# DrorT/demucs

Measured on AMD Instinct MI355X. Metric: real-time factor (audio-sec/wall-sec) htdemucs 4-stem 44.1kHz stereo, 1/8 GPU, higher is better.
Workload: dtype f32

## Files before the change

### demucs_amd/_lib.py

```python
from __future__ import annotations

import ctypes as C
import os
import threading

_HERE = os.path.dirname(os.path.abspath(__file__))
LIB_PATH = os.environ.get("DEMUCS_AMD_LIB") or os.path.join(_HERE, "libdemucs_amd.so")

MI_OK = 0


class MiTensorDesc(C.Structure):
    _fields_ = [("name", C.c_char_p), ("data", C.c_void_p), ("numel", C.c_int64)]


class MiConfig(C.Structure):
    _fields_ = [("n_sources", C.c_int32), ("segment_length", C.c_int32), ("max_batch", C.c_int32),
                ("dtype", C.c_int32)]


class MiProfileRow(C.Structure):
    _fields_ = [("name", C.c_char * 48), ("launches", C.c_int64), ("ms", C.c_double), ("flops", C.c_double),
                ("bytes", C.c_double)]


class MiConvDesc(C.Structure):
    _fields_ = [
        ("wt", C.c_void_p), ("M", C.c_int32), ("Mpad", C.c_int32), ("K", C.c_int32), ("Kpad", C.c_int32),
        ("ktab", C.c_void_p),
        ("x", C.c_void_p), ("x_bstride", C.c_int64),
        ("B", C.c_int32), ("D1", C.c_int32), ("D2", C.c_int32), ("O1", C.c_int32), ("O2", C.c_int32),
        ("S1", C.c_int32), ("S2", C.c_int32),
        ("pro", C.c_int32), ("pro_stats", C.c_void_p), ("pro_w", C.c_void_p), ("pro_b", C.c_void_p),
        ("row_mode", C.c_int32),
        ("epi", C.c_int32), ("flags", C.c_int32),
        ("bias", C.c_void_p), ("scale", C.c_void_p), ("res", C.c_void_p), ("emb", C.c_void_p),
        ("y", C.c_void_p), ("y_bstride", C.c_int64), ("y_cstride", C.c_int64),
        ("stats", C.c_void_p), ("gn_stats", C.c_void_p), ("gn_w", C.c_void_p), ("gn_b", C.c_void_p),
        ("out_len", C.c_int32), ("tile_m", C.c_int32), ("plain", C.c_int32), ("half", C.c_int32),
        ("o2_valid", C.c_int32), ("ktab_len", C.c_int32), ("sink", C.c_void_p), ("wx", C.c_void_p), ("tr_stride", C.c_int32), ("tr_pad", C.c_int32), ("x_ld", C.c_int32), ("x_ld_pad", C.c_int32), ("wh", C.c_void_p),
        ("xh", C.c_void_p), ("xh_n", C.c_int64), ("yh", C.c_void_p), ("yh_n", C.c_int64),
        ("wtap", C.c_void_p), ("ntaps", C.c_int32), ("tap_k2", C.c_int32), ("tap_pad1", C.c_int32), ("tap_pad2", C.c_int32),
        ("tap_dil1", C.c_int32), ("tap_dil2", C.c_int32), ("yh_pq", C.c_int64),
        ("dma_rows", C.c_int32), ("dma_rows_pad", C.c_int32),
    ]


SIGNATURES = {
    "mi_model_create": (C.c_int, [C.POINTER(MiConfig), C.POINTER(MiTensorDesc), C.c_size_t, C.POINTER(C.c_void_p)]),
    "mi_model_destroy": (None, [C.c_void_p]),
    "mi_model_forward": (C.c_int, [C.c_void_p, C.c_void_p, C.c_void_p, C.c_int32, C.c_void_p]),
    "mi_model_forward_core": (C.c_int, [C.c_void_p, C.c_void_p, C.c_void_p, C.c_void_p, C.c_void_p, C.c_int32, C.c_void_p]),
    "mi_model_tap": (C.c_int, [C.c_void_p, C.c_char_p, C.c_void_p, C.c_int32, C.POINTER(C.c_int64), C.c_void_p]),
    "mi_hmodel_create": (C.c_int, [C.POINTER(MiConfig), C.POINTER(MiTensorDesc), C.c_size_t, C.POINTER(C.c_void_p)]),
    "mi_hmodel_destroy": (None, [C.c_void_p]),
    "mi_hmodel_forward": (C.c_int, [C.c_void_p, C.c_void_p, C.c_void_p, C.c_int32, C.c_int32, C.c_void_p]),
    "mi_hmodel_tap": (C.c_int, [C.c_void_p, C.c_char_p, C.c_void_p, C.c_int32, C.POINTER(C.c_int64), C.c_void_p]),
    "mi_hmodel_device_bytes": (C.c_int64, [C.c_void_p]),
    "mi_hmodel_status": (C.c_int, [C.c_void_p, C.c_void_p]),
    "mi_set_two_streams": (C.c_int, [C.c_int32]),
    "mi_set_split_bf16": (C.c_int, [C.c_int32]),
    "mi_set_istft_fused": (C.c_int, [C.c_int32]),
    "mi_set_transpose_tiles": (C.c_int, [C.c_int32]),
    "mi_profile_begin": (C.c_int, [C.c_void_p]),
    "mi_profile_end": (C.c_int, [C.c_void_p, C.POINTER(MiProfileRow), C.c_int32, C.POINTER(C.c_int32), C.c_void_p]),
    "mi_model_device_bytes": (C.c_int64, [C.c_void_p]),
    "mi_segments_gather": (C.c_int, [C.c_void_p, C.c_int64, C.c_int32, C.c_void_p, C.c_int32, C.c_int32, C.c_void_p,
                                     C.c_int64, C.c_void_p]),
    "mi_ola_accumulate": (C.c_int, [C.c_void_p, C.c_int64, C.c_int32, C.c_void_p, C.c_int32, C.c_int64, C.c_void_p, C.c_void_p,
                                    C.c_void_p, C.c_int32, C.c_int64, C.c_int64, C.c_void_p, C.c_int32, C.c_void_p]),
    "mi_ola_finish": (C.c_int, [C.c_void_p, C.c_int64, C.c_int32, C.c_int64, C.c_void_p, C.c_void_p, C.c_int32,
                                C.c_int32, C.c_void_p, C.c_void_p]),
    "mi_segments_gather_packed": (C.c_int, [C.c_void_p, C.c_int64, C.c_int32, C.c_void_p, C.c_int32, C.c_int32, C.c_void_p,
                                            C.c_int64, C.c_void_p]),
    "mi_ola_accumulate_packed": (C.c_int, [C.c_void_p, C.c_int64, C.c_int32, C.c_void_p, C.c_int32, C.c_int64, C.c_void_p, C.c_int32,
                                           C.c_void_p, C.c_int32, C.c_void_p, C.c_int64, C.c_void_p]),
    "mi_ola_finish_packed": (C.c_int, [C.c_void_p, C.c_int64, C.c_int32, C.c_void_p, C.c_int32, C.c_void_p, C.c_int32, C.c_void_p,
                                       C.c_int64, C.c_void_p]),
    "mi_stream_emit": (C.c_int, [C.c_void_p, C.c_int64, C.c_int32, C.c_int32, C.c_void_p, C.c_int32, C.c_void_p, C.c_int32,
                                 C.c_void_p, C.c_int64, C.c_void_p, C.c_int32, C.c_int32, C.c_int32, C.c_void_p, C.c_int64,
                                 C.c_void_p, C.c_int64, C.c_void_p]),
    "mi_streams_emit": (C.c_int, [C.c_void_p, C.c_int64, C.c_int32, C.c_int32, C.c_void_p, C.c_int32, C.c_int64, C.c_void_p,
                                  C.c_int32, C.c_void_p, C.c_int32, C.c_void_p, C.c_int64, C.c_void_p, C.c_int32, C.c_int32,
                                  C.c_int32, C.c_void_p, C.c_int32, C.c_void_p, C.c_int64, C.c_void_p]),
    "mi_streams_append": (C.c_int, [C.c_void_p, C.c_int64, C.c_int32, C.c_void_p, C.c_int32, C.c_int64, C.c_void_p, C.c_int32,
                                    C.c_void_p]),
    "mi_streams_convert_append": (C.c_int, [C.c_void_p, C.c_int64, C.c_int32, C.c_void_p, C.c_int32, C.c_int64, C.c_void_p, C.c_int64,
                                            C.c_void_p, C.c_int64, C.c_void_p, C.c_int32, C.c_int32, C.c_void_p]),
    "mi_pcm_planar": (C.c_int, [C.c_void_p, C.c_int32, C.c_int32, C.c_int64, C.c_int32, C.c_void_p, C.c_void_p, C.c_void_p]),
    "mi_streams_append_pcm": (C.c_int, [C.c_void_p, C.c_int64, C.c_int32, C.c_void_p, C.c_int32, C.c_int64, C.c_void_p, C.c_int32,
                                        C.c_void_p]),
    "mi_streams_convert_append_pcm": (C.c_int, [C.c_void_p, C.c_int64, C.c_int32, C.c_void_p, C.c_int32, C.c_int64, C.c_void_p,
                                                C.c_int64, C.c_void_p, C.c_int64, C.c_void_p, C.c_int32, C.c_int32, C.c_void_p]),
    "mi_streams_compact": (C.c_int, [C.c_void_p, C.c_int64, C.c_void_p, C.c_int64, C.c_void_p, C.c_int32, C.c_int64, C.c_void_p]),
    "mi_mono_stats_scratch_bytes": (C.c_int32, []),
    "mi_mono_stats": (C.c_int, [C.c_void_p, C.c_int32, C.c_int64, C.c_void_p, C.c_void_p, C.c_void_p]),
    "mi_mono_stats_state_bytes": (C.c_int32, []),
    "mi_mono_stats_update": (C.c_int, [C.c_void_p, C.c_int32, C.c_int32, C.c_int64, C.c_int32, C.c_int64, C.c_void_p, C.c_void_p]),
    "mi_mono_stats_finish": (C.c_int, [C.c_void_p, C.c_int64, C.c_void_p, C.c_void_p, C.c_void_p]),
    "mi_sdr_state_bytes": (C.c_int64, [C.c_int32]),
    "mi_sdr_scratch_bytes": (C.c_int64, [C.c_int32]),
    "mi_sdr_update": (C.c_int, [C.c_void_p, C.c_int32, C.c_int32, C.c_int64, C.c_void_p, C.c_int64, C.c_int32, C.c_int32, C.c_int64,
                                C.c_int64, C.c_void_p, C.c_void_p]),
    "mi_sdr_finish": (C.c_int, [C.c_void_p, C.c_int32, C.c_void_p, C.c_void_p, C.c_void_p]),
    "mi_sdr": (C.c_int, [C.c_void_p, C.c_void_p, C.c_int32, C.c_int32, C.c_int32, C.c_int64, C.c_void_p, C.c_void_p, C.c_void_p,
                         C.c_void_p]),
    "mi_track_affine": (C.c_int, [C.c_void_p, C.c_int64, C.c_void_p, C.c_int32, C.c_void_p]),
    "mi_prevent_clip": (C.c_int, [C.c_void_p, C.c_int64, C.c_int32, C.c_void_p, C.c_void_p, C.c_void_p]),
    "mi_two_stems": (C.c_int, [C.c_void_p, C.c_int32, C.c_int32, C.c_void_p, C.c_int32, C.c_int64, C.c_void_p, C.c_void_p]),
    "mi_deliver_peaks": (C.c_int, [C.c_void_p, C.c_int32, C.c_int64, C.c_int32, C.c_int32, C.c_void_p, C.c_int32, C.c_int64, C.c_void_p]),
    "mi_deliver_pcm": (C.c_int, [C.c_void_p, C.c_int32, C.c_int64, C.c_int32, C.c_int32, C.c_void_p, C.c_int32, C.c_void_p, C.c_int64,
                                 C.c_void_p]),
    "mi_deliver_resample_pcm": (C.c_int, [C.c_void_p, C.c_int32, C.c_int64, C.c_int32, C.c_int32, C.c_void_p, C.c_int64, C.c_void_p,
                                          C.c_int64, C.c_int32, C.c_void_p, C.c_int64, C.c_void_p]),
    "mi_stft_cac": (C.c_int, [C.c_void_p, C.c_int32, C.c_int32, C.c_void_p, C.c_void_p]),
    "mi_istft_cac": (C.c_int, [C.c_void_p, C.c_int32, C.c_int32, C.c_int32, C.c_void_p, C.c_void_p]),
    "mi_stft_norm": (C.c_int, [C.c_void_p, C.c_int32, C.c_int32, C.c_void_p, C.c_int32, C.c_void_p, C.c_void_p, C.c_void_p]),
    "mi_istft_full": (C.c_int, [C.c_void_p, C.c_int32, C.c_int32, C.c_int32, C.c_int32, C.c_void_p, C.c_void_p, C.c_int32, C.c_void_p,
                                C.c_void_p, C.c_void_p]),
    "mi_item_norm": (C.c_int, [C.c_void_p, C.c_int32, C.c_int64, C.c_void_p, C.c_void_p, C.c_void_p, C.c_void_p]),
    "mi_item_denorm": (C.c_int, [C.c_void_p, C.c_int32, C.c_int64, C.c_void_p, C.c_void_p, C.c_void_p]),
    "mi_conv_forward": (C.c_int, [C.POINTER(MiConvDesc), C.c_void_p]),
    "mi_resample_frac": (C.c_int, [C.c_void_p, C.c_int32, C.c_int64, C.c_void_p, C.c_int32, C.c_int32, C.c_int32, C.c_void_p, C.c_int64,
                                   C.c_void_p]),
    "mi_conv_pack_split": (C.c_int, [C.c_void_p, C.c_int32, C.c_int32, C.c_int32, C.c_void_p, C.c_void_p]),
    "mi_conv_pack_half": (C.c_int, [C.c_void_p, C.c_int32, C.c_int32, C.c_int32, C.c_void_p, C.c_void_p]),
    "mi_f32_to_image": (C.c_int, [C.c_void_p, C.c_int32, C.c_int32, C.c_int64, C.c_int32, C.c_void_p, C.c_void_p]),
    "mi_conv_pack_tap": (C.c_int, [C.c_void_p, C.c_int32, C.c_int32, C.c_int32, C.c_int32, C.c_void_p, C.c_void_p]),
    "mi_attention": (C.c_int, [C.c_void_p, C.c_void_p, C.c_void_p, C.c_void_p, C.c_int32, C.c_int32, C.c_int32,
                               C.c_int32, C.c_int64, C.c_int64, C.c_int64, C.c_int32, C.c_void_p]),
    "mi_attention_split": (C.c_int, [C.c_void_p, C.c_void_p, C.c_void_p, C.c_void_p, C.c_int32, C.c_int32, C.c_int32,
                                     C.c_int32, C.c_int64, C.c_int64, C.c_int64, C.c_void_p]),
    "mi_attention_heads": (C.c_int, [C.c_void_p, C.c_void_p, C.c_void_p, C.c_void_p, C.c_int32, C.c_int32, C.c_int32, C.c_int32,
                                     C.c_int32, C.c_int32, C.c_int32, C.c_void_p]),
    "mi_attention_heads_image": (C.c_int, [C.c_void_p, C.c_void_p, C.c_void_p, C.c_void_p, C.c_int64, C.c_int32, C.c_int32, C.c_int32,
                                           C.c_int32, C.c_int32, C.c_int32, C.c_int32, C.c_void_p]),
    "mi_attention_image": (C.c_int, [C.c_void_p, C.c_void_p, C.c_void_p, C.c_void_p, C.c_int64, C.c_int32, C.c_int32, C.c_int32,
                                     C.c_int32, C.c_int64, C.c_int64, C.c_int32, C.c_void_p]),
    "mi_lstm_seq": (C.c_int, [C.c_void_p, C.c_void_p, C.c_int32, C.c_int32, C.c_int32, C.c_void_p, C.c_int32, C.c_void_p]),
    "mi_gn_gelu": (C.c_int, [C.c_void_p, C.c_int32, C.c_int32, C.c_int32, C.c_int32, C.c_int32, C.c_int32, C.c_void_p, C.c_void_p,
                             C.c_void_p, C.c_void_p]),
    "mi_gram_order": (C.c_int32, [C.c_int32]),
    "mi_gn_gelu_gram": (C.c_int, [C.c_void_p, C.c_int32, C.c_int32, C.c_int32, C.c_int32, C.c_int32, C.c_int32, C.c_int32, C.c_void_p,
                                  C.c_void_p, C.c_void_p, C.c_void_p, C.c_int32, C.c_void_p]),
    "mi_dconv_gn_gelu_gram": (C.c_int, [C.c_void_p, C.c_int32, C.c_int32, C.c_int32, C.c_int32, C.c_int32, C.c_int32, C.c_int32,
                                        C.c_void_p, C.c_void_p, C.c_void_p, C.c_void_p, C.c_int32, C.c_void_p]),
    "mi_gram_finalize": (C.c_int, [C.c_void_p, C.c_int32, C.c_int32, C.c_int32, C.c_void_p, C.c_void_p, C.c_double, C.c_double,
                                   C.c_double, C.c_double, C.c_float, C.c_void_p, C.c_void_p]),
    "mi_layernorm_cf": (C.c_int, [C.c_void_p, C.c_int32, C.c_int32, C.c_int32, C.c_void_p, C.c_void_p, C.c_void_p,
                                  C.c_void_p, C.c_void_p]),
    "mi_token_norm": (C.c_int, [C.c_int32, C.c_void_p, C.c_int32, C.c_int32, C.c_int32, C.c_void_p, C.c_void_p, C.c_void_p, C.c_void_p,
                                C.c_void_p, C.c_void_p, C.c_void_p, C.c_int64, C.c_int32, C.c_void_p]),
    "mi_local_attn": (C.c_int, [C.c_void_p, C.c_int32, C.c_int32, C.c_int32, C.c_int32, C.c_void_p, C.c_int32, C.c_void_p]),
    "mi_group_norm_apply": (C.c_int, [C.c_void_p, C.c_int32, C.c_int32, C.c_int32, C.c_int32, C.c_int32, C.c_int32, C.c_void_p,
                                      C.c_void_p, C.c_int32, C.c_int32, C.c_void_p, C.c_void_p, C.c_int32, C.c_void_p, C.c_int32,
                                      C.c_int32, C.c_int32, C.c_int32, C.c_void_p, C.c_void_p, C.c_void_p]),
    "mi_blstm_unfold": (C.c_int, [C.c_void_p, C.c_int32, C.c_int32, C.c_int32, C.c_int32, C.c_int32, C.c_int32, C.c_void_p, C.c_void_p]),
    "mi_blstm_restitch": (C.c_int, [C.c_void_p, C.c_int32, C.c_int32, C.c_int32, C.c_int32, C.c_int32, C.c_int32, C.c_void_p,
                                    C.c_void_p, C.c_void_p]),
    "mi_row_affine_pitch": (C.c_int, [C.c_void_p, C.c_int32, C.c_int32, C.c_int32, C.c_int32, C.c_void_p, C.c_void_p, C.c_void_p]),
    "mi_dconv_row": (C.c_int, [C.c_void_p, C.c_void_p, C.c_int32, C.c_int32, C.c_int32, C.c_int32, C.c_void_p, C.c_int32, C.c_void_p]),
    "mi_dconv_time_layer": (C.c_int, [C.c_void_p, C.c_void_p, C.c_int32, C.c_int32, C.c_int32, C.c_int32, C.c_int32, C.c_void_p,
                                      C.c_void_p, C.c_void_p, C.c_void_p, C.c_void_p, C.c_void_p]),
    "mi_debug_set_post_launch_hook": (None, [C.c_void_p]),
    "mi_debug_last_conv_route": (C.c_int, []),
    "mi_debug_last_conv_tile": (C.c_int, []),
    "mi_debug_conv_route": (C.c_int, [C.POINTER(MiConvDesc), C.POINTER(C.c_int)]),
    "mi_debug_switches": (C.c_int, [C.c_char_p, C.c_int32]),
    "mi_last_error": (C.c_char_p, []),
    "mi_version": (C.c_char_p, []),
}

_lib = None
_lock = threading.Lock()


class EngineError(RuntimeError):
    """A libdemucs_amd call returned a non-zero status (the reference convention for this path
    is "exceptions propagate", demucs/apply.py:289-293)."""


def load() -> C.CDLL:
    global _lib
    with _lock:
        if _lib is None:
            if not os.path.exists(LIB_PATH):
                raise EngineError(
                    f"{LIB_PATH} not found: build it with `python -c 'import __graft_entry__ as g; g.build()'` "
                    "(hipcc --offload-arch=gfx950).  demucs_amd has no CPU / eager fallback.")
            lib = C.CDLL(LIB_PATH)
            for name, (res, args) in SIGNATURES.items():
                fn = getattr(lib, name)
                fn.restype = res
                fn.argtypes = args
            _lib = lib
    return _lib


def check(status: int, what: str) -> None:
    if status != MI_OK:
        msg = load().mi_last_error().decode(errors="replace")
        raise EngineError(f"{what} failed ({status}): {msg}")


def current_stream_ptr() -> int:
    import torch
    return torch.cuda.current_stream().cuda_stream
```

### demucs_amd/csrc/api.hip

```cpp
#include <new>

#include "hmodel.h"
#include "model.h"

namespace mi {

post_launch_hook_t g_post_launch_hook = nullptr;
int g_last_conv_route = -1;
int g_last_conv_tile = -1;

char *last_error_buf() {
    static thread_local char buf[1024] = "";
    return buf;
}

int set_error(int code, const char *fmt, ...) {
    va_list ap;
    va_start(ap, fmt);
    vsnprintf(last_error_buf(), 1024, fmt, ap);
    va_end(ap);
    return code;
}

struct Tables {
    FftTables t{};
    bool ready = false;
};
static int get_tables(FftTables *out) {
    static Tables tb;
    if (!tb.ready) {
        const FftHostTables h = fft_host_tables();
        float *dw, *de; float2 *dt;
        MI_HIP(hipMalloc((void **)&dw, 4096 * 4)); MI_HIP(hipMalloc((void **)&dt, h.twiddle.size() * 8)); MI_HIP(hipMalloc((void **)&de, 1024 * 4));
        MI_HIP(hipMemcpy(dw, h.window.data(), 4096 * 4, hipMemcpyHostToDevice));
        MI_HIP(hipMemcpy(dt, h.twiddle.data(), h.twiddle.size() * 8, hipMemcpyHostToDevice));
        MI_HIP(hipMemcpy(de, h.envelope.data(), 1024 * 4, hipMemcpyHostToDevice));
        tb.t = FftTables{dw, dt, de};
        tb.ready = true;
    }
    *out = tb.t;
    return MI_OK;
}

static size_t dconv_layer_floats(int C) { const size_t h = C / 8; return h * C * 3 + 3 * h + 2 * C * h + 6 * (size_t)C + C; }
struct DConvTestLayer {
    std::vector<void *> bufs;
    DConvTimeLayer l{};
    ~DConvTestLayer() { for (void *p : bufs) (void)hipFree(p); }
    template <typename T> int up(const T *h, size_t n, const T **out) {
        void *p = nullptr;
        MI_HIP(hipMalloc(&p, n * sizeof(T)));
        bufs.push_back(p);
        MI_HIP(hipMemcpy(p, h, n * sizeof(T), hipMemcpyHostToDevice));
        *out = (const T *)p;
        return MI_OK;
    }
    int init(int C, const float *w) {
        const int h = C / 8;
        const float *w0 = w, *b0 = w0 + (size_t)h * C * 3, *g1w = b0 + h, *g1b = g1w + h, *w3 = g1b + h, *b3 = w3 + (size_t)2 * C * h,
                    *g2w = b3 + 2 * C, *g2b = g2w + 2 * C, *ls = g2b + 2 * C;
        const DConvHostPack p = dconv_pack_host(C, h, w0, b0, g1w, g1b, w3, b3);
        MI_TRY(up(p.w0.data(), p.w0.size(), &l.w.w0)); MI_TRY(up(p.b0.data(), p.b0.size(), &l.w.b0));
        MI_TRY(up(p.g1w.data(), p.g1w.size(), &l.w.g1w)); MI_TRY(up(p.g1b.data(), p.g1b.size(), &l.w.g1b));
        MI_TRY(up(p.w3.data(), p.w3.size(), &l.w.w3));
        MI_TRY(up(b3, (size_t)2 * C, &l.w.b3)); MI_TRY(up(g2w, (size_t)2 * C, &l.w.g2w)); MI_TRY(up(g2b, (size_t)2 * C, &l.w.g2b));
        MI_TRY(up(ls, (size_t)C, &l.w.ls));
        MI_TRY(up(p.gram_a.data(), p.gram_a.size(), &l.gram_a)); MI_TRY(up(p.gram_v.data(), p.gram_v.size(), &l.gram_v));
        MI_TRY(up(p.gram_c.data(), p.gram_c.size(), &l.gram_c)); MI_TRY(up(p.gram_e1.data(), p.gram_e1.size(), &l.gram_e1));
        MI_TRY(up(p.gram_e2.data(), p.gram_e2.size(), &l.gram_e2));
        l.sum_b3 = p.sum_b3; l.sum_b3sq = p.sum_b3sq;
        return MI_OK;
    }
};

struct TestScratch {
    std::vector<void *> bufs;
    ~TestScratch() { for (void *p : bufs) (void)hipFree(p); }
    template <typename T> int get(size_t n, T **out) {
        void *p = nullptr;
        MI_HIP(hipMalloc(&p, std::max<size_t>(n, 1) * sizeof(T)));
        bufs.push_back(p);
        *out = (T *)p;
        return MI_OK;
    }
};
static int finish_entry(int r, hipStream_t st, const char *who) {
    const hipError_t e = hipStreamSynchronize(st);
    if (e != hipSuccess && r == MI_OK) r = set_error(MI_EHIP, "%s: hipStreamSynchronize: %s", who, hipGetErrorString(e));
    return r;
}

static int stft_entry(const char *who, const float *mix_dev, int B, int L, float *x_dev, int x_pitch, float *norm_dev, float *denorm_dev,
                      hipStream_t st) {
    FftTables tb;
    MI_TRY(get_tables(&tb));
    const int T = (L + 1023) / 1024;
    TestScratch ws;
    float *zt = nullptr; double *stats = nullptr;
    MI_TRY(ws.get((size_t)B * T * 4 * 2048, &zt));
    MI_TRY(ws.get((size_t)2 * kStatSlots * B, &stats));
    MI_HIP(hipMemsetAsync(stats, 0, sizeof(double) * 2 * kStatSlots * B, st));
    int r = launch_stft_frames(mix_dev, B, L, tb, zt, stats, st);
    if (r == MI_OK && norm_dev) r = launch_finalize_stats(stats, B, 4.0 * 2048 * T, 1e-5f, 1, (float2 *)norm_dev, (float2 *)denorm_dev, st);
    if (r == MI_OK) r = launch_cac_transpose(zt, B, T, (const float2 *)norm_dev, x_dev, st, x_pitch);
    return finish_entry(r, st, who);
}

static const char *const kKindNames[2] = {"htdemucs", "hdemucs"};
template <typename Engine>
static Engine *engine_of(void *handle, EngineKind want, const char *entry) {
    EngineCore *core = static_cast<EngineCore *>(handle);
    if (core->kind != want) {
        set_error(MI_EINVAL, "%s: the handle belongs to the %s engine, this entry takes one of the %s engine", entry, kKindNames[core->kind], kKindNames[want]);
        return nullptr;
    }
    return static_cast<Engine *>(core);
}
static Model *as_model(void *handle, const char *entry) { return engine_of<Model>(handle, ENGINE_HTDEMUCS, entry); }
static HModel *as_hmodel(void *handle, const char *entry) { return engine_of<HModel>(handle, ENGINE_HDEMUCS, entry); }

}

using namespace mi;

extern "C" {

const char *mi_last_error(void) { return last_error_buf(); }
void mi_debug_set_post_launch_hook(void (*hook)(void *stream)) { g_post_launch_hook = hook; }
int mi_debug_last_conv_route(void) { return g_last_conv_route; }
int mi_debug_last_conv_tile(void) { return g_last_conv_tile; }
int mi_debug_conv_route(const struct mi_conv_desc *desc, int *tile) {
    if (!desc) return -1;
    if (conv_check_tile_m(*desc) != MI_OK) return -1;
    const ConvRoute r = conv_route(*desc);
    if (tile) *tile = r.tile;
    return r.route;
}
const char *mi_version(void) { return "demucs_amd 0.1 gfx950"; }

int mi_model_create(const mi_config *cfg, const mi_tensor_desc *weights, size_t n_weights, void **handle) {
    if (!cfg || !weights || !handle) return set_error(MI_EINVAL, "mi_model_create: null argument");
    *handle = nullptr;
    Model *m = new (std::nothrow) Model();
    if (!m) return set_error(MI_ENOMEM, "mi_model_create: host allocation failed");
    const int r = m->init(*cfg, weights, n_weights);
    if (r != MI_OK) { delete m; return r; }
    *handle = static_cast<EngineCore *>(m);
    return MI_OK;
}

void mi_model_destroy(void *handle) {
    if (!handle) return;
    Model *m = as_model(handle, "mi_model_destroy");
    if (!m) return;
    (void)hipDeviceSynchronize();
    delete m;
}

int mi_model_forward(void *handle, const float *mix_dev, float *out_dev, int32_t B, void *stream) {
    if (!handle) return set_error(MI_EINVAL, "mi_model_forward: null handle");
    Model *m = as_model(handle, "mi_model_forward");
    return m ? m->forward(mix_dev, out_dev, B, (hipStream_t)stream) : MI_EINVAL;
}

int mi_model_tap(void *handle, const char *name, float *dst_dev, int32_t B, int64_t *numel_per_item, void *stream) {
    if (!handle || !name || !numel_per_item) return set_error(MI_EINVAL, "mi_model_tap: null argument");
    Model *m = as_model(handle, "mi_model_tap");
    if (!m) return MI_EINVAL;
    const float *src = nullptr;
    const float **ptr_dev = &src;
    const std::string n(name);
    const int64_t T = m->T, Tf = 8 * T, Tt = m->Lt[4];
    static const int ch[4] = {48, 96, 192, 384}, fr[4] = {512, 128, 32, 8};
    *ptr_dev = nullptr;
    if (n == "x0") { *ptr_dev = m->w_x0; *numel_per_item = 4 * 2048 * T; }
    else if (n == "xt0") { *ptr_dev = m->w_xt0; *numel_per_item = 2 * (int64_t)m->SL; }
    else if (n == "yspec") { *ptr_dev = m->w_yspec; *numel_per_item = 4 * (int64_t)m->S * 2048 * T; }
    else if (n == "ytime") { *ptr_dev = m->w_ytime; *numel_per_item = 2 * (int64_t)m->S * m->SL; }
    else if (n == "tr_f") { *ptr_dev = m->w_tr_x[0][1]; *numel_per_item = 512 * Tf; }
    else if (n == "tr_t") { *ptr_dev = m->w_tr_x[1][1]; *numel_per_item = 512 * Tt; }
    else if (n.size() == 4 && n.compare(0, 3, "enc") == 0 && n[3] >= '0' && n[3] <= '3') {
        const int i = n[3] - '0'; *ptr_dev = m->w_skip[i]; *numel_per_item = (int64_t)ch[i] * fr[i] * T;
    } else if (n.size() == 5 && n.compare(0, 4, "tenc") == 0 && n[4] >= '0' && n[4] <= '3') {
        const int i = n[4] - '0'; *ptr_dev = m->w_skip_t[i]; *numel_per_item = (int64_t)ch[i] * m->Lp[i + 1];
    }
    if (!*ptr_dev) return set_error(MI_EINVAL, "mi_model_tap: unknown tap '%s'", name);
    if (dst_dev) {
        MI_REQUIRE(B >= 1 && B <= m->cfg.max_batch, "mi_model_tap: batch %d out of range", B);
        MI_HIP(hipMemcpyAsync(dst_dev, src, sizeof(float) * (size_t)B * *numel_per_item, hipMemcpyDeviceToDevice, (hipStream_t)stream));
    }
    return MI_OK;
}

int mi_model_forward_core(void *handle, const float *mix_dev, const float *mag_dev, float *spec_out_dev, float *time_out_dev,
                          int32_t B, void *stream) {
    if (!handle) return set_error(MI_EINVAL, "mi_model_forward_core: null handle");
    Model *m = as_model(handle, "mi_model_forward_core");
    return m ? m->forward_core(mix_dev, mag_dev, spec_out_dev, time_out_dev, B, (hipStream_t)stream) : MI_EINVAL;
}

int mi_hmodel_create(const mi_config *cfg, const mi_tensor_desc *weights, size_t n_weights, void **handle) {
    if (!cfg || !weights || !handle) return set_error(MI_EINVAL, "mi_hmodel_create: null argument");
    *handle = nullptr;
    HModel *m = new (std::nothrow) HModel();
    if (!m) return set_error(MI_ENOMEM, "mi_hmodel_create: host allocation failed");
    const int r = m->hinit(*cfg, weights, n_weights);
    if (r != MI_OK) { delete m; return r; }
    *handle = static_cast<EngineCore *>(m);
    return MI_OK;
}

void mi_hmodel_destroy(void *handle) {
    if (!handle) return;
    HModel *m = as_hmodel(handle, "mi_hmodel_destroy");
    if (!m) return;
    (void)hipDeviceSynchronize();
    delete m;
}

int mi_hmodel_forward(void *handle, const float *mix_dev, float *out_dev, int32_t B, int32_t length, void *stream) {
    if (!handle) return set_error(MI_EINVAL, "mi_hmodel_forward: null handle");
    HModel *m = as_hmodel(handle, "mi_hmodel_forward");
    return m ? m->hforward(mix_dev, out_dev, B, length, (hipStream_t)stream) : MI_EINVAL;
}

int mi_hmodel_tap(void *handle, const char *name, float *dst_dev, int32_t B, int64_t *numel_per_item, void *stream) {
    if (!handle || !name || !numel_per_item) return set_error(MI_EINVAL, "mi_hmodel_tap: null argument");
    HModel *m = as_hmodel(handle, "mi_hmodel_tap");
    if (!m) return MI_EINVAL;
    auto it = m->taps.find(name);
    if (it == m->taps.end()) return set_error(MI_EINVAL, "mi_hmodel_tap: unknown tap '%s'", name);
    *numel_per_item = it->second.second;
    if (dst_dev) {
        MI_REQUIRE(B >= 1 && B <= m->cfg.max_batch, "mi_hmodel_tap: batch %d out of range", B);
        MI_HIP(hipMemcpyAsync(dst_dev, it->second.first, sizeof(float) * (size_t)B * it->second.second, hipMemcpyDeviceToDevice, (hipStream_t)stream));
    }
    return MI_OK;
}

int mi_hmodel_status(void *handle, void *stream) {
    if (!handle) return set_error(MI_EINVAL, "mi_hmodel_status: null handle");
    HModel *m = as_hmodel(handle, "mi_hmodel_status");
    if (!m) return MI_EINVAL;
    MI_HIP(hipStreamSynchronize((hipStream_t)stream));
    MI_REQUIRE(!m->lstm_timeout || *(volatile unsigned *)m->lstm_timeout == 0,
               "a forward's persistent LSTM kernel timed out waiting for its hidden-state exchange (GPU shared with another process's "
               "persistent kernels?): its output and every later one are invalid; MI_LSTM_STEPS=1 selects the one-launch-per-step recurrence");
    return MI_OK;
}

int64_t mi_hmodel_device_bytes(void *handle) {
    HModel *m = handle ? as_hmodel(handle, "mi_hmodel_device_bytes") : nullptr;
    return m ? m->weights.bytes + m->work.bytes : 0;
}

int mi_set_two_streams(int32_t enabled) {
    const int old = g_two_streams;
    g_two_streams = enabled ? 1 : 0;
    return old;
}

int mi_set_istft_fused(int32_t enabled) {
    const int old = g_istft_fused;
    g_istft_fused = enabled ? 1 : 0;
    return old;
}

int mi_set_split_bf16(int32_t enabled) {
    const int old = g_split_bf16;
    g_split_bf16 = enabled ? 1 : 0;
    return old;
}

int mi_set_transpose_tiles(int32_t enabled) {
    const int old = g_transpose_tiles == 7 ? 1 : g_transpose_tiles;
    g_transpose_tiles = enabled == 1 ? 7 : (enabled & 7);
    return old;
}

int mi_profile_begin(void *handle) {
    if (!handle) return set_error(MI_EINVAL, "mi_profile_begin: null handle");
    static_cast<EngineCore *>(handle)->prof.begin();
    return MI_OK;
// ... 626 lines not shown
```

### demucs_amd/csrc/common.h

```cpp
#pragma once
#include <hip/hip_runtime.h>
#include <cstdarg>
#include <cstdint>
#include <cstdio>
#include <cstring>
#include <string>

#include "../../include/demucs_amd.h"

namespace mi {

char *last_error_buf();
int set_error(int code, const char *fmt, ...);

#define MI_HIP(expr)                                                                              \
    do {                                                                                          \
        hipError_t _e = (expr);                                                                   \
        if (_e != hipSuccess)                                                                     \
            return mi::set_error(MI_EHIP, "%s failed: %s (%s:%d)", #expr, hipGetErrorString(_e), \
                                 __FILE__, __LINE__);                                             \
    } while (0)

typedef void (*post_launch_hook_t)(void *stream);
extern post_launch_hook_t g_post_launch_hook;
extern int g_last_conv_route;
extern int g_last_conv_tile;

#define MI_CHECK_LAUNCH()                                                   \
    do {                                                                    \
        MI_HIP(hipGetLastError());                                          \
        if (mi::g_post_launch_hook) mi::g_post_launch_hook((void *)st);     \
    } while (0)

#define MI_REQUIRE(cond, ...)                                  \
    do {                                                       \
        if (!(cond)) return mi::set_error(MI_EINVAL, __VA_ARGS__); \
    } while (0)

#define MI_TRY(expr)              \
    do {                          \
        int _r = (expr);          \
        if (_r != MI_OK) return _r; \
    } while (0)

static inline int ceil_div(int64_t a, int64_t b) { return (int)((a + b - 1) / b); }

__device__ __forceinline__ float gelu_exact(float x) {
    const float t = fminf(fabsf(x), 5.586143494f);
    float q = 5.128879366e-07f;
    q = fmaf(q, t, -9.561274965e-06f);
    q = fmaf(q, t, 7.498410559e-05f);
    q = fmaf(q, t, -2.843918046e-04f);
    q = fmaf(q, t, 1.508691730e-05f);
    q = fmaf(q, t, 6.931011099e-03f);
    q = fmaf(q, t, -5.243470520e-02f);
    q = fmaf(q, t, -4.592214525e-01f);
    q = fmaf(q, t, -1.151104212e+00f);
    const float e = __builtin_amdgcn_exp2f(q * t);
    return 0.5f * x * (1.0f + copysignf(1.0f - e, x));
}
__device__ __forceinline__ float sigmoid_f(float x) {
    return __builtin_amdgcn_rcpf(1.0f + __builtin_amdgcn_exp2f(-1.44269504088896341f * x));
}

__device__ __forceinline__ float tanh_f(float x) {
    const float e = __builtin_amdgcn_exp2f(-2.88539008177792681f * fabsf(x));
    return copysignf((1.0f - e) * __builtin_amdgcn_rcpf(1.0f + e), x);
}
__device__ __forceinline__ unsigned lstm_tag(int step) { return (((unsigned)step >> 1) & 1u) ^ 1u; }
__device__ __forceinline__ float lstm_cell(float ai, float af, float ag, float ao, float &c, unsigned tag) {
    c = sigmoid_f(af) * c + sigmoid_f(ai) * tanh_f(ag);
    const float h = sigmoid_f(ao) * tanh_f(c);
    return __uint_as_float((__float_as_uint(h) & ~1u) | tag);
}

__device__ __forceinline__ unsigned pack_half2(int dtype, float a, float b) {
    typedef __bf16 pk_bf16x2 __attribute__((ext_vector_type(2)));
    typedef _Float16 pk_f16x2 __attribute__((ext_vector_type(2)));
    if (dtype == 1 ) {
        const pk_bf16x2 h = {(__bf16)a, (__bf16)b};
        return __builtin_bit_cast(unsigned, h);
    }
    const pk_f16x2 h = {(_Float16)a, (_Float16)b};
    return __builtin_bit_cast(unsigned, h);
}

#pragma clang diagnostic push
#pragma clang diagnostic ignored "-Winline-asm"
__device__ __forceinline__ void lds_dma16(const void *g, void *lds_wave_base) {
    const unsigned l = (unsigned)(uintptr_t)(__attribute__((address_space(3))) void *)lds_wave_base;
    asm volatile("s_mov_b32 m0, %1\n\ts_nop 0\n\tglobal_load_lds_dwordx4 %0, off" ::"v"(g), "s"(l) : "memory", "m0");
}
__device__ __forceinline__ void lds_dma16_s(const void *sbase, unsigned voff, void *lds_wave_base) {
    const unsigned l = (unsigned)(uintptr_t)(__attribute__((address_space(3))) void *)lds_wave_base;
    asm volatile("s_mov_b32 m0, %2\n\ts_nop 0\n\tglobal_load_lds_dwordx4 %0, %1" ::"v"(voff), "s"(sbase), "s"(l) : "memory", "m0");
}
#pragma clang diagnostic pop
__device__ __forceinline__ void lds_dma16_tracked(const void *g, void *lds_wave_base) {
    __builtin_amdgcn_global_load_lds((__attribute__((address_space(1))) const void *)g, (__attribute__((address_space(3))) void *)lds_wave_base,
                                     16, 0, 0);
}

typedef float v2f __attribute__((ext_vector_type(2)));
__device__ __forceinline__ v2f fma2(v2f a, v2f b, v2f c) { return __builtin_elementwise_fma(a, b, c); }
__device__ __forceinline__ v2f splat2(float x) { return (v2f){x, x}; }

constexpr int kStatSlots = 32;

}
```

### demucs_amd/csrc/conv_route.hip

```cpp
#include "common.h"
#include "kernels.h"

namespace mi {

int g_split_bf16 = 1;

int conv_pick_tile(int M) {
    if (M <= 32) return 32;
    if (M <= 64) return 64;
    if (M % 128 == 0) return 128;
    if (M % 96 == 0) return 96;
    if (M <= 96) return 96;
    return 128;
}

static bool under_filled(const mi_conv_desc &d, int tile = 128) {
    return (int64_t)(d.Mpad / tile) * ceil_div((int64_t)d.B * d.O1 * d.O2, BN) < 200;
}

static bool dmatap_eligible(const mi_conv_desc &d, int tile, bool has_image, bool split = false) {
    const bool off = switches().no_dma_tap;
    const int ld = d.x_ld ? d.x_ld : d.D2;
    if (switches().no_dma_dconv && d.epi == MI_EPI_BIAS_STATS) return false;
    const int dil = d.tap_dil2 ? d.tap_dil2 : 1;
    const bool kind = (d.epi == MI_EPI_GLU && (tile == 96 || tile == 128) && (d.ntaps == 9 || d.ntaps == 3) && dil == 1) ||
                      (d.epi == MI_EPI_BIAS_STATS && (tile == 32 || tile == 64) && d.ntaps == 3 && (dil == 1 || dil == 2) && d.flags == 0);
    return !off && !d.half && (split ? has_image && d.epi == MI_EPI_GLU : !has_image) && kind && d.tap_k2 == 3 && d.Mpad % tile == 0 &&
           d.K % d.ntaps == 0 && d.S1 == 1 && d.S2 == 1 && d.O1 == d.D1 && d.O2 == ld && ld % 4 == 0 && d.tap_pad2 == dil &&
           d.tap_pad1 == (d.ntaps / 3 - 1) / 2 && !(d.flags & (MI_FLAG_IMG | MI_FLAG_IMG4)) && d.x_bstride == (int64_t)(d.K / d.ntaps) * d.D1 * ld;
}
static bool dmarow_eligible(const mi_conv_desc &d, int tile, bool plain, bool has_image, bool split = false) {
    const bool off = switches().no_dma_rows;
    const int ld = d.x_ld ? d.x_ld : d.D2;
    const int lf = d.flags & (MI_FLAG_GELU | MI_FLAG_SCALE | MI_FLAG_RES | MI_FLAG_LN | MI_FLAG_STATS | MI_FLAG_IMG | MI_FLAG_IMG4 | MI_FLAG_HEADS);
    const bool epi_ok = (d.epi == MI_EPI_LINEAR && lf == MI_FLAG_GELU && !plain) || d.epi == MI_EPI_CONVTR ||
                        ((d.epi == MI_EPI_GLU || d.epi == MI_EPI_GN_GLU) && plain && tile == 128 && !(d.flags & (MI_FLAG_IMG | MI_FLAG_IMG4)));
    if (split && (d.epi == MI_EPI_GN_GLU || tile == 64)) return false;
    return !off && !d.half && (split ? has_image : !has_image) && d.ktab && epi_ok && (plain || d.dma_rows) && (tile == 64 || tile == 96 || tile == 128) &&
           d.Mpad % tile == 0 && d.S2 == 1 && d.O2 == ld && ld % 4 == 0 && ((uintptr_t)d.x & 3) == 0 && ((uintptr_t)d.ktab & 63) == 0 &&
           (d.epi == MI_EPI_CONVTR || tile != 64 || d.epi == MI_EPI_LINEAR);
}

int conv_check_tile_m(const mi_conv_desc &d) {
    MI_REQUIRE(d.tile_m != 192 || (d.M > 0 && d.M % 192 == 0 && d.Mpad == d.M), "conv: tile_m 192 needs M %% 192 == 0 and no M padding (M %d, Mpad %d)", d.M, d.Mpad);
    return MI_OK;
}

static bool conv_plain(const mi_conv_desc &d) {
    const int64_t P = (int64_t)d.O1 * d.O2;
    return d.plain && (d.xh || (d.K == d.Kpad && P % 4 == 0 && d.x_bstride % 4 == 0 && ((uintptr_t)d.x & 15) == 0)) &&
           d.S1 == 1 && d.S2 == 1 && d.D1 == d.O1 && (d.x_ld ? d.x_ld : d.D2) == d.O2;
}

static bool half_img256_only(int f) { return f == (MI_FLAG_LN | MI_FLAG_HEADS) || f == (MI_FLAG_LN | MI_FLAG_GELU | MI_FLAG_IMG); }
static int half_linear_flags(const mi_conv_desc &d) {
    return d.flags & (MI_FLAG_GELU | MI_FLAG_SCALE | MI_FLAG_RES | MI_FLAG_LN | MI_FLAG_IMG | MI_FLAG_HEADS | MI_FLAG_STATS);
}

int conv_validate(const mi_conv_desc &d) {
    MI_TRY(conv_check_tile_m(d));
    MI_REQUIRE((int64_t)d.Mpad * d.y_cstride < (1ll << 31), "conv: output channel stride too large for 32-bit row offsets");
    MI_REQUIRE(d.Kpad % BK == 0 && d.Kpad >= BK, "conv: Kpad %d must be a positive multiple of %d", d.Kpad, BK);
    MI_REQUIRE(d.Mpad % 4 == 0, "conv: Mpad %d must be a multiple of 4", d.Mpad);
    MI_REQUIRE(d.O2 >= 32 || d.row_mode == 0 || (d.epi != MI_EPI_BIAS_STATS && d.epi != MI_EPI_STATS_ONLY),
               "conv: statistics epilogue needs O2 >= 32");
    MI_REQUIRE(d.pro == 0, "conv: the fused GroupNorm+GELU prologue was replaced by launch_gn_gelu");
    MI_REQUIRE(!(d.flags & MI_FLAG_IMG4) || (d.epi == MI_EPI_GLU && d.half && d.yh && d.yh_pq > 0 && d.yh_n >= (int64_t)d.B * d.yh_pq && d.M % 32 == 0 &&
                                             ((uintptr_t)d.yh & 15) == 0),
               "conv: MI_FLAG_IMG4 needs a half-mode GLU layer with M %% 32 == 0 and an aligned phase image of >= B * yh_pq positions per plane");
    MI_REQUIRE(!(d.flags & MI_FLAG_STATS) || (d.epi == MI_EPI_LINEAR && d.stats && d.O2 >= 32 && d.row_mode == 0),
               "conv: MI_FLAG_STATS needs a LINEAR layer, a statistics buffer and O2 >= 32");
    MI_REQUIRE(!(d.flags & MI_FLAG_LN) || (d.pro_stats && d.scale && d.epi == MI_EPI_LINEAR), "conv: MI_FLAG_LN needs pro_stats and scale");
    const int64_t P = (int64_t)d.O1 * d.O2;
    MI_REQUIRE(!(d.flags & MI_FLAG_IMG) || d.epi == MI_EPI_CONVTR ||
               (d.half && d.yh && d.epi == MI_EPI_LINEAR && d.M % 8 == 0 && d.yh_n >= (int64_t)d.B * P && ((uintptr_t)d.yh & 15) == 0) ||
               (d.half && d.yh && d.epi == MI_EPI_GLU && d.M % 32 == 0 && !(d.flags & (MI_FLAG_IMG4 | MI_FLAG_EMB)) && d.yh_n >= (int64_t)d.B * P &&
                ((uintptr_t)d.yh & 15) == 0),
               "conv: MI_FLAG_IMG needs a half-precision LINEAR layer with M %% 8 == 0 (or GLU layer with M %% 32 == 0) and an aligned "
               "output image of >= B * P columns");
    MI_REQUIRE(d.epi != MI_EPI_CONVTR || ((int64_t)d.Mpad * d.y_cstride < (1ll << 30) && (d.tr_stride == 0 || d.tr_stride == 2 || d.tr_stride == 4) &&
                                          d.M % (d.tr_stride == 2 ? 2 : 4) == 0),
               "conv: transposed conv needs stride 2 or 4, M a multiple of it and 30-bit output offsets per item");
    {
        const int f = d.flags & (MI_FLAG_GELU | MI_FLAG_RES | MI_FLAG_IMG);
        MI_REQUIRE(d.epi != MI_EPI_CONVTR || f == 0 || (d.tr_stride != 2 && (f == (MI_FLAG_GELU | MI_FLAG_RES) || f == (MI_FLAG_GELU | MI_FLAG_RES | MI_FLAG_IMG))),
                   "conv: transposed conv epilogue supports no flags, GELU|RES or GELU|RES|IMG (stride 2: no flags), got %d", d.flags);
    }
    MI_REQUIRE(!(d.flags & MI_FLAG_IMG) || d.epi != MI_EPI_CONVTR ||
               (d.half && d.yh && d.yh_n >= (int64_t)d.B * d.y_cstride && ((uintptr_t)d.yh & 15) == 0),
               "conv: MI_FLAG_IMG on a transposed conv needs a half mode and an output image of >= B * y_cstride positions");
    MI_REQUIRE(!d.wtap || (d.half && d.xh), "conv: tap-ordered weights need a half mode and an operand-image input");
    MI_REQUIRE(d.wtap || !(d.flags & MI_FLAG_HEADS) || (d.half && d.yh && d.epi == MI_EPI_LINEAR && d.M % 512 == 0 && d.O1 == 1 && d.yh_n >= d.O2 &&
                                                        ((uintptr_t)d.yh & 15) == 0 && !(d.flags & MI_FLAG_IMG)),
               "conv: MI_FLAG_HEADS needs a half-precision LINEAR layer on tokens (O1 = 1) with M %% 512 == 0 and an aligned output");
    MI_REQUIRE(!d.xh || d.half, "conv: an operand-image input needs a half-precision layer");
    if (d.xh && !d.wtap) {
        const int f = half_linear_flags(d);
        MI_REQUIRE(d.epi == MI_EPI_LINEAR && conv_plain(d), "conv: an operand-image input needs a plain LINEAR layer");
        MI_REQUIRE(f == (MI_FLAG_SCALE | MI_FLAG_RES) || f == (MI_FLAG_SCALE | MI_FLAG_RES | MI_FLAG_STATS) || half_img256_only(f),
                   "conv: an operand-image input is not instantiated for LINEAR flags %d", d.flags);
    }
    return MI_OK;
}

ConvRoute conv_route(const mi_conv_desc &d) {
    const bool image = d.wx && g_split_bf16;
    const Switches &sw = switches();
    const int tile = d.tile_m && d.tile_m != 192 ? d.tile_m : conv_pick_tile(d.M);
    const bool plain = conv_plain(d);
    if (d.wtap) return {MI_ROUTE_TAP_HALF, tile, plain};
    if (d.half && d.xh) {
        const int f = half_linear_flags(d);
        const bool wide = d.Mpad % 256 == 0;
        if (half_img256_only(f) || (f == (MI_FLAG_SCALE | MI_FLAG_RES) && sw.img256 && wide)) return {MI_ROUTE_HALF_IMG256, 256, plain};
        return {MI_ROUTE_HALF_IMG, wide ? 256 : 128, plain};
    }
    if (d.half) return {MI_ROUTE_HALF, sw.half_tile256 && plain && tile == 128 && d.epi == MI_EPI_LINEAR && d.Mpad % 256 == 0 ? 256 : tile, plain};
    const bool t192 = d.tile_m == 192 && image;
    const bool small = sw.small_tile && tile == 128 && !t192 && under_filled(d), small_linear = small && plain && d.epi == MI_EPI_LINEAR;
    const int lf = d.flags & (MI_FLAG_GELU | MI_FLAG_SCALE | MI_FLAG_RES | MI_FLAG_LN | MI_FLAG_STATS);
    auto split_tile = [&](int ntaps) {
        if (!t192) return small ? 64 : tile;
        const bool filled = !(sw.small_tile && under_filled(d, 192));
        return filled && conv_x6_tile192(d.epi, d.epi == MI_EPI_LINEAR ? lf : 0, plain, ntaps) ? 192 : 96;
    };
    if (!plain && !sw.x6_plain_only && dmatap_eligible(d, tile, image, true)) return {MI_ROUTE_TAP_X6, split_tile(d.ntaps), plain};
    if (!sw.x6_plain_only && dmarow_eligible(d, tile, plain, image, true)) return {MI_ROUTE_ROWS_X6, split_tile(kRowTaps), plain};
    const int ktile = small && !plain && d.epi == MI_EPI_GLU && d.Mpad % 96 == 0 ? 96 : tile;
    if (!plain && dmatap_eligible(d, ktile, image)) return {MI_ROUTE_DMATAP, ktile, plain};
    if (dmarow_eligible(d, tile, plain, image)) return {MI_ROUTE_DMAROW, tile, plain};
    if (image && conv_x6_supported(tile) && (!sw.x6_plain_only || plain)) return {MI_ROUTE_X6, t192 ? split_tile(0) : small_linear ? 64 : tile, plain};
    const int ntile = small_linear && d.Mpad % 64 == 0 ? 64 : tile;
    const bool dma = plain && ntile == 128 && d.epi == MI_EPI_LINEAR && !sw.no_dma;
    return {dma ? MI_ROUTE_DMA : MI_ROUTE_TABLE, ntile, plain, sw.mgroups};
}

}
```

### demucs_amd/csrc/engine_core.h

```cpp
#pragma once
#include <algorithm>
#include <cstring>
#include <map>
#include <string>
#include <vector>

#include "common.h"
#include "gemm_conv.h"
#include "kernels.h"

namespace mi {

extern int g_two_streams;

struct DeviceArena {
    int64_t bytes = 0;
    DeviceArena() = default;
    DeviceArena(const DeviceArena &) = delete;
    DeviceArena &operator=(const DeviceArena &) = delete;
    int alloc(void **p, size_t n);
    void release(void *p);
    ~DeviceArena();

   private:
    std::map<void *, size_t> sizes;
};

struct PackedConv {
    float *wt = nullptr, *bias = nullptr;
    void *wx = nullptr;
    void *wh = nullptr;
    void *wtap = nullptr;
    int ntaps = 0;
    int M = 0, Mpad = 0, K = 0, Kpad = 0, tile = 0, half = 0;
};

struct DConvLayerW {
    PackedConv conv3, conv1;
    mi_ktab_entry *ktab3 = nullptr, *ktab1 = nullptr;
    float *gn1_w = nullptr, *gn1_b = nullptr, *gn2_w = nullptr, *gn2_b = nullptr, *ls = nullptr;
    double *gram_wt = nullptr, *gram_ct = nullptr, sum_b = 0.0, sum_bsq = 0.0;
};
struct DConvW {
    DConvLayerW l[2];
    int h = 0;
    bool has_row = false;
    DConvRowLayer row[2];
    bool has_time = false;
    DConvTimeLayer tl[2];
};

struct ProfRow {
    int cls = 0;
    char name[48] = "";
    long long launches = 0;
    double ms = 0.0, flops = 0.0, bytes = 0.0;
};
struct Profiler {
    bool on = false;
    struct Pending { int cls; hipEvent_t a, b; double flops, bytes; long long launches = 1; };
    std::vector<Pending> pending;
    std::vector<hipEvent_t> pool;
    ProfRow rows[128];
    hipEvent_t get();
    template <typename Fn>
    int timed(int cls, const char *name, double flops, double bytes, hipStream_t st, Fn &&fn, long long launches = 1) {
        if (!on) return fn();
        Pending p{cls, get(), get(), flops, bytes, launches};
        MI_HIP(hipEventRecord(p.a, st));
        const int r = fn();
        MI_HIP(hipEventRecord(p.b, st));
        pending.push_back(p);
        if (name) snprintf(rows[cls].name, sizeof(rows[cls].name), "%s", name);
        return r;
    }
    void begin();
    int end(hipStream_t st);
    ~Profiler();
};

enum SplitScope {
    SPLIT_OPT_IN,
    SPLIT_DEFAULT,
    SPLIT_ROWS,
};

struct WeightTable {
    std::map<std::string, std::pair<const float *, int64_t>> t;
    int get(const std::string &name, int64_t numel, const float **out) const {
        auto it = t.find(name);
        if (it == t.end()) return set_error(MI_EWEIGHT, "missing tensor '%s'", name.c_str());
        if (it->second.second != numel)
            return set_error(MI_EWEIGHT, "tensor '%s' has %lld elements, expected %lld", name.c_str(),
                             (long long)it->second.second, (long long)numel);
        *out = it->second.first;
        return MI_OK;
    }
};

static inline int round_up(int v, int m) { return (v + m - 1) / m * m; }

struct Gather {
    int Cin, K1, K2, dil1, dil2, pad1, pad2;
    int64_t chan_stride;
    int D2;
};

static inline std::vector<mi_ktab_entry> build_ktab(const Gather &g, int Kpad) {
    std::vector<mi_ktab_entry> tab(Kpad);
    const int K = g.Cin * g.K1 * g.K2;
    for (int k = 0; k < Kpad; ++k) {
        mi_ktab_entry e;
        if (k < K) {
            const int ci = k / (g.K1 * g.K2), r = k % (g.K1 * g.K2), k1 = r / g.K2, k2 = r % g.K2;
            e.d1 = k1 * g.dil1 - g.pad1;
            e.d2 = k2 * g.dil2 - g.pad2;
            e.off = (int32_t)(ci * g.chan_stride + (int64_t)e.d1 * g.D2 + e.d2);
            e.ci = ci;
        } else {
            e.d1 = -(1 << 29); e.d2 = -(1 << 29); e.off = 0; e.ci = 0;
        }
        tab[k] = e;
    }
    return tab;
}

struct Geo {
    int B, D1, D2;
    int row_mode;
    int ld;
    int pitch() const { return ld ? ld : D2; }
};

static inline mi_conv_desc base_desc(const PackedConv &pc, const mi_ktab_entry *ktab, const float *x, int64_t x_bs, const Geo &g) {
    mi_conv_desc d;
    memset(&d, 0, sizeof(d));
    d.wt = pc.wt; d.M = pc.M; d.Mpad = pc.Mpad; d.K = pc.K; d.Kpad = pc.Kpad; d.ktab = ktab; d.bias = pc.bias; d.tile_m = pc.tile; d.wx = pc.wx;
    d.wh = pc.wh; d.half = pc.wh ? pc.half : 0; d.ktab_len = round_up(pc.Kpad, 32);
    d.x = x; d.x_bstride = x_bs; d.B = g.B; d.D1 = g.D1; d.D2 = g.D2; d.O1 = g.D1; d.O2 = g.pitch(); d.S1 = 1; d.S2 = 1;
    d.o2_valid = g.pitch() != g.D2 ? g.D2 : 0;
    d.x_ld = g.pitch() != g.D2 ? g.pitch() : 0;
    d.row_mode = g.row_mode;
    return d;
}

enum EngineKind { ENGINE_HTDEMUCS, ENGINE_HDEMUCS };

struct EngineCore {
    const EngineKind kind;
    mi_config cfg{};
    Profiler prof;
    int conv(const mi_conv_desc &d, hipStream_t st);
    DeviceArena weights;
    FftTables fft{};

    hipStream_t side_st = nullptr;
    hipEvent_t ev_main = nullptr, ev_side = nullptr;
    int side_streams();

   protected:
    explicit EngineCore(EngineKind k) : kind(k) {}
    ~EngineCore();
    template <typename T> int upload(const std::vector<T> &h, T **dptr) {
        void *p = nullptr;
        MI_TRY(weights.alloc(&p, std::max<size_t>(h.size(), 1) * sizeof(T)));
        MI_HIP(hipMemcpy(p, h.data(), h.size() * sizeof(T), hipMemcpyHostToDevice));
        *dptr = (T *)p;
        return MI_OK;
    }
    int upload_fft_tables();
    int pack_split(PackedConv *pc, SplitScope scope);
    int pack_half(PackedConv *pc);
    int pack_conv(const float *W, const float *bias, int M, int K, bool glu, PackedConv *pc, int ntaps = 0, SplitScope scope = SPLIT_OPT_IN);
    int pack_tap(PackedConv *pc, int ntaps);
    int pack_enc_tap(const float *W, int Cin, PackedConv *pc);
    int pack_convtr(const float *W, const float *bias, int Cin, int Cout, PackedConv *pc, int stride = 4, SplitScope scope = SPLIT_OPT_IN);
    int pack_vec(const float *v, int n, int npad, bool glu, float **out);
    int pack_linear_ln(const float *W, const float *bias, const float *ln_w, const float *ln_b, int M, int K, PackedConv *pc,
                       float **c1, SplitScope scope);
    int make_ktab(const Gather &g, int Kpad, mi_ktab_entry **out);
    int load_dconv(const WeightTable &wt, const std::string &prefix, int C, int64_t chan_stride, int D2, bool freq, DConvW *dw, int comp = 8);
    double *dconv_gram = nullptr;
    double *dconv_gram2 = nullptr;
    size_t dconv_gram2_bytes = 0;
    bool dconv_tap_dma = false;
    int run_dconv(const DConvW &w, int C, const Geo &g, float *x, float *tmp, float *hidden, double *stats, float2 *st1, float2 *st2,
                  hipStream_t st, double *gram2 = nullptr, size_t gram2_cap = 0);
};

}
```

### demucs_amd/csrc/engine_core.hip

```cpp
#include <cmath>
#include <string>
#include <vector>

#include "engine_core.h"

namespace mi {

int DeviceArena::alloc(void **p, size_t n) {
    n = (n + 255) & ~(size_t)255;
    hipError_t e = hipMalloc(p, n);
    if (e != hipSuccess) return set_error(MI_ENOMEM, "hipMalloc(%zu) failed: %s", n, hipGetErrorString(e));
    sizes[*p] = n;
    bytes += (int64_t)n;
    return MI_OK;
}
void DeviceArena::release(void *p) {
    auto it = sizes.find(p);
    if (it == sizes.end()) return;
    (void)hipFree(p);
    bytes -= (int64_t)it->second;
    sizes.erase(it);
}
DeviceArena::~DeviceArena() {
    for (auto &a : sizes) (void)hipFree(a.first);
}

int EngineCore::upload_fft_tables() {
    const FftHostTables h = fft_host_tables();
    float *dw, *de; float2 *dt;
    MI_TRY(upload(h.window, &dw)); MI_TRY(upload(h.twiddle, &dt)); MI_TRY(upload(h.envelope, &de));
    fft = FftTables{dw, dt, de};
    return MI_OK;
}

EngineCore::~EngineCore() {
    if (side_st) (void)hipStreamDestroy(side_st);
    if (ev_main) (void)hipEventDestroy(ev_main);
    if (ev_side) (void)hipEventDestroy(ev_side);
}

int g_two_streams = 1;

int EngineCore::side_streams() {
    if (side_st) return MI_OK;
    const int prio = switches().side_prio;
    if (prio) {
        int least = 0, greatest = 0;
        MI_HIP(hipDeviceGetStreamPriorityRange(&least, &greatest));
        MI_HIP(hipStreamCreateWithPriority(&side_st, hipStreamNonBlocking, prio < 0 ? least : greatest));
    } else
        MI_HIP(hipStreamCreateWithFlags(&side_st, hipStreamNonBlocking));
    MI_HIP(hipEventCreateWithFlags(&ev_main, hipEventDisableTiming));
    MI_HIP(hipEventCreateWithFlags(&ev_side, hipEventDisableTiming));
    return MI_OK;
}

hipEvent_t Profiler::get() {
    if (!pool.empty()) { hipEvent_t e = pool.back(); pool.pop_back(); return e; }
    hipEvent_t e;
    (void)hipEventCreate(&e);
    return e;
}
void Profiler::begin() {
    for (auto &r : rows) r = ProfRow();
    on = true;
}
int Profiler::end(hipStream_t st) {
    on = false;
    MI_HIP(hipStreamSynchronize(st));
    for (auto &p : pending) {
        float ms = 0.f;
        MI_HIP(hipEventElapsedTime(&ms, p.a, p.b));
        ProfRow &r = rows[p.cls];
        r.cls = p.cls; r.launches += p.launches; r.ms += ms; r.flops += p.flops; r.bytes += p.bytes;
        pool.push_back(p.a); pool.push_back(p.b);
    }
    pending.clear();
    return MI_OK;
}
Profiler::~Profiler() {
    for (auto &p : pending) { (void)hipEventDestroy(p.a); (void)hipEventDestroy(p.b); }
    for (auto e : pool) (void)hipEventDestroy(e);
}

static const char *kEpiNames[6] = {"linear", "glu", "bias_stats", "stats_only", "gn_glu", "convtr"};

int EngineCore::conv(const mi_conv_desc &d, hipStream_t st) {
    if (!prof.on) return launch_conv(d, st);
    const int route = conv_route(d).route;
    const int tile = d.tile_m && d.tile_m != 192 ? d.tile_m : conv_pick_tile(d.M), ti = tile == 32 ? 0 : tile == 64 ? 1 : tile == 96 ? 2 : 3;
    const bool tap_x6 = route == MI_ROUTE_TAP_X6, rows_x6 = route == MI_ROUTE_ROWS_X6;
    const int cls = tap_x6    ? 105 + (d.ntaps == 9 ? 2 : 0) + (tile == 128 ? 1 : 0)
                    : rows_x6 ? 109 + (d.epi == MI_EPI_CONVTR ? 4 : d.epi == MI_EPI_GLU ? 2 : 0) + (tile == 128 ? 1 : 0)
                              : (route >= MI_ROUTE_X6 ? 48 : 0) + d.epi * 8 + ti * 2 + (d.plain ? 1 : 0);
    const double N = (double)d.B * d.O1 * d.O2;
    const double in_bytes = 4.0 * (double)d.B * (double)d.x_bstride;
    double out_rows = d.M;
    if (d.epi == MI_EPI_GLU || d.epi == MI_EPI_GN_GLU) out_rows = d.M / 2;
    if (d.epi == MI_EPI_CONVTR) out_rows = d.M;
    if (d.epi == MI_EPI_STATS_ONLY) out_rows = 0;
    double bytes = in_bytes + 4.0 * out_rows * N + 4.0 * (double)d.M * d.K;
    if (d.flags & MI_FLAG_RES || d.epi == MI_EPI_GN_GLU) bytes += 4.0 * out_rows * N;
    char name[sizeof(ProfRow::name)];
    const bool unnamed = !prof.rows[cls].name[0];
    if (unnamed && tap_x6)
        snprintf(name, sizeof(name), "conv_tap_x6<%s,tile%d,taps%d>", kEpiNames[d.epi], tile, d.ntaps);
    else if (unnamed && rows_x6)
        snprintf(name, sizeof(name), "conv_rows_x6<%s,tile%d>", kEpiNames[d.epi], tile);
    else if (unnamed)
        snprintf(name, sizeof(name), "conv_gemm%s<%s,tile%d%s>", d.half == MI_DTYPE_BF16 ? "_bf16" : d.half == MI_DTYPE_F16 ? "_f16" : cls >= 48 ? "_x6" : "",
                 kEpiNames[d.epi], tile, d.plain ? ",1x1" : "");
    return prof.timed(cls, unnamed ? name : nullptr, 2.0 * d.M * (double)d.K * N, bytes, st, [&] { return launch_conv(d, st); });
}

int EngineCore::pack_split(PackedConv *pc, SplitScope scope) {
    const Switches &sw = switches();
    const bool in_default = scope == SPLIT_DEFAULT || (scope == SPLIT_ROWS && !sw.no_dma_rows);
    const bool want = sw.x6_scope == 2 || (sw.x6_scope == 1 && in_default && cfg.dtype == MI_DTYPE_F32);
    if (!want || !conv_x6_supported(pc->tile)) return MI_OK;
    const bool t192 = pc->M % 192 == 0 && pc->Mpad == pc->M;
    MI_TRY(weights.alloc(&pc->wx, (size_t)6 * pc->Kpad * pc->Mpad));
    MI_TRY(launch_pack_split(pc->wt, pc->Kpad, pc->Mpad, t192 ? 96 : pc->tile, pc->wx, nullptr));
    MI_HIP(hipStreamSynchronize(nullptr));
    if (t192) pc->tile = 192;
    return MI_OK;
}

int EngineCore::pack_half(PackedConv *pc) {
    if (cfg.dtype == MI_DTYPE_F32) return MI_OK;
    const int Kh = round_up(pc->Kpad, 32);
    MI_TRY(weights.alloc(&pc->wh, (size_t)2 * Kh * pc->Mpad));
    pc->half = cfg.dtype;
    MI_TRY(launch_pack_half(pc->wt, pc->Kpad, pc->Mpad, cfg.dtype, pc->wh, nullptr));
    MI_HIP(hipStreamSynchronize(nullptr));
    return MI_OK;
}

int EngineCore::pack_tap(PackedConv *pc, int ntaps) {
    if (cfg.dtype == MI_DTYPE_F32 || switches().no_tap_image || ntaps < 2 || pc->K % ntaps || (pc->K / ntaps) % 8) return MI_OK;
    const int Cin = pc->K / ntaps;
    MI_TRY(weights.alloc(&pc->wtap, (size_t)16 * conv_tap_pairs_pad(Cin, ntaps) * pc->Mpad));
    pc->ntaps = ntaps;
    MI_TRY(launch_pack_tap(pc->wt, pc->Mpad, Cin, ntaps, cfg.dtype, pc->wtap, nullptr));
    MI_HIP(hipStreamSynchronize(nullptr));
    return MI_OK;
}

int EngineCore::pack_enc_tap(const float *W , int Cin, PackedConv *pc) {
    if (cfg.dtype == MI_DTYPE_F32 || switches().no_enc_image || switches().no_tap_image || Cin % 8) return MI_OK;
    const int M = pc->M, K = 8 * Cin;
    std::vector<float> wt((size_t)K * pc->Mpad, 0.f);
    for (int m = 0; m < M; ++m)
        for (int ci = 0; ci < Cin; ++ci)
            for (int rho = 0; rho < 4; ++rho)
                for (int j = 0; j < 2; ++j) {
                    const int tau = 4 * (j - (rho >= 2)) + rho + 2, ce = ((ci >> 3) * 4 + rho) * 8 + (ci & 7);
                    wt[(size_t)(ce * 2 + j) * pc->Mpad + m] = W[((size_t)m * Cin + ci) * 8 + tau];
                }
    float *tmp = nullptr;
    MI_HIP(hipMalloc((void **)&tmp, wt.size() * sizeof(float)));
    MI_HIP(hipMemcpy(tmp, wt.data(), wt.size() * sizeof(float), hipMemcpyHostToDevice));
    int r = weights.alloc(&pc->wtap, (size_t)16 * conv_tap_pairs_pad(4 * Cin, 2) * pc->Mpad);
    if (r == MI_OK) r = launch_pack_tap(tmp, pc->Mpad, 4 * Cin, 2, cfg.dtype, pc->wtap, nullptr);
    (void)hipStreamSynchronize(nullptr);
    (void)hipFree(tmp);
    if (r == MI_OK) pc->ntaps = 2;
    return r;
}

int EngineCore::pack_conv(const float *W, const float *bias, int M, int K, bool glu, PackedConv *pc, int ntaps, SplitScope scope) {
    const int tile = conv_pick_tile(M);
    pc->M = M; pc->K = K; pc->Mpad = round_up(M, tile); pc->Kpad = round_up(K, 16); pc->tile = tile;
    std::vector<float> wt((size_t)pc->Kpad * pc->Mpad, 0.f), b(pc->Mpad, 0.f);
    for (int m = 0; m < M; ++m) {
        const int src = glu ? ((m & 1) ? (m >> 1) + M / 2 : (m >> 1)) : m;
        for (int k = 0; k < K; ++k) wt[(size_t)k * pc->Mpad + m] = W[(size_t)src * K + k];
        b[m] = bias ? bias[src] : 0.f;
    }
    MI_TRY(upload(wt, &pc->wt));
    MI_TRY(upload(b, &pc->bias));
    MI_TRY(pack_half(pc));
    MI_TRY(pack_tap(pc, ntaps));
    return pack_split(pc, scope);
}

int EngineCore::pack_convtr(const float *W, const float *bias, int Cin, int Cout, PackedConv *pc, int stride, SplitScope scope) {
    const int M = stride * Cout, K = 2 * Cin, ks = 2 * stride;
    const int tile = conv_pick_tile(M);
    pc->M = M; pc->K = K; pc->Mpad = round_up(M, tile); pc->Kpad = round_up(K, 16); pc->tile = tile;
    std::vector<float> wt((size_t)pc->Kpad * pc->Mpad, 0.f), b(pc->Mpad, 0.f);
    for (int ci = 0; ci < Cin; ++ci)
        for (int co = 0; co < Cout; ++co)
            for (int r = 0; r < stride; ++r)
                for (int j = 0; j < 2; ++j)
                    wt[(size_t)(2 * ci + j) * pc->Mpad + stride * co + r] = W[((size_t)ci * Cout + co) * ks + r + stride * j];
    for (int co = 0; co < Cout; ++co)
        for (int r = 0; r < stride; ++r) b[stride * co + r] = bias[co];
    MI_TRY(upload(wt, &pc->wt));
    MI_TRY(upload(b, &pc->bias));
    MI_TRY(pack_half(pc));
    MI_TRY(pack_tap(pc, 2));
    return pack_split(pc, scope);
}

int EngineCore::pack_linear_ln(const float *W, const float *bias, const float *ln_w, const float *ln_b, int M, int K, PackedConv *pc,
                               float **c1, SplitScope scope) {
    std::vector<float> wf((size_t)M * K), c2(M), c1h(M);
    for (int m = 0; m < M; ++m) {
        double s1 = 0.0, s2 = bias ? (double)bias[m] : 0.0;
        for (int k = 0; k < K; ++k) {
            const float wp = W[(size_t)m * K + k] * ln_w[k];
            wf[(size_t)m * K + k] = wp;
            s1 += (double)wp;
            s2 += (double)W[(size_t)m * K + k] * (double)ln_b[k];
        }
        c1h[m] = (float)s1; c2[m] = (float)s2;
    }
    MI_TRY(pack_conv(wf.data(), c2.data(), M, K, false, pc, 0, scope));
    return pack_vec(c1h.data(), M, pc->Mpad, false, c1);
}

int EngineCore::pack_vec(const float *v, int n, int npad, bool glu, float **out) {
    std::vector<float> h(npad, 0.f);
    for (int m = 0; m < n; ++m) h[m] = v[glu ? ((m & 1) ? (m >> 1) + n / 2 : (m >> 1)) : m];
    return upload(h, out);
}

int EngineCore::make_ktab(const Gather &g, int Kpad, mi_ktab_entry **out) {
    return upload(build_ktab(g, round_up(Kpad, 32)), out);
}

int EngineCore::load_dconv(const WeightTable &wt, const std::string &prefix, int C, int64_t chan_stride, int D2, bool freq, DConvW *dw, int comp) {
    const int h = C / comp;
    dw->h = h;
    dw->has_row = comp == 8 && freq && dconv_row_supported(C, D2);
    dw->has_time = comp == 8 && !freq && !switches().no_dconv_time && dconv_time_supported(C, D2);
    for (int d = 0; d < 2; ++d) {
        DConvLayerW &l = dw->l[d];
        const std::string p = prefix + ".dconv.layers." + std::to_string(d);
        const float *w0, *b0, *g1w, *g1b, *w3, *b3, *g2w, *g2b, *ls;
        MI_TRY(wt.get(p + ".0.weight", (int64_t)h * C * 3, &w0));
        MI_TRY(wt.get(p + ".0.bias", h, &b0));
        MI_TRY(wt.get(p + ".1.weight", h, &g1w));
        MI_TRY(wt.get(p + ".1.bias", h, &g1b));
        MI_TRY(wt.get(p + ".3.weight", (int64_t)2 * C * h, &w3));
        MI_TRY(wt.get(p + ".3.bias", 2 * C, &b3));
        MI_TRY(wt.get(p + ".4.weight", 2 * C, &g2w));
        MI_TRY(wt.get(p + ".4.bias", 2 * C, &g2b));
        MI_TRY(wt.get(p + ".6.scale", C, &ls));
        MI_TRY(pack_conv(w0, b0, h, 3 * C, false, &l.conv3));
        const int dil = 1 << d;
        MI_TRY(make_ktab(Gather{C, 1, 3, 1, dil, 0, dil, chan_stride, D2}, l.conv3.Kpad, &l.ktab3));
        const int hp = round_up(h, 16);
        std::vector<float> w3p((size_t)2 * C * hp, 0.f);
        for (int m = 0; m < 2 * C; ++m)
            for (int k = 0; k < h; ++k) w3p[(size_t)m * hp + k] = w3[(size_t)m * h + k];
        MI_TRY(pack_conv(w3p.data(), b3, 2 * C, hp, true, &l.conv1));
        MI_TRY(make_ktab(Gather{hp, 1, 1, 1, 1, 0, 0, chan_stride, D2}, l.conv1.Kpad, &l.ktab1));
        MI_TRY(pack_vec(g1w, h, h, false, &l.gn1_w));
        MI_TRY(pack_vec(g1b, h, h, false, &l.gn1_b));
        MI_TRY(pack_vec(g2w, 2 * C, l.conv1.Mpad, true, &l.gn2_w));
        MI_TRY(pack_vec(g2b, 2 * C, l.conv1.Mpad, true, &l.gn2_b));
        MI_TRY(pack_vec(ls, C, C, false, &l.ls));
        {
            const int HP = gram_hp(h);
            std::vector<double> gw((size_t)HP * HP, 0.0), gc(HP, 0.0);
            double sb = 0.0, sbq = 0.0;
            for (int m = 0; m < 2 * C; ++m) { sb += (double)b3[m]; sbq += (double)b3[m] * (double)b3[m]; }
            for (int i = 0; i < h; ++i) {
                for (int k = 0; k < h; ++k) {
// ... 80 lines not shown
```

### demucs_amd/csrc/gemm_conv.h

```cpp
#pragma once
#include <stdint.h>

#ifdef __cplusplus
extern "C" {
#endif

enum mi_epilogue {
    MI_EPI_LINEAR = 0,
    MI_EPI_GLU = 1,
    MI_EPI_BIAS_STATS = 2,
    MI_EPI_STATS_ONLY = 3,
    MI_EPI_GN_GLU = 4,
    MI_EPI_CONVTR = 5
};

#define MI_FLAG_GELU 1
#define MI_FLAG_SCALE 2
#define MI_FLAG_RES 4
#define MI_FLAG_EMB 8
#define MI_FLAG_TR_FREQ 16
#define MI_FLAG_LN 32
#define MI_FLAG_IMG 64
#define MI_FLAG_HEADS 128
#define MI_FLAG_STATS 256
#define MI_FLAG_IMG4 512

#define MI_SINK_FLOATS 256
#define MI_ZERO_PAGE_FLOATS 64

typedef struct mi_ktab_entry {
    int32_t off;
    int32_t d1;
    int32_t d2;
    int32_t ci;
} mi_ktab_entry;

typedef struct mi_conv_desc {
    const float *wt;
    int32_t M, Mpad, K, Kpad;
    const mi_ktab_entry *ktab;
    const float *x;
    int64_t x_bstride;
    int32_t B, D1, D2, O1, O2, S1, S2;
    int32_t pro;
    const float *pro_stats;
    const float *pro_w, *pro_b;
    int32_t row_mode;
    int32_t epi, flags;
    const float *bias;
    const float *scale;
    const float *res;
    const float *emb;
    float *y;
    int64_t y_bstride, y_cstride;
    double *stats;
    const float *gn_stats;
    const float *gn_w, *gn_b;
    int32_t out_len;
    int32_t tile_m;
    int32_t plain;
    int32_t half;
    int32_t o2_valid;
    int32_t ktab_len;
    float *sink;
    const void *wx;
    int32_t tr_stride;
    int32_t tr_pad;
    int32_t x_ld;
    int32_t x_ld_pad;
    const void *wh;
    const void *xh;
    int64_t xh_n;
    void *yh;
    int64_t yh_n;
    const void *wtap;
    int32_t ntaps, tap_k2, tap_pad1, tap_pad2;
    int32_t tap_dil1, tap_dil2;
    int64_t yh_pq;
    int32_t dma_rows;
    int32_t dma_rows_pad;
} mi_conv_desc;

#ifdef __cplusplus
}
#endif
```

### demucs_amd/csrc/gemm_conv.hip

```cpp
#include "gemm_loop.h"

namespace mi {

template <int WM, int WN, int TM, int TN, int EPI, int LFLAGS, bool PLAIN>
__global__ __launch_bounds__(256, (TM * TN == 4 ? 3 : 4)) void conv_gemm_kernel(const mi_conv_desc d, const int N, const int MT, const int Gm) {
    constexpr int BM = WM * TM * 32;
    static_assert(WN * TN * 32 == BN, "block N tile is 128");
    static_assert(WM * WN == 4, "4 waves");
    __shared__ float As[2][BK][BM];
    __shared__ float Bs[2][BK][BN];
    Wg w;
    if (!wg_tile<WN, BM>(d, MT, Gm, N, w)) return;
    const int tid = w.tid;

    constexpr int A_F4 = BK * BM / 4, A_FULL = A_F4 / 256, A_REM = A_F4 % 256;
    constexpr int A_SLOTS = A_FULL + (A_REM ? 1 : 0);
    static_assert(A_SLOTS <= 2, "A tile fits two float4 per thread");
    const int aidx0 = tid < A_F4 ? tid : 0, aidx1 = (tid + 256 < A_F4) ? tid + 256 : 0;
    const int ar0 = aidx0 / (BM / 4), ac0 = (aidx0 % (BM / 4)) * 4;
    const int ar1 = aidx1 / (BM / 4), ac1 = (aidx1 % (BM / 4)) * 4;
    const bool a_on0 = tid < A_F4, a_on1 = tid + 256 < A_F4;
    const float *ap0 = d.wt + (size_t)ar0 * d.Mpad + w.m0 + ac0;
    const float *ap1 = d.wt + (size_t)ar1 * d.Mpad + w.m0 + ac1;
    const size_t a_step = (size_t)BK * d.Mpad;
// ... 35 lines not shown
        } else {                                                                                      \
            _Pragma("unroll") for (int j = 0; j < 8; ++j)                                              \
                Bs[buf][khalf + 2 * j][tid & 127] = bok[j] ? breg[j] : 0.f;                            \
        }                                                                                             \
        if (A_SLOTS >= 1 && a_on0) *reinterpret_cast<float4 *>(&As[buf][ar0][ac0]) = areg0;           \
        if (A_SLOTS >= 2 && a_on1) *reinterpret_cast<float4 *>(&As[buf][ar1][ac1]) = areg1;           \
    } while (0)

    f32x16 acc[TM][TN];
    zero_acc(acc);

    const int nk = d.Kpad / BK;
    MI_LOAD_TILE(0);
    MI_STORE_TILE(0);
    __syncthreads();
    int cur = 0;
    for (int kt = 0; kt < nk; ++kt) {
        if (kt + 1 < nk) MI_LOAD_TILE(kt + 1);
        fp32_kstep<TM, TN, BM>(&As[cur][0][0], &Bs[cur][0][0], w, acc);
        if (kt + 1 < nk) MI_STORE_TILE(cur ^ 1);
        __syncthreads();
        cur ^= 1;
    }
#undef MI_LOAD_TILE
#undef MI_STORE_TILE

    conv_epilogue<TM, TN, EPI, LFLAGS>(d, acc, w.m0, w.n0, w.wm, w.wn, N, w.P, w.o2v);
}

template <int BM, int EPI, int LFLAGS, int NT, int DIL, bool ROWPAIRS>
__device__ __forceinline__ void conv_dma_body(const mi_conv_desc &d, const int N, const int MT, const int Gm) {
    constexpr int WM = BM == 128 ? 2 : 1, WN = 4 / WM, TM = BM / (32 * WM), TN = BN / (32 * WN);
    constexpr int SS = BK * (BM + BN);
    __shared__ __attribute__((aligned(16))) float smem[3 * SS];
    Wg w;
    if (!wg_tile<WN, BM>(d, MT, Gm, N, w)) return;
    const AImagePlan<BM, ROWPAIRS> A(d, w);
    BLoader<NT, DIL> B(d, w, N, (int64_t)d.D1 * (d.x_ld ? d.x_ld : d.D2));
    const auto brows = [&](int stage) { return smem + stage * SS + BK * BM + (4 * w.wave) * BN; };
    f32x16 acc[TM][TN];
    zero_acc(acc);
    dma_ring3(
        d.Kpad / BK, kBInFlight + A.in_flight(), [&](int kt) { B.prefetch(kt); },
        [&](int kt, int stage) {
            A.issue(kt, smem + stage * SS);
            B.issue(d, kt, brows(stage));
        },
        [&](int kt, int stage) {
            if constexpr (NT > 0) {
                B.fix(d, kt, brows(stage));
                asm volatile("s_waitcnt lgkmcnt(0)" ::: "memory");
            }
        },
        [&](int stage) { fp32_kstep<TM, TN, BM>(smem + stage * SS, smem + stage * SS + BK * BM, w, acc); });
    conv_epilogue<TM, TN, EPI, LFLAGS>(d, acc, w.m0, w.n0, w.wm, w.wn, N, w.P, w.o2v);
}

template <int EPI, int LFLAGS>
__global__ __launch_bounds__(256, 3) void conv_gemm_dma_kernel(const mi_conv_desc d, const int N, const int MT, const int Gm) {
    conv_dma_body<128, EPI, LFLAGS, 0, 1, true>(d, N, MT, Gm);
}

template <int BMT, int EPI, int NT, int DIL = 1>
__global__ __launch_bounds__(256, 3) void conv_gemm_dmatap_kernel(const mi_conv_desc d, const int N, const int MT, const int Gm) {
    conv_dma_body<BMT, EPI, 0, NT, DIL, true>(d, N, MT, Gm);
}

template <int EPI>
static int launch_dmatap(const mi_conv_desc &d, int tile, hipStream_t st) {
    ConvGeom g;
    MI_TRY(conv_geom(d, "conv: DMA tap route", tile, tile, g));
    if constexpr (EPI == MI_EPI_BIAS_STATS) {
        const bool d2 = d.tap_dil2 == 2;
        if (tile == 64 && d2) MI_LAUNCH_TILES((conv_gemm_dmatap_kernel<64, EPI, 3, 2>), d, g, 1, st);
        else if (tile == 64) MI_LAUNCH_TILES((conv_gemm_dmatap_kernel<64, EPI, 3, 1>), d, g, 1, st);
        else if (d2) MI_LAUNCH_TILES((conv_gemm_dmatap_kernel<32, EPI, 3, 2>), d, g, 1, st);
        else MI_LAUNCH_TILES((conv_gemm_dmatap_kernel<32, EPI, 3, 1>), d, g, 1, st);
    } else if (tile == 128 && d.ntaps == 9) MI_LAUNCH_TILES((conv_gemm_dmatap_kernel<128, EPI, 9>), d, g, 1, st);
    else if (tile == 128) MI_LAUNCH_TILES((conv_gemm_dmatap_kernel<128, EPI, 3>), d, g, 1, st);
    else if (d.ntaps == 9) MI_LAUNCH_TILES((conv_gemm_dmatap_kernel<96, EPI, 9>), d, g, 1, st);
    else MI_LAUNCH_TILES((conv_gemm_dmatap_kernel<96, EPI, 3>), d, g, 1, st);
    return MI_OK;
}

template <int BMT, int EPI, int LFLAGS>
__global__ __launch_bounds__(256, 3) void conv_gemm_dmarow_kernel(const mi_conv_desc d, const int N, const int MT, const int Gm) {
    conv_dma_body<BMT, EPI, LFLAGS, kRowTaps, 1, false>(d, N, MT, Gm);
}

template <int EPI, int LFLAGS>
static int launch_dmarow(const mi_conv_desc &d, int tile, hipStream_t st) {
    ConvGeom g;
    MI_TRY(conv_geom(d, "conv: DMA row route", tile, tile, g));
    if (tile == 128) MI_LAUNCH_TILES((conv_gemm_dmarow_kernel<128, EPI, LFLAGS>), d, g, 1, st);
    else if constexpr (EPI == MI_EPI_LINEAR || EPI == MI_EPI_CONVTR) {
        if (tile == 96) MI_LAUNCH_TILES((conv_gemm_dmarow_kernel<96, EPI, LFLAGS>), d, g, 1, st);
        else MI_LAUNCH_TILES((conv_gemm_dmarow_kernel<64, EPI, LFLAGS>), d, g, 1, st);
    } else return set_error(MI_EINVAL, "conv: DMA row route has no %d-row tile for epilogue %d", tile, EPI);
    return MI_OK;
}

template <int WM, int WN, int TM, int TN, int EPI, int LFLAGS, bool PLAIN>
static int launch_cfg(const mi_conv_desc &d, const ConvRoute &r, hipStream_t st) {
    constexpr int BM = WM * TM * 32;
    const bool dma = r.route == MI_ROUTE_DMA;
    ConvGeom g;
    MI_TRY(conv_geom(d, "conv", BM, BM, g));
    const int Gm = r.mgroups ? pick_m_groups(g.MT, (size_t)d.Kpad * d.Mpad * 4) : 1;
    if constexpr (PLAIN && BM == 128 && EPI == MI_EPI_LINEAR) {
        if (dma) {
            MI_LAUNCH_TILES((conv_gemm_dma_kernel<EPI, LFLAGS>), d, g, Gm, st);
            return MI_OK;
        }
    }
    MI_REQUIRE(!dma, "conv: the LDS-DMA linear tile takes a plain LINEAR layer on the 128-row tile");
    MI_LAUNCH_TILES((conv_gemm_kernel<WM, WN, TM, TN, EPI, LFLAGS, PLAIN>), d, g, Gm, st);
    return MI_OK;
}

template <int EPI, int LFLAGS, bool PLAIN>
static int launch_tile(const mi_conv_desc &d, const ConvRoute &r, hipStream_t st) {
    switch (r.tile) {
        case 128: return launch_cfg<2, 2, 2, 2, EPI, LFLAGS, PLAIN>(d, r, st);
        case 96: return launch_cfg<1, 4, 3, 1, EPI, LFLAGS, PLAIN>(d, r, st);
        case 64: return launch_cfg<1, 4, 2, 1, EPI, LFLAGS, PLAIN>(d, r, st);
        case 32: return launch_cfg<1, 4, 1, 1, EPI, LFLAGS, PLAIN>(d, r, st);
    }
    return set_error(MI_EINVAL, "conv: unsupported tile_m %d", r.tile);
}

static float *conv_sink() {
    static float *p = nullptr;
    if (!p) {
        if (hipMalloc((void **)&p, (MI_SINK_FLOATS + MI_ZERO_PAGE_FLOATS) * sizeof(float)) != hipSuccess) { p = nullptr; return nullptr; }
        (void)hipMemset(p, 0, (MI_SINK_FLOATS + MI_ZERO_PAGE_FLOATS) * sizeof(float));
    }
    return p;
}

const void *conv_zero_page() {
    float *p = conv_sink();
    return p ? p + MI_SINK_FLOATS : nullptr;
}

int launch_conv(const mi_conv_desc &din, hipStream_t st) {
    mi_conv_desc d = din;
    if (!d.sink) d.sink = conv_sink();
    MI_REQUIRE(d.sink && ((uintptr_t)d.sink & 15) == 0, "conv: the store sink could not be allocated or is not 16-byte aligned");
    MI_TRY(conv_validate(d));
    const ConvRoute r = conv_route(d);
    const int image_tile = d.tile_m == 192 ? 96 : d.tile_m ? d.tile_m : conv_pick_tile(d.M);
    g_last_conv_route = r.route;
    g_last_conv_tile = r.tile;
    switch (r.route) {
        case MI_ROUTE_TAP_HALF: return launch_conv_tap(d, r.tile, st);
        case MI_ROUTE_HALF:
        case MI_ROUTE_HALF_IMG:
        case MI_ROUTE_HALF_IMG256: return launch_conv_half(d, r, st);
        case MI_ROUTE_TAP_X6: return launch_conv_tap_x6(d, r.tile, image_tile, st);
        case MI_ROUTE_ROWS_X6: return launch_conv_rows_x6(d, r.tile, image_tile, st);
        case MI_ROUTE_X6: return launch_conv_x6(d, r.tile, image_tile, r.plain, st);
        case MI_ROUTE_DMATAP:
            return d.epi == MI_EPI_GLU ? launch_dmatap<MI_EPI_GLU>(d, r.tile, st) : launch_dmatap<MI_EPI_BIAS_STATS>(d, r.tile, st);
        case MI_ROUTE_DMAROW:
            switch (d.epi) {
                case MI_EPI_LINEAR: return launch_dmarow<MI_EPI_LINEAR, MI_FLAG_GELU>(d, r.tile, st);
                case MI_EPI_CONVTR: return launch_dmarow<MI_EPI_CONVTR, 0>(d, r.tile, st);
                case MI_EPI_GLU: return launch_dmarow<MI_EPI_GLU, 0>(d, r.tile, st);
                case MI_EPI_GN_GLU: return launch_dmarow<MI_EPI_GN_GLU, 0>(d, r.tile, st);
            }
            return set_error(MI_EINVAL, "conv: DMA row route has no epilogue %d", d.epi);
    }
    return dispatch_epilogue(d, [&](auto epi, auto lflags) {
        constexpr int E = decltype(epi)::value, F = decltype(lflags)::value;
        return r.plain ? launch_tile<E, F, true>(d, r, st) : launch_tile<E, F, false>(d, r, st);
    });
}

}
```

### demucs_amd/csrc/gemm_loop.h

```cpp
#pragma once
#include "gemm_tile.h"

namespace mi {

struct Wg {
    int tid, lane, li, lh;
    int wave, wm, wn;
    int mt, nt, m0, n0;
    int P, o2v;
};
template <int WN>
__device__ __forceinline__ Wg wg_lanes(const mi_conv_desc &d) {
    Wg w;
    w.tid = threadIdx.x; w.lane = w.tid & 63; w.li = w.lane & 31; w.lh = w.lane >> 5;
    w.wave = __builtin_amdgcn_readfirstlane(w.tid >> 6);
    w.wm = w.wave / WN; w.wn = w.wave % WN;
    w.mt = w.nt = w.m0 = w.n0 = 0;
    w.P = d.O1 * d.O2;
    w.o2v = d.o2_valid ? d.o2_valid : d.O2;
    return w;
}
template <int WN, int BM>
__device__ __forceinline__ bool wg_tile(const mi_conv_desc &d, int MT, int Gm, int N, Wg &w) {
    w = wg_lanes<WN>(d);
// ... 94 lines not shown
    issue(0, 0);
    if (nk > 1) { prefetch(1); issue(1, 1); }
    int stage = 0;
    for (int kt = 0; kt < nk; ++kt) {
        if (kt + 2 < nk) prefetch(kt + 2);
        if (kt + 1 < nk) wait_vmcnt(in_flight);
        else wait_vmcnt(0);
        landed(kt, stage);
        __builtin_amdgcn_s_barrier();
        if (kt + 2 < nk) issue(kt + 2, stage == 0 ? 2 : stage - 1);
        step(stage);
        stage = stage == 2 ? 0 : stage + 1;
    }
}

template <int BM, bool ROWPAIRS>
struct AImagePlan {
    static constexpr int NA = BM >= 96 ? 2 : 1;
    const float *src[NA];
    size_t step;
    int lds[NA];
    bool a1, a2;
    __device__ __forceinline__ AImagePlan(const mi_conv_desc &d, const Wg &w) {
        a1 = BM != 32 || w.wave < 2; a2 = BM == 128 || (BM == 96 && w.wave < 2);
        step = (size_t)BK * d.Mpad;
#pragma unroll
        for (int j = 0; j < NA; ++j) {
            int row, col;
            if (ROWPAIRS && BM == 128) { row = 4 * w.wave + 2 * j + w.lh; col = w.li * 4; lds[j] = (4 * w.wave + 2 * j) * BM; }
            else { const int q = j ? 4 + w.wave : w.wave, f = 256 * q + 4 * w.lane; row = f / BM; col = f % BM; lds[j] = 256 * q; }
            src[j] = d.wt + (size_t)row * d.Mpad + w.m0 + col;
        }
    }
    __device__ __forceinline__ int in_flight() const { return a2 ? 2 : a1 ? 1 : 0; }
    __device__ __forceinline__ void issue(int kt, float *sa) const {
#pragma unroll
        for (int j = 0; j < NA; ++j)
            if (j == 0 ? a1 : a2) lds_dma16_tracked(src[j] + (size_t)kt * step, sa + lds[j]);
    }
};

constexpr int kBInFlight = 2;

struct PlainRows {
    const float *src;
    size_t row2, step;
    __device__ __forceinline__ PlainRows(const mi_conv_desc &d, const Wg &w, int N, int64_t) {
        const ColInfo lc = decompose(w.n0 + w.li * 4, N, w.P, d.O2, d.O2);
        src = lc.valid ? d.x + (size_t)lc.b * d.x_bstride + lc.p + (size_t)(4 * w.wave + w.lh) * w.P : d.sink + MI_SINK_FLOATS;
        row2 = lc.valid ? (size_t)2 * w.P : 0; step = lc.valid ? (size_t)BK * w.P : 0;
    }
    __device__ __forceinline__ void prefetch(int) {}
    __device__ __forceinline__ void issue(const mi_conv_desc &, int kt, float *brows) const {
        const float *g = src + (size_t)kt * step;
        lds_dma16_tracked(g, brows);
        lds_dma16_tracked(g + row2, brows + 2 * BN);
    }
    __device__ __forceinline__ void fix(const mi_conv_desc &, int, float *) const {}
};

template <int NT, int DIL>
struct TapRows {
    static constexpr int K2 = 3;
    ColInfo lc;
    const float *xcol;
    int64_t chan;
    int x_ld, rb0, lofs, fix_l, fix_r;
    bool edge;
    __device__ __forceinline__ TapRows(const mi_conv_desc &d, const Wg &w, int N, int64_t chan_stride) {
        lc = decompose(w.n0 + w.li * 4, N, w.P, d.O2, w.o2v);
        x_ld = d.x_ld ? d.x_ld : d.D2;
        chan = chan_stride;
        rb0 = 4 * w.wave + w.lh; lofs = w.lh * BN + w.li * 4;
        xcol = d.x + (size_t)lc.b * d.x_bstride + (size_t)lc.o1 * x_ld + lc.o2;
        fix_l = (lc.valid && lc.o2 == 0) ? 0 : -1;
        const int fr = d.D2 - 1 - lc.o2;
        fix_r = (lc.valid && fr >= 0 && fr < 4) ? fr : -1;
        edge = lc.valid && (lc.o2 < 4 || lc.o2 + 8 > d.D2);
    }
    __device__ __forceinline__ void prefetch(int) {}
    __device__ __forceinline__ int row_k(int kt, int j) const {
        const int k = kt * BK + rb0 + 2 * j;
        __builtin_assume(k >= 0);
        return k;
    }
    __device__ __forceinline__ void issue(const mi_conv_desc &d, int kt, float *brows) const {
        const float *const zero = d.sink + MI_SINK_FLOATS;
#pragma unroll
        for (int j = 0; j < 2; ++j) {
            const int k = row_k(kt, j), ci = k / NT, tap = k - ci * NT, t1 = tap / K2, t2 = tap - t1 * K2;
            const int i1 = lc.o1 + t1 - d.tap_pad1;
            const bool ok = lc.valid && k < d.K && (unsigned)i1 < (unsigned)d.D1;
            const float *g = xcol + (int64_t)ci * chan + (int64_t)(t1 - d.tap_pad1) * x_ld + (t2 * DIL - d.tap_pad2);
            lds_dma16_tracked(ok ? g : zero, brows + 2 * j * BN);
        }
    }
    __device__ __forceinline__ void fix(const mi_conv_desc &d, int kt, float *brows) const {
        float *sb = brows + lofs;
        if constexpr (DIL == 1) {
#pragma unroll
            for (int j = 0; j < 2; ++j) {
                const int k = row_k(kt, j), tap = k % NT, dd2 = tap % K2 - d.tap_pad2;
                if (dd2 < 0 && fix_l >= 0) sb[2 * j * BN + fix_l] = 0.f;
                if (dd2 > 0 && fix_r >= 0) sb[2 * j * BN + fix_r] = 0.f;
            }
        } else if (edge) {
#pragma unroll
            for (int j = 0; j < 2; ++j) {
                const int k = row_k(kt, j), tap = k % NT, dd2 = (tap % K2) * DIL - d.tap_pad2;
#pragma unroll
                for (int e = 0; e < 4; ++e)
                    if ((unsigned)(lc.o2 + e + dd2) >= (unsigned)d.D2) sb[2 * j * BN + e] = 0.f;
            }
        }
    }
};

#define MI_ROW_LOADS "s_load_dwordx2 %0, %4, 0x0\n\ts_load_dwordx2 %1, %4, 0x10\n\ts_load_dwordx2 %2, %4, 0x20\n\t" \
                     "s_load_dwordx2 %3, %4, 0x30\n\t"
struct RowTaps {
    typedef int v2i __attribute__((ext_vector_type(2)));
    const float *xcol;
    const int4 *ktab4;
    int i1b, lh;
    bool valid;
    v2i e0, e1, e2, e3;
    __device__ __forceinline__ RowTaps(const mi_conv_desc &d, const Wg &w, int N, int64_t) {
        const ColInfo lc = decompose(w.n0 + w.li * 4, N, w.P, d.O2, w.o2v);
        valid = lc.valid; lh = w.lh;
        i1b = lc.o1 * d.S1;
        xcol = d.x + (size_t)lc.b * d.x_bstride + (size_t)i1b * (d.x_ld ? d.x_ld : d.D2) + lc.o2;
        ktab4 = reinterpret_cast<const int4 *>(d.ktab) + 4 * w.wave;
    }
    template <bool DRAIN = false>
    __device__ __forceinline__ void prefetch(int kt) {
        if constexpr (DRAIN)
            asm volatile(MI_ROW_LOADS "s_waitcnt vmcnt(0) lgkmcnt(0)" : "=&s"(e0), "=&s"(e1), "=&s"(e2), "=&s"(e3) : "s"(ktab4 + kt * BK) : "memory");
        else
            asm volatile(MI_ROW_LOADS "s_waitcnt lgkmcnt(0)" : "=&s"(e0), "=&s"(e1), "=&s"(e2), "=&s"(e3) : "s"(ktab4 + kt * BK) : "memory");
    }
    __device__ __forceinline__ void issue(const mi_conv_desc &d, int, float *brows) const {
        const float *const zero = d.sink + MI_SINK_FLOATS;
#pragma unroll
        for (int j = 0; j < 2; ++j) {
            const int off = j ? (lh ? e3.x : e2.x) : (lh ? e1.x : e0.x), dd1 = j ? (lh ? e3.y : e2.y) : (lh ? e1.y : e0.y);
            const bool ok = valid && (unsigned)(i1b + dd1) < (unsigned)d.D1;
            lds_dma16_tracked(ok ? xcol + off : zero, brows + 2 * j * BN);
        }
    }
    __device__ __forceinline__ void fix(const mi_conv_desc &, int, float *) const {}
};
#undef MI_ROW_LOADS

template <int NT, int DIL = 1>
using BLoader = std::conditional_t<NT == 0, PlainRows, std::conditional_t<NT == kRowTaps, RowTaps, TapRows<(NT > 0 ? NT : 3), DIL>>>;

struct ConvGeom { int N, MT, NT; };
static inline int conv_geom(const mi_conv_desc &d, const char *what, int tile, int image_rows, ConvGeom &g, int bn = BN) {
    const int64_t N64 = (int64_t)d.B * d.O1 * d.O2;
    MI_REQUIRE(N64 < (1ll << 31) - 256, "%s: too many output positions (%lld)", what, (long long)N64);
    MI_REQUIRE(d.Mpad % image_rows == 0, "%s: Mpad %d not a multiple of the %d-row tile", what, d.Mpad, tile);
    g.N = (int)N64; g.MT = d.Mpad / tile; g.NT = ceil_div(g.N, bn);
    return MI_OK;
}
#define MI_LAUNCH_TILES(kernel, d, g, Gm, st)                                                                          \
    do {                                                                                                          \
        hipLaunchKernelGGL(kernel, dim3(grouped_grid((g).MT, (g).NT, (Gm))), dim3(256), 0, (st), (d), (g).N, (g).MT, (Gm)); \
        MI_CHECK_LAUNCH();                                                                                        \
    } while (0)

}
```

### demucs_amd/csrc/gemm_x6.hip

```cpp
#include "gemm_loop.h"
#include "split_bf16.h"

namespace mi {

__global__ void pack_split_kernel(const float *__restrict__ wt, int Kpad, int Mpad, int BM, __bf16 *__restrict__ wx) {
    const size_t idx = blockIdx.x * (size_t)blockDim.x + threadIdx.x;
    if (idx >= (size_t)Kpad * Mpad) return;
    const int k = (int)(idx / Mpad), m = (int)(idx % Mpad);
    const int mt = m / BM, mi = m % BM, kt = k / BK, h = (k % BK) / 8, j = k % 8, nk = Kpad / BK;
    const float x = wt[idx];
    const __bf16 a = (__bf16)x;
    const float r = x - (float)a;
    const __bf16 b = (__bf16)r;
    const __bf16 c = (__bf16)(r - (float)b);
    __bf16 *img = wx + ((size_t)mt * nk + kt) * ((size_t)BM * 48);
    img[((0 * 2 + h) * BM + mi) * 8 + j] = a;
    img[((1 * 2 + h) * BM + mi) * 8 + j] = b;
    img[((2 * 2 + h) * BM + mi) * 8 + j] = c;
}

int launch_pack_split(const float *wt, int Kpad, int Mpad, int tile_m, void *wx, hipStream_t st) {
    MI_REQUIRE(Kpad % BK == 0 && Mpad % tile_m == 0, "pack_split: Kpad %d / Mpad %d do not fit tile %d", Kpad, Mpad, tile_m);
    const size_t n = (size_t)Kpad * Mpad;
    hipLaunchKernelGGL(pack_split_kernel, dim3((unsigned)((n + 255) / 256)), dim3(256), 0, st, wt, Kpad, Mpad, tile_m, (__bf16 *)wx);
    MI_CHECK_LAUNCH();
    return MI_OK;
}

template <int WM, int WN, int TM, int TN, int EPI, int LFLAGS, bool PLAIN, bool HALF_IMG, int NT>
__device__ __forceinline__ void conv_x6_body(const mi_conv_desc &d, const int N, const int MT, const int Gm) {
    constexpr int BM = WM * TM * 32;
    constexpr bool RAW = PLAIN || NT != 0;
    constexpr bool ROWS = NT == kRowTaps;
    static_assert(NT <= 0 || (!PLAIN && EPI == MI_EPI_GLU), "tap loader: GLU rewrite convs");
    static_assert(!ROWS || (!PLAIN && (EPI == MI_EPI_LINEAR || EPI == MI_EPI_CONVTR || EPI == MI_EPI_GLU)),
                  "row-tap loader: encoder / transposed convs, 1 x 1 + GLU rewrites");
    static_assert(NT >= kRowTaps, "NT: taps, 0 or kRowTaps");
    static_assert(WN * TN * 32 == BN, "block N tile is 128");
    static_assert(WM * WN == 4, "4 waves");
    constexpr int A_BYTES = BM * 96, B_BYTES = BN * 96, STAGE = A_BYTES + B_BYTES;
    constexpr int A_CHUNKS = A_BYTES / 1024;
    static_assert(!HALF_IMG || BM == 64, "HALF_IMG: 64-row tile of a 128-row image");
    constexpr bool PAIR = BM == 192;
    static_assert(!PAIR || (WM == 2 && TM == 3), "192-row tile: two wave rows of 96 rows");
    constexpr int IMG_ROWS = PAIR ? 96 : BM, IMG_BYTES = IMG_ROWS * 96, IMG_CHUNKS = IMG_BYTES / 1024;
    constexpr int A_KSTEP = HALF_IMG ? 2 * A_BYTES : IMG_BYTES, A_CHUNK_STRIDE = HALF_IMG ? 2048 : 1024;
    __shared__ __attribute__((aligned(16))) unsigned char smem[2 * STAGE];
    __shared__ __attribute__((aligned(16))) float braw[RAW ? 2 * BK * BN : 4];

    agpr_anchor();
    Wg w;
    if (!wg_tile<WN, BM>(d, MT, Gm, N, w)) return;
    const int nk = d.Kpad / BK;

    const unsigned char *aimg = reinterpret_cast<const unsigned char *>(d.wx) + (size_t)(HALF_IMG ? w.mt >> 1 : PAIR ? 2 * w.mt : w.mt) * nk * A_KSTEP +
                                (HALF_IMG ? (w.mt & 1) * 1024 : 0) + w.lane * 16;
#define MI_A_DMA(kt, stage)                                                                                         \
    do {                                                                                                            \
        _Pragma("unroll") for (int c = 0; c < (A_CHUNKS + 3) / 4; ++c) {                                             \
            const int chunk = c * 4 + w.wave, img = PAIR ? chunk / IMG_CHUNKS : 0, ic = chunk - img * IMG_CHUNKS;      \
            if (chunk < A_CHUNKS)                                                                                   \
                lds_dma16_tracked(aimg + ((size_t)img * nk + (kt)) * A_KSTEP + ic * A_CHUNK_STRIDE,                    \
                                  smem + (stage) * STAGE + chunk * 1024);                                          \
        }                                                                                                           \
    } while (0)

    const int bn = w.tid & 127;
    const int bh = __builtin_amdgcn_readfirstlane(w.tid >> 7);
    const ColInfo lc = decompose(w.n0 + bn, N, w.P, d.O2, PLAIN ? d.O2 : w.o2v);
    const int i1b = lc.o1 * d.S1, i2b = lc.o2 * d.S2;
    const float *xcol = d.x + (size_t)lc.b * d.x_bstride + (PLAIN ? (size_t)lc.p : (size_t)i1b * (d.x_ld ? d.x_ld : d.D2) + i2b);
    const float *bp = lc.valid ? xcol + (size_t)(8 * bh) * w.P : d.sink + MI_SINK_FLOATS;
    const size_t b_row = lc.valid ? (size_t)w.P : 0, b_step = lc.valid ? (size_t)BK * w.P : 0;
    float breg[8];
    BLoader<NT> L(d, w, N, w.P);
#define MI_BRAW_DMA(kt, rs) L.issue(d, (kt), braw + (rs) * (BK * BN) + (4 * w.wave) * BN)
#define MI_BRAW_FIX(kt, rs) L.fix(d, (kt), braw + (rs) * (BK * BN) + (4 * w.wave) * BN)
#define MI_BRAW_READ(rs)                                                                                            \
    do {                                                                                                            \
        _Pragma("unroll") for (int j = 0; j < 8; ++j) breg[j] = braw[(rs) * (BK * BN) + (8 * bh + j) * BN + bn];     \
    } while (0)

#define MI_B_LOAD(kt)                                                                                               \
    do {                                                                                                            \
        if (PLAIN) {                                                                                                \
            _Pragma("unroll") for (int j = 0; j < 8; ++j) breg[j] = bp[(size_t)(kt) * b_step + j * b_row];           \
        } else {                                                                                                    \
            mi_ktab_entry ke[8];                                                                                    \
            _Pragma("unroll") for (int j = 0; j < 8; ++j) ke[j] = d.ktab[(kt) * BK + 8 * bh + j];                    \
            _Pragma("unroll") for (int j = 0; j < 8; ++j) {                                                          \
                bool ok;                                                                                            \
                const float v = gather_b(d, ke[j], xcol, i1b, i2b, lc.valid, ok);                                   \
                breg[j] = ok ? v : 0.f;                                                                             \
            }                                                                                                       \
        }                                                                                                           \
    } while (0)

#define MI_B_STORE(stage)                                                                                           \
    do {                                                                                                            \
        unsigned ph[4], pm[4], pl[4];                                                                               \
        _Pragma("unroll") for (int j = 0; j < 4; ++j) split3(breg[2 * j], breg[2 * j + 1], ph[j], pm[j], pl[j]);    \
        unsigned char *bs = smem + (stage) * STAGE + A_BYTES + (bh * BN + bn) * 16;                                 \
        *reinterpret_cast<uint4 *>(bs) = make_uint4(ph[0], ph[1], ph[2], ph[3]);                                    \
        *reinterpret_cast<uint4 *>(bs + 2 * BN * 16) = make_uint4(pm[0], pm[1], pm[2], pm[3]);                      \
        *reinterpret_cast<uint4 *>(bs + 4 * BN * 16) = make_uint4(pl[0], pl[1], pl[2], pl[3]);                      \
    } while (0)

    f32x16 acc[TM][TN];
    zero_acc(acc);

    constexpr int PA[6] = {2, 0, 1, 1, 0, 0}, PB[6] = {0, 2, 1, 0, 1, 0};
    MI_A_DMA(0, 0);
    if constexpr (RAW) {
        L.prefetch(0);
        MI_BRAW_DMA(0, 0);
        if (nk > 1) {
            L.prefetch(1);
            MI_BRAW_DMA(1, 1);
        }
        if (nk > 2) L.prefetch(2);
        asm volatile("s_waitcnt vmcnt(0)" ::: "memory");
        MI_BRAW_FIX(0, 0);
        if (nk > 1) MI_BRAW_FIX(1, 1);
        __syncthreads();
        MI_BRAW_READ(0);
    } else {
        MI_B_LOAD(0);
    }
    MI_B_STORE(0);
    asm volatile("s_waitcnt vmcnt(0)" ::: "memory");
    __syncthreads();
    int cur = 0;
    for (int kt = 0; kt < nk; ++kt) {
        const unsigned char *As = smem + cur * STAGE, *Bs = As + A_BYTES;
        bf16x8 af[TM][3], bf[TN][3];
#pragma unroll
        for (int p = 0; p < 3; ++p) {
#pragma unroll
            for (int a = 0; a < TM; ++a)
                af[a][p] = *reinterpret_cast<const bf16x8 *>(As + (PAIR ? w.wm * IMG_BYTES : 0) +
                                                             (((p * 2 + w.lh) * IMG_ROWS) + ((PAIR ? 0 : w.wm * TM) + a) * 32 + w.li) * 16);
#pragma unroll
            for (int b = 0; b < TN; ++b)
                bf[b][p] = *reinterpret_cast<const bf16x8 *>(Bs + (((p * 2 + w.lh) * BN) + (w.wn * TN + b) * 32 + w.li) * 16);
        }
        __builtin_amdgcn_sched_barrier(0);
        if (kt + 1 < nk) {
            MI_A_DMA(kt + 1, cur ^ 1);
            if constexpr (RAW) {
                if (kt + 2 < nk) MI_BRAW_DMA(kt + 2, kt & 1);
            } else {
                MI_B_LOAD(kt + 1);
            }
        }
        if constexpr (RAW) {
            MI_BRAW_READ((kt + 1) & 1);
        }
        __builtin_amdgcn_sched_barrier(0);
#pragma unroll
        for (int q = 0; q < 6; ++q)
#pragma unroll
            for (int a = 0; a < TM; ++a)
#pragma unroll
                for (int b = 0; b < TN; ++b)
                    acc[a][b] = __builtin_amdgcn_mfma_f32_32x32x16_bf16(af[a][PA[q]], bf[b][PB[q]], acc[a][b], 0, 0, 0);
        if (RAW || kt + 1 < nk) MI_B_STORE(cur ^ 1);
        if constexpr (RAW) {
#pragma unroll
            for (int i = 0; i < 6 * TM * TN; ++i) {
                __builtin_amdgcn_sched_group_barrier(0x008, 1, 0);
                __builtin_amdgcn_sched_group_barrier(0x002, (72 + 6 * TM * TN - 1) / (6 * TM * TN), 0);
            }
        }
        if constexpr (ROWS) {
            if (kt + 3 < nk) L.template prefetch<true>(kt + 3);
            else asm volatile("s_waitcnt vmcnt(0)" ::: "memory");
        } else {
            asm volatile("s_waitcnt vmcnt(0)" ::: "memory");
        }
        if (kt + 2 < nk) MI_BRAW_FIX(kt + 2, kt & 1);
        __syncthreads();
        cur ^= 1;
    }
#undef MI_A_DMA
#undef MI_B_LOAD
#undef MI_BRAW_DMA
#undef MI_BRAW_FIX
#undef MI_BRAW_READ
#undef MI_B_STORE

    conv_epilogue<TM, TN, EPI, LFLAGS>(d, acc, w.m0, w.n0, w.wm, w.wn, N, w.P, w.o2v);
}

template <int WM, int WN, int TM, int TN, int EPI, int LFLAGS, bool PLAIN, bool HALF_IMG = false>
__global__ __launch_bounds__(256, 2) void conv_gemm_x6_kernel(const mi_conv_desc d, const int N, const int MT, const int Gm) {
    conv_x6_body<WM, WN, TM, TN, EPI, LFLAGS, PLAIN, HALF_IMG, 0>(d, N, MT, Gm);
}

template <int WM, int WN, int TM, int TN, bool HALF_IMG, int NT>
__global__ __launch_bounds__(256, 2) void conv_tap_x6_kernel(const mi_conv_desc d, const int N, const int MT, const int Gm) {
    conv_x6_body<WM, WN, TM, TN, MI_EPI_GLU, 0, false, HALF_IMG, NT>(d, N, MT, Gm);
}

template <int WM, int WN, int TM, int TN, int EPI, int LFLAGS, bool HALF_IMG>
__global__ __launch_bounds__(256, 2) void conv_rows_x6_kernel(const mi_conv_desc d, const int N, const int MT, const int Gm) {
    conv_x6_body<WM, WN, TM, TN, EPI, LFLAGS, false, HALF_IMG, kRowTaps>(d, N, MT, Gm);
}

template <int WM, int WN, int TM, int TN, int EPI, int LFLAGS, bool PLAIN, bool HALF_IMG = false, int NTAPS = 0>
static int launch_cfg_x6(const mi_conv_desc &d, hipStream_t st) {
    constexpr int BM = WM * TM * 32;
    ConvGeom g;
    MI_TRY(conv_geom(d, "conv", BM, HALF_IMG ? 2 * BM : BM, g));
    const int Gm = pick_m_groups(g.MT, (size_t)d.Kpad * d.Mpad * 6);
    if constexpr (NTAPS > 0) MI_LAUNCH_TILES((conv_tap_x6_kernel<WM, WN, TM, TN, HALF_IMG, NTAPS>), d, g, Gm, st);
    else if constexpr (NTAPS == kRowTaps) MI_LAUNCH_TILES((conv_rows_x6_kernel<WM, WN, TM, TN, EPI, LFLAGS, HALF_IMG>), d, g, Gm, st);
    else MI_LAUNCH_TILES((conv_gemm_x6_kernel<WM, WN, TM, TN, EPI, LFLAGS, PLAIN, HALF_IMG>), d, g, Gm, st);
    return MI_OK;
}

template <int EPI, int LFLAGS, bool PLAIN, int NTAPS>
static int launch_tile_x6(const mi_conv_desc &d, int tile, int image_tile, hipStream_t st) {
    if (tile != image_tile) {
        if constexpr (NTAPS != 0 || (PLAIN && EPI == MI_EPI_LINEAR)) {
            if (tile == 64 && image_tile == 128) return launch_cfg_x6<1, 4, 2, 1, EPI, LFLAGS, PLAIN, true, NTAPS>(d, st);
        }
        if constexpr (conv_x6_tile192(EPI, LFLAGS, PLAIN, NTAPS)) {
            if (tile == 192 && image_tile == 96) return launch_cfg_x6<2, 2, 3, 2, EPI, LFLAGS, PLAIN, false, NTAPS>(d, st);
        }
        return set_error(MI_EINVAL, "conv x6: no %d-row tile on a %d-row image for epilogue %d", tile, image_tile, EPI);
    }
    switch (tile) {
        case 128: return launch_cfg_x6<2, 2, 2, 2, EPI, LFLAGS, PLAIN, false, NTAPS>(d, st);
        case 96: return launch_cfg_x6<1, 4, 3, 1, EPI, LFLAGS, PLAIN, false, NTAPS>(d, st);
        case 64:
            if constexpr (NTAPS == 0) return launch_cfg_x6<1, 4, 2, 1, EPI, LFLAGS, PLAIN>(d, st);
    }
    return set_error(MI_EINVAL, "conv x6: unsupported tile_m %d", tile);
}

int launch_conv_tap_x6(const mi_conv_desc &d, int tile, int image_tile, hipStream_t st) {
    MI_REQUIRE(d.wx && ((uintptr_t)d.wx & 15) == 0, "conv tap x6: split weight image missing or misaligned");
    MI_REQUIRE(d.epi == MI_EPI_GLU && (image_tile == 96 || image_tile == 128) && (d.ntaps == 9 || d.ntaps == 3),
               "conv tap x6: GLU layer with 9 or 3 taps on a 96- or 128-row tile (epi %d, tile %d, ntaps %d)", d.epi, image_tile, d.ntaps);
    return d.ntaps == 9 ? launch_tile_x6<MI_EPI_GLU, 0, false, 9>(d, tile, image_tile, st) : launch_tile_x6<MI_EPI_GLU, 0, false, 3>(d, tile, image_tile, st);
}

int launch_conv_rows_x6(const mi_conv_desc &d, int tile, int image_tile, hipStream_t st) {
    MI_REQUIRE(d.wx && ((uintptr_t)d.wx & 15) == 0, "conv rows x6: split weight image missing or misaligned");
    MI_REQUIRE(d.ktab && ((uintptr_t)d.ktab & 63) == 0, "conv rows x6: gather table missing or misaligned");
    MI_REQUIRE(image_tile == 96 || image_tile == 128, "conv rows x6: 96- or 128-row tile (tile %d)", image_tile);
    if (d.epi == MI_EPI_CONVTR) return launch_tile_x6<MI_EPI_CONVTR, 0, false, kRowTaps>(d, tile, image_tile, st);
    if (d.epi == MI_EPI_GLU) {
        MI_REQUIRE(image_tile == 128 || d.tile_m == 192, "conv rows x6: GLU on a 128-row tile or a 192-row layer (tile %d)", image_tile);
        return launch_tile_x6<MI_EPI_GLU, 0, false, kRowTaps>(d, tile, image_tile, st);
    }
    MI_REQUIRE(d.epi == MI_EPI_LINEAR && (d.flags & (MI_FLAG_GELU | MI_FLAG_SCALE | MI_FLAG_RES | MI_FLAG_LN | MI_FLAG_STATS)) == MI_FLAG_GELU,
               "conv rows x6: LINEAR + GELU, CONVTR or GLU (epi %d, flags %d)", d.epi, d.flags);
    return launch_tile_x6<MI_EPI_LINEAR, MI_FLAG_GELU, false, kRowTaps>(d, tile, image_tile, st);
}

int launch_conv_x6(const mi_conv_desc &d, int tile, int image_tile, bool plain, hipStream_t st) {
    MI_REQUIRE(d.wx && ((uintptr_t)d.wx & 15) == 0, "conv x6: split weight image missing or misaligned");
    return dispatch_epilogue(d, [&](auto epi, auto lflags) {
        constexpr int E = decltype(epi)::value, F = decltype(lflags)::value;
        return plain ? launch_tile_x6<E, F, true, 0>(d, tile, image_tile, st) : launch_tile_x6<E, F, false, 0>(d, tile, image_tile, st);
    });
}

}
```

### demucs_amd/csrc/kernels.h

```cpp
#pragma once
#include <cmath>
#include <vector>
#include <hip/hip_runtime.h>
#include <stdint.h>

#include "gemm_conv.h"

namespace mi {

struct FftTables {
    const float *window;
    const float2 *twiddle;
    const float *envelope;
};
struct FftHostTables {
    std::vector<float> window, envelope;
    std::vector<float2> twiddle;
};
static inline FftHostTables fft_host_tables() {
    FftHostTables t{std::vector<float>(4096), std::vector<float>(1024), std::vector<float2>(2048)};
    for (int i = 0; i < 4096; ++i) t.window[i] = 0.5f - 0.5f * cosf((float)i * (float)(2.0 * M_PI / 4096.0));
    for (int r = 0; r < 1024; ++r) {
        float e = 0.f;
        for (int j = 3; j >= 0; --j) e += t.window[r + 1024 * j] * t.window[r + 1024 * j];
        t.envelope[r] = e;
    }
    for (int i = 0; i < 2048; ++i) { const double a = -2.0 * M_PI * i / 4096.0; t.twiddle[i] = make_float2((float)cos(a), (float)sin(a)); }
    return t;
}

int launch_stft_frames(const float *mix, int B, int L, const FftTables &tb, float *zt, double *stats, hipStream_t st);
int launch_cac_transpose(const float *zt, int B, int T, const float2 *norm, float *x, hipStream_t st, int x_pitch = 0 );
int launch_istft(const float *y, int B, int S, int L, const float2 *denorm, const float *xt, const float2 *denorm_t,
                 const FftTables &tb, float *yt, float *fr, float *out, hipStream_t st, int xt_pitch = 0 ,
                 int y_pitch = 0 );

extern int g_transpose_tiles;
extern int g_istft_fused;

int launch_row_stats(const float *x, int rows, int64_t count, int64_t row_stride, double *stats, hipStream_t st);
int launch_finalize_stats(double *stats, int rows, double count, float eps, int mode, float2 *out_a, float2 *out_b,
                          hipStream_t st);
int launch_row_affine(const float *x, int rows, int64_t count, const float2 *norm, float *y, hipStream_t st);
int launch_row_denorm(const float *x, int rows, int64_t count, const float2 *denorm, float *y, hipStream_t st);
int launch_layernorm_cf(const float *x, int B, int C, int T, const float *w, const float *b, const float *pe, float *y,
                        float2 *ostat, hipStream_t st, void *img = nullptr, int64_t img_n = 0, int img_dtype = 0);
int launch_token_stats(const float *x, int B, int C, int T, float2 *ostat, hipStream_t st, void *img = nullptr, int64_t img_n = 0,
                       int img_dtype = 0);
int launch_gn_apply_tokstats(const float *x, int B, int C, int T, const float2 *gstat, const float *w, const float *b, float *y,
                             float2 *ostat, hipStream_t st, void *img = nullptr, int64_t img_n = 0, int img_dtype = 0);

int gram_hp(int h);
int launch_gn_gelu_gram(float *x, int B, int h, int Cs, int D1, int D2 , int pitch, int row_mode, const float2 *stats, const float *w,
                        const float *b, double *gram , int slots, bool zero_pad, hipStream_t st);
int launch_gram_finalize(double *gram, int rows, int h, int slots, const double *wt , const double *ct , double sum_b,
                         double sum_bsq, double cols, double count, float eps, float2 *out, hipStream_t st);
int launch_gn_gelu(float *x, int B, int C, int Cs, int D1, int D2, int row_mode, const float2 *stats, const float *w, const float *b,
                   hipStream_t st);

struct DConvRowLayer {
    const float *w0;
    const float *b0;
    const float *g1w, *g1b;
    const float *w3;
    const float *b3, *g2w, *g2b;
    const float *ls;
};
struct DConvTimeLayer {
    DConvRowLayer w;
    const double *gram_a;
    const double *gram_v;
    const double *gram_c;
    const double *gram_e1, *gram_e2;
    double sum_b3, sum_b3sq;
};
struct DConvRowArgs {
    DConvTimeLayer l[2];
    const float *x;
    float *y;
    int Fr, T;
};
struct DConvHostPack {
    std::vector<float> w0, b0, g1w, g1b, w3;
    std::vector<double> gram_a, gram_v, gram_c, gram_e1, gram_e2;
    double sum_b3, sum_b3sq;
};
DConvHostPack dconv_pack_host(int C, int h, const float *w0, const float *b0, const float *g1w, const float *g1b, const float *w3,
                              const float *b3);
bool dconv_row_supported(int C, int T);
bool dconv_row_lds_supported(int C, int T);
int launch_dconv_row(const DConvRowArgs &a, int C, int rows, bool lds_row, hipStream_t st);

bool dconv_time_supported(int C, int Lp);
int launch_dconv_time_layer(const DConvTimeLayer &l, int C, int dil, int B, int Lv, int Lp, const float *x, float *y, float *hbuf,
                            double *stats, double *gram, float2 *st1, float2 *st2, hipStream_t st);

int launch_conv(const mi_conv_desc &d, hipStream_t st);

constexpr int BK = 16;
constexpr int BN = 128;
int conv_pick_tile(int M);
int conv_check_tile_m(const mi_conv_desc &d);
int conv_validate(const mi_conv_desc &d);
extern int g_split_bf16;
struct ConvRoute { int route; int tile; bool plain; bool mgroups; };
ConvRoute conv_route(const mi_conv_desc &d);
struct Switches {
    bool no_dma;
    bool no_dma_tap;
    bool no_dma_rows;
    bool no_dma_dconv;
    bool small_tile;
    bool mgroups;
    bool x6_plain_only;
    bool img256;
    bool half_tile256;
    int x6_scope;
    bool no_tap_image;
    bool no_enc_image;
    bool no_dconv_time;
    bool no_lin2_stats;
    bool no_ffn_image;
    bool no_qkv_heads;
    bool no_input_image;
    bool one_stream;
    bool debug_sync;
    int side_prio;
    bool h_no_deep_tap;
    bool h_no_last_tap;
    bool h_one_stream;
    bool lstm_steps;
    bool lstm_write_through;
    bool lstm_debug;
    int transpose_tiles;
    bool istft_split;
    bool dconv_row_lds;
};
const Switches &switches();
constexpr bool conv_x6_supported(int tile) { return tile == 128 || tile == 96 || tile == 64; }
constexpr int kRowTaps = -1;
constexpr bool conv_x6_tile192(int epi, int lflags, bool plain, int ntaps) {
    if (ntaps > 0) return epi == MI_EPI_GLU;
    if (ntaps == kRowTaps) return (epi == MI_EPI_LINEAR && lflags == MI_FLAG_GELU) || epi == MI_EPI_CONVTR || epi == MI_EPI_GLU;
    return plain && epi == MI_EPI_LINEAR && lflags == MI_FLAG_LN;
}
int launch_conv_x6(const mi_conv_desc &d, int tile, int image_tile, bool plain, hipStream_t st);
int launch_conv_tap_x6(const mi_conv_desc &d, int tile, int image_tile, hipStream_t st);
int launch_conv_rows_x6(const mi_conv_desc &d, int tile, int image_tile, hipStream_t st);
int launch_pack_split(const float *wt, int Kpad, int Mpad, int tile_m, void *wx, hipStream_t st);

int launch_conv_half(const mi_conv_desc &d, const ConvRoute &r, hipStream_t st);
int launch_pack_half(const float *wt, int Kpad, int Mpad, int dtype, void *wh, hipStream_t st);
int conv_tap_pairs_pad(int Cin, int ntaps);
int launch_pack_tap(const float *wt, int Mpad, int Cin, int ntaps, int dtype, void *out, hipStream_t st);
int launch_conv_tap(const mi_conv_desc &d, int tile, hipStream_t st);
int launch_f32_to_image(const float *x, int B, int C, int64_t P, int dtype, void *img, hipStream_t st);

int launch_row_affine_pitch(const float *x, int B, int C, int L, int out_pitch, const float2 *norm, float *y, hipStream_t st);
int launch_gn_apply(const float *x, int B, int Cin, int G, int in_pitch, int off, const float2 *stats, const float *w, const float *bias,
                    int glu, int gelu, const float *scale, const float *res, int res_pitch, float *y, int Cout, int out_len,
                    int out_pitch, hipStream_t st, int chan_div = 1);
int launch_unfold_frames(const float *x, int B, int C, int T, int F, int W, int S, float *fr, hipStream_t st);
int launch_restitch_frames(const float *fr, int B, int C, int T, int F, int W, int S, const float *skip, float *y, hipStream_t st);
void pack_lstm_whh(const float *whh , int H, float *packed);
int launch_lstm_seq(const float *gx, const float *whh , int N, int H, int W, float *out, float *state , hipStream_t st);
size_t lstm_persist_scratch_bytes();
size_t lstm_persist_ctl_offset();
int launch_lstm_persist(const float *gx, const float *whh , int N, int H, int W, float *out, void *scratch, unsigned *ctl_host,
                        hipStream_t st);
int launch_lstm_small(const float *gx, const float *whh_natural , int N, int H, int W, float *out, hipStream_t st);
int launch_local_attn(const float *qkc, int B, int C, int T, int ld , float *out, int ld_o, hipStream_t st);

int launch_attention(const float *q, const float *k, const float *v, float *o, int B, int heads, int Tq, int Tk, int64_t q_bs,
                     int64_t kv_bs, int64_t o_bs, int dtype, hipStream_t st, void *oh = nullptr, int64_t oh_n = 0);
int launch_attention_x6(const float *q, const float *k, const float *v, float *o, int B, int heads, int Tq, int Tk, int64_t q_bs,
                        int64_t kv_bs, int64_t o_bs, hipStream_t st);

int launch_segments_gather(const float *track, int64_t track_len, int channels, const int64_t *starts_dev, int B, int valid,
                           float *seg, hipStream_t st);
int launch_ola_accumulate(float *acc, int64_t acc_len, int rows, const float *model_out, int valid, const int64_t *offs_dev,
                          const int32_t *lens_dev, const int32_t *trim_dev, int B, int64_t span_lo, int64_t span_hi,
                          const float *weight, int weight_len, hipStream_t st);
int launch_ola_finish(float *acc, int64_t acc_len, int rows, int64_t acc_off0, const int64_t *offs_dev, const int32_t *lens_dev,
                      int n_segments, int max_len, const float *weight, hipStream_t st);

int launch_segments_gather_packed(const float *tracks, int64_t tracks_cap, int channels, const int64_t *items_dev, int B, int valid,
                                  float *seg, hipStream_t st);
int launch_ola_accumulate_packed(float *acc, int64_t acc_cap, int rows, const float *model_out, int valid, const int64_t *items_dev,
                                 int B, const int64_t *tiles_dev, int n_tiles, const float *weights, int64_t weights_cap,
                                 hipStream_t st);
int launch_ola_finish_packed(float *acc, int64_t acc_cap, int rows, const int64_t *tiles_dev, int n_tiles, const int64_t *segs_dev,
                             int n_segs, const float *weights, int64_t weights_cap, hipStream_t st);

int launch_resample_frac(const float *x, int rows, int64_t L, const float *table, int old_sr, int new_sr, int width, float *y,
                         int64_t Lout, hipStream_t st);

int launch_streams_convert_append(float *win, int64_t win_cap, int channels, const int64_t *table, int n_streams, int64_t max_groups,
                                  const float *bank, int64_t bank_cap, float *hist, int64_t hist_cap, const float *stats, int n_stats,
                                  int lds_floats, hipStream_t st);
int launch_streams_convert_append_pcm(float *win, int64_t win_cap, int channels, const int64_t *table, int n_streams,
                                      int64_t max_groups, const float *bank, int64_t bank_cap, float *hist, int64_t hist_cap,
                                      const float *stats, int n_stats, int lds_floats, hipStream_t st);

int launch_pcm_planar(const unsigned char *src, int fmt, int src_ch, int64_t n, int channels, const float *stats, float *dst,
                      hipStream_t st);
int launch_streams_append_pcm(float *win, int64_t win_cap, int channels, const int64_t *table, int n_streams, int64_t max_bytes,
                              const float *stats, int n_stats, hipStream_t st);

int mono_stats_state_bytes();
int launch_mono_stats_update(const unsigned char *src, int fmt, int src_ch, int64_t n, int channels, int64_t before, double *state,
                             hipStream_t st);
int launch_mono_stats_finish(const double *state, int64_t length, double *scratch, float *stats, hipStream_t st);

int64_t sdr_state_bytes(int n_sources);
int64_t sdr_scratch_bytes(int n_sources);
int launch_sdr_update(const void *const *refs, int fmt, int src_ch, int64_t ref_stride, const float *est, int64_t est_stride, int n_sources,
                      int channels, int64_t n, int64_t before, double *state, hipStream_t st);
int launch_sdr_finish(const double *state, int n_sources, double *scratch, double *sums, hipStream_t st);
int launch_sdr(const float *ref, const float *est, int B, int n_sources, int channels, int64_t length, double *state, double *scratch,
               double *sums, hipStream_t st);

const void *conv_zero_page();
int launch_attention_heads(const void *q, const void *k, const void *v, const void *zero_page, int B, int heads, int Tq, int Tk, int Tq_pitch,
                           int Tk_pitch, int dtype, void *oh, int64_t oh_n, float *o, int64_t o_bs, hipStream_t st);

int post_stats_scratch_bytes();
int launch_mono_stats(const float *wav, int channels, int64_t length, double *scratch, float *stats, hipStream_t st);
int launch_mono_stats_final(const double *scratch, int64_t length, float *stats, hipStream_t st);
int launch_stream_emit(const float *acc, int64_t acc_cap, int n_sources, int channels, const int64_t *passes, int n_passes,
                       const int64_t *segs, int n_segs, const float *weights, int64_t weights_cap, const float *scales, int n_members,
                       int shifts, int bag, const float *stats, int64_t n, float *out, hipStream_t st);
int launch_streams_emit(const float *acc, int64_t acc_cap, int n_sources, int channels, const int64_t *streams, int n_streams, int64_t max_n,
                        const int64_t *passes, int n_passes, const int64_t *segs, int n_segs, const float *weights, int64_t weights_cap,
                        const float *scales, int n_members, int shifts, int bag, const float *stats, int n_stats, float *out,
                        int64_t out_cap, hipStream_t st);
int launch_streams_append(float *win, int64_t win_cap, int channels, const int64_t *table, int n_streams, int64_t max_n,
                          const float *stats, int n_stats, hipStream_t st);
int launch_streams_compact(float *dst, int64_t dst_cap, const float *src, int64_t src_cap, const int64_t *table, int n_rows, int64_t max_len,
                           hipStream_t st);
int launch_track_affine(float *x, int64_t n, const float *stats, int mode, hipStream_t st);
int launch_prevent_clip(const float *x, int64_t n, int mode, unsigned *peak, float *y, hipStream_t st);
int launch_two_stems(const float *const *stems, int S, int sel, const float *origin, int mode, int64_t n, float *y, hipStream_t st);

int launch_deliver_peaks(const int64_t *table, int n_rows, int64_t max_n, int n_sources, int channels, unsigned *peaks, int n_peaks,
                         int64_t dst_cap, hipStream_t st);
int launch_deliver_pcm(const int64_t *table, int n_rows, int64_t max_n, int n_sources, int channels, const unsigned *peaks, int n_peaks,
                       unsigned char *dst, int64_t dst_cap, hipStream_t st);

int launch_deliver_resample_pcm(const int64_t *table, int n_rows, int64_t max_groups, int n_sources, int channels, const float *bank,
                                int64_t bank_cap, float *hist, int64_t hist_cap, int lds_floats, unsigned char *dst, int64_t dst_cap,
                                hipStream_t st);

}
```

### demucs_amd/csrc/model.hip

```cpp
#include <cmath>
#include <map>
#include <memory>
#include <mutex>
#include <string>
#include <vector>

#include "model.h"

namespace mi {

int Model::attn(const float *q, const float *k, const float *v, float *o, int B, int Tq, int Tk, int64_t q_bs, int64_t kv_bs,
                int64_t o_bs, hipStream_t st, bool image) {
    void *oh = image ? (void *)o : nullptr;
    const int64_t oh_n = (int64_t)B * Tq;
    const bool x6 = cfg.dtype == MI_DTYPE_F32 && !image && g_split_bf16 && switches().x6_scope != 0;
    auto launch = [&]() {
        return x6 ? launch_attention_x6(q, k, v, o, B, 8, Tq, Tk, q_bs, kv_bs, o_bs, st)
                  : launch_attention(q, k, v, o, B, 8, Tq, Tk, q_bs, kv_bs, o_bs, cfg.dtype, st, oh, oh_n);
    };
    const int cls = x6 ? 104 : 100;
    const char *name = x6 ? "attention_x6_kernel" : cfg.dtype == MI_DTYPE_BF16 ? "attention_bf16_kernel" : cfg.dtype == MI_DTYPE_F16 ? "attention_f16_kernel" : "attention_kernel";
    return prof.timed(cls, name, 4.0 * B * 8 * (double)Tq * Tk * 64.0, 4.0 * B * 512.0 * (2.0 * Tq + 2.0 * Tk), st, launch);
}

int Model::attn_heads(const void *q, const void *k, const void *v, float *o, int B, int Tq, int Tk, hipStream_t st) {
    const int64_t oh_n = (int64_t)B * Tq;
    const void *zero = conv_zero_page();
    MI_REQUIRE(zero, "attention: could not allocate the zero page");
    return prof.timed(100, cfg.dtype == MI_DTYPE_BF16 ? "attention_heads_bf16_kernel" : "attention_heads_f16_kernel",
                      4.0 * B * 8 * (double)Tq * Tk * 64.0, 2.0 * B * 512.0 * (2.0 * Tq + 2.0 * Tk), st,
                      [&] { return launch_attention_heads(q, k, v, zero, B, 8, Tq, Tk, Tq, Tk, cfg.dtype, o, oh_n, nullptr, 0, st); });
}

static const int kFr[5] = {2048, 512, 128, 32, 8};
static const int kCh[4] = {48, 96, 192, 384};

int Model::init(const mi_config &c, const mi_tensor_desc *weights, size_t n) {
    cfg = c;
    MI_REQUIRE(c.n_sources >= 1 && c.n_sources <= 8, "n_sources %d unsupported", c.n_sources);
    MI_REQUIRE(c.max_batch >= 1 && c.max_batch <= 64, "max_batch %d out of range [1, 64]", c.max_batch);
    MI_REQUIRE(c.dtype == MI_DTYPE_F32 || c.dtype == MI_DTYPE_BF16 || c.dtype == MI_DTYPE_F16, "unknown compute dtype %d", c.dtype);
    MI_REQUIRE(c.segment_length > 4096 && c.segment_length % 4 == 0, "segment_length %d unsupported", c.segment_length);
    S = c.n_sources; SL = c.segment_length; T = (SL + 1023) / 1024;
    MI_REQUIRE(T % 4 == 0, "segment_length %d gives %d STFT frames; the engine needs a multiple of 4", SL, T);
    Lt[0] = SL;
    for (int i = 0; i < 4; ++i) Lt[i + 1] = (Lt[i] + 3) / 4;
    for (int i = 0; i < 5; ++i) Lp[i] = round_up(Lt[i], 4);
    MI_REQUIRE(Lt[4] % 4 == 0, "time branch bottleneck length %d must be a multiple of 4", Lt[4]);
    WeightTable wt;
    for (size_t i = 0; i < n; ++i) wt.t[weights[i].name] = {weights[i].data, weights[i].numel};

    MI_TRY(upload_fft_tables());

    for (int i = 0; i < 4; ++i) {
        const int Cin = i ? kCh[i - 1] : 4, C = kCh[i];
        const std::string p = "encoder." + std::to_string(i);
        const float *w, *b, *rw, *rb;
        MI_TRY(wt.get(p + ".conv.weight", (int64_t)C * Cin * 8, &w));
        MI_TRY(wt.get(p + ".conv.bias", C, &b));
        MI_TRY(wt.get(p + ".rewrite.weight", (int64_t)2 * C * C, &rw));
        MI_TRY(wt.get(p + ".rewrite.bias", 2 * C, &rb));
        EncW &e = enc[i];
        MI_TRY(pack_conv(w, b, C, Cin * 8, false, &e.conv, 0, i > 0 ? SPLIT_ROWS : SPLIT_OPT_IN));
        if (i) MI_TRY(pack_enc_tap(w, Cin, &e.conv));
        MI_TRY(make_ktab(Gather{Cin, 8, 1, 1, 1, 2, 0, (int64_t)kFr[i] * T, T}, e.conv.Kpad, &e.ktab_conv));
        MI_TRY(pack_conv(rw, rb, 2 * C, C, true, &e.rewrite, 0, i >= 2 ? SPLIT_ROWS : SPLIT_OPT_IN));
        MI_TRY(make_ktab(Gather{C, 1, 1, 1, 1, 0, 0, (int64_t)kFr[i + 1] * T, T}, e.rewrite.Kpad, &e.ktab_rw));
        MI_TRY(load_dconv(wt, p, C, (int64_t)kFr[i + 1] * T, T, true, &e.dconv));

        const int Cint = i ? kCh[i - 1] : 2;
        const std::string pt = "tencoder." + std::to_string(i);
        MI_TRY(wt.get(pt + ".conv.weight", (int64_t)C * Cint * 8, &w));
        MI_TRY(wt.get(pt + ".conv.bias", C, &b));
        MI_TRY(wt.get(pt + ".rewrite.weight", (int64_t)2 * C * C, &rw));
        MI_TRY(wt.get(pt + ".rewrite.bias", 2 * C, &rb));
        EncW &te = tenc[i];
        MI_TRY(pack_conv(w, b, C, Cint * 8, false, &te.conv));
        if (i) MI_TRY(pack_enc_tap(w, Cint, &te.conv));
        MI_TRY(make_ktab(Gather{Cint, 1, 8, 1, 1, 0, 2, (int64_t)Lp[i], Lp[i]}, te.conv.Kpad, &te.ktab_conv));
        MI_TRY(pack_conv(rw, rb, 2 * C, C, true, &te.rewrite, 0, i >= 2 ? SPLIT_ROWS : SPLIT_OPT_IN));
        MI_TRY(make_ktab(Gather{C, 1, 1, 1, 1, 0, 0, (int64_t)Lp[i + 1], Lp[i + 1]}, te.rewrite.Kpad, &te.ktab_rw));
        MI_TRY(load_dconv(wt, pt, C, (int64_t)Lp[i + 1], Lp[i + 1], false, &te.dconv));
    }
    {
        const float *ew;
        MI_TRY(wt.get("freq_emb.embedding.weight", 512 * 48, &ew));
        std::vector<float> emb(48 * 512);
        for (int f = 0; f < 512; ++f)
            for (int ch = 0; ch < 48; ++ch) emb[ch * 512 + f] = 0.2f * (ew[f * 48 + ch] * 10.0f);
        MI_TRY(upload(emb, &freq_emb));
    }
    for (int j = 0; j < 4; ++j) {
        const int C = kCh[3 - j], Fr = kFr[4 - j];
        const int Cout = j < 3 ? kCh[2 - j] : 4 * S, Coutt = j < 3 ? kCh[2 - j] : 2 * S;
        const std::string p = "decoder." + std::to_string(j);
        const float *w, *b, *rw, *rb;
        MI_TRY(wt.get(p + ".conv_tr.weight", (int64_t)C * Cout * 8, &w));
        MI_TRY(wt.get(p + ".conv_tr.bias", Cout, &b));
        MI_TRY(wt.get(p + ".rewrite.weight", (int64_t)2 * C * C * 9, &rw));
        MI_TRY(wt.get(p + ".rewrite.bias", 2 * C, &rb));
        DecW &dd = dec[j];
        MI_TRY(pack_conv(rw, rb, 2 * C, C * 9, true, &dd.rewrite, 9, SPLIT_DEFAULT));
        MI_TRY(make_ktab(Gather{C, 3, 3, 1, 1, 1, 1, (int64_t)Fr * T, T}, dd.rewrite.Kpad, &dd.ktab_rw));
        MI_TRY(load_dconv(wt, p, C, (int64_t)Fr * T, T, true, &dd.dconv));
        MI_TRY(pack_convtr(w, b, C, Cout, &dd.convtr, 4, j < 3 ? SPLIT_ROWS : SPLIT_OPT_IN));
        MI_TRY(make_ktab(Gather{C, 2, 1, -1, 1, 0, 0, (int64_t)Fr * T, T}, dd.convtr.Kpad, &dd.ktab_tr));

        const int L = Lp[4 - j];
        const std::string pt = "tdecoder." + std::to_string(j);
        MI_TRY(wt.get(pt + ".conv_tr.weight", (int64_t)C * Coutt * 8, &w));
        MI_TRY(wt.get(pt + ".conv_tr.bias", Coutt, &b));
        MI_TRY(wt.get(pt + ".rewrite.weight", (int64_t)2 * C * C * 3, &rw));
        MI_TRY(wt.get(pt + ".rewrite.bias", 2 * C, &rb));
        DecW &td = tdec[j];
        MI_TRY(pack_conv(rw, rb, 2 * C, C * 3, true, &td.rewrite, 3, SPLIT_DEFAULT));
        MI_TRY(make_ktab(Gather{C, 1, 3, 1, 1, 0, 1, (int64_t)L, L}, td.rewrite.Kpad, &td.ktab_rw));
        MI_TRY(load_dconv(wt, pt, C, (int64_t)L, L, false, &td.dconv));
        MI_TRY(pack_convtr(w, b, C, Coutt, &td.convtr));
        MI_TRY(make_ktab(Gather{C, 1, 2, 1, -1, 0, 0, (int64_t)L, L}, td.convtr.Kpad, &td.ktab_tr));
    }
    const int Tf = 8 * T, Tt = Lt[4];
    {
        const char *names[4] = {"channel_upsampler", "channel_upsampler_t", "channel_downsampler", "channel_downsampler_t"};
        for (int i = 0; i < 4; ++i) {
            const int M = i < 2 ? 512 : 384, K = i < 2 ? 384 : 512, P = (i & 1) ? Tt : Tf;
            const float *w, *b;
            MI_TRY(wt.get(std::string(names[i]) + ".weight", (int64_t)M * K, &w));
            MI_TRY(wt.get(std::string(names[i]) + ".bias", M, &b));
            MI_TRY(pack_conv(w, b, M, K, false, &chan[i]));
            MI_TRY(make_ktab(Gather{K, 1, 1, 1, 1, 0, 0, (int64_t)P, P}, chan[i].Kpad, &chan_ktab[i]));
        }
        for (int br = 0; br < 2; ++br) {
            const int P = br ? Tt : Tf;
            MI_TRY(make_ktab(Gather{512, 1, 1, 1, 1, 0, 0, (int64_t)P, P}, 512, &tr_ktab512[br]));
            MI_TRY(make_ktab(Gather{2048, 1, 1, 1, 1, 0, 0, (int64_t)P, P}, 2048, &tr_ktab2048[br]));
        }
    }
    for (int br = 0; br < 2; ++br) {
        const std::string ni = br ? "crosstransformer.norm_in_t" : "crosstransformer.norm_in";
        const float *w, *b;
        MI_TRY(wt.get(ni + ".weight", 512, &w)); MI_TRY(wt.get(ni + ".bias", 512, &b));
        MI_TRY(pack_vec(w, 512, 512, false, &norm_in_w[br])); MI_TRY(pack_vec(b, 512, 512, false, &norm_in_b[br]));
        for (int k = 0; k < 5; ++k) {
            const std::string p = std::string("crosstransformer.") + (br ? "layers_t." : "layers.") + std::to_string(k);
            const bool cross = k & 1;
            const std::string at = p + (cross ? ".cross_attn" : ".self_attn");
            TrLayerW &l = tr[br][k];
            const float *ipw, *ipb, *ow, *ob, *w1, *b1, *w2, *b2;
            MI_TRY(wt.get(at + ".in_proj_weight", 1536 * 512, &ipw));
            MI_TRY(wt.get(at + ".in_proj_bias", 1536, &ipb));
            MI_TRY(wt.get(at + ".out_proj.weight", 512 * 512, &ow));
            MI_TRY(wt.get(at + ".out_proj.bias", 512, &ob));
            MI_TRY(wt.get(p + ".linear1.weight", 2048 * 512, &w1)); MI_TRY(wt.get(p + ".linear1.bias", 2048, &b1));
            MI_TRY(wt.get(p + ".linear2.weight", 512 * 2048, &w2)); MI_TRY(wt.get(p + ".linear2.bias", 512, &b2));
            const float *nw[4] = {}, *nb[4] = {};
            const char *nn[4] = {".norm1", ".norm2", ".norm3", ".norm_out"};
            for (int q = 0; q < 4; ++q) {
                if (q == 2 && !cross) continue;
                MI_TRY(wt.get(p + nn[q] + ".weight", 512, &nw[q])); MI_TRY(wt.get(p + nn[q] + ".bias", 512, &nb[q]));
            }
            MI_TRY(pack_vec(nw[3], 512, 512, false, &l.norm_w[3])); MI_TRY(pack_vec(nb[3], 512, 512, false, &l.norm_b[3]));
            if (cross) {
                MI_TRY(pack_linear_ln(ipw, ipb, nw[0], nb[0], 512, 512, &l.q_proj, &l.q_c1, SPLIT_DEFAULT));
                MI_TRY(pack_linear_ln(ipw + 512 * 512, ipb + 512, nw[1], nb[1], 1024, 512, &l.kv_proj, &l.kv_c1, SPLIT_DEFAULT));
                MI_TRY(pack_linear_ln(w1, b1, nw[2], nb[2], 2048, 512, &l.lin1, &l.lin1_c1, SPLIT_DEFAULT));
            } else {
                MI_TRY(pack_linear_ln(ipw, ipb, nw[0], nb[0], 1536, 512, &l.qkv_proj, &l.qkv_c1, SPLIT_DEFAULT));
                MI_TRY(pack_linear_ln(w1, b1, nw[1], nb[1], 2048, 512, &l.lin1, &l.lin1_c1, SPLIT_DEFAULT));
            }
            MI_TRY(pack_conv(ow, ob, 512, 512, false, &l.out_proj, 0, SPLIT_DEFAULT));
            MI_TRY(pack_conv(w2, b2, 512, 2048, false, &l.lin2, 0, SPLIT_DEFAULT));
            MI_TRY(wt.get(p + ".gamma_1.scale", 512, &w)); MI_TRY(pack_vec(w, 512, 512, false, &l.gamma1));
            MI_TRY(wt.get(p + ".gamma_2.scale", 512, &w)); MI_TRY(pack_vec(w, 512, 512, false, &l.gamma2));
        }
    }
    {
        std::vector<float> pe2((size_t)512 * Tf), pe1((size_t)512 * Tt);
        for (int i = 0; i < 128; ++i) {
            const float div = expf((float)(2 * i) * (float)(-(log(10000.0) / 256.0)));
            for (int fr = 0; fr < 8; ++fr)
                for (int t1 = 0; t1 < T; ++t1) {
                    const size_t tok = (size_t)fr * T + t1;
                    pe2[(size_t)(2 * i) * Tf + tok] = sinf((float)t1 * div);
                    pe2[(size_t)(2 * i + 1) * Tf + tok] = cosf((float)t1 * div);
                    pe2[(size_t)(256 + 2 * i) * Tf + tok] = sinf((float)fr * div);
                    pe2[(size_t)(256 + 2 * i + 1) * Tf + tok] = cosf((float)fr * div);
                }
        }
        for (int i = 0; i < 256; ++i) {
            const float den = powf(10000.0f, (float)i / 255.0f);
            for (int t2 = 0; t2 < Tt; ++t2) {
                const float ph = (float)t2 / den;
                pe1[(size_t)i * Tt + t2] = cosf(ph);
                pe1[(size_t)(256 + i) * Tt + t2] = sinf(ph);
            }
        }
        MI_TRY(upload(pe2, &pos_emb[0])); MI_TRY(upload(pe1, &pos_emb[1]));
    }
    MI_TRY(alloc_workspace());
    {
        const Switches &sw = switches();
        const bool half = cfg.dtype != MI_DTYPE_F32;
        plan.ffn_img = half && !sw.no_ffn_image;
        plan.qkv_heads = plan.ffn_img && !sw.no_qkv_heads;
        plan.in_img = plan.qkv_heads && !sw.no_input_image;
        plan.lin2_stats = !sw.no_lin2_stats;
        plan.tap_img = half && dec[0].rewrite.wtap && tdec[0].rewrite.wtap;
        for (int i = 1; i < 4; ++i) {
            plan.enc_img[0][i] = enc[i].conv.wtap && w_eimg[0][i - 1];
            plan.enc_img[1][i] = tenc[i].conv.wtap && w_eimg[1][i - 1];
        }
    }
    MI_HIP(hipDeviceSynchronize());
    return MI_OK;
}

static std::mutex g_ws_mutex;
static std::map<std::string, std::weak_ptr<Workspace>> g_ws;

int Model::alloc_workspace() {
    int dev = 0;
    MI_HIP(hipGetDevice(&dev));
    char key[128];
    snprintf(key, sizeof(key), "htdemucs dev%d S%d SL%d B%d %s", dev, S, SL, cfg.max_batch, cfg.dtype == MI_DTYPE_F32 ? "f32" : "half");
    std::lock_guard<std::mutex> lock(g_ws_mutex);
    auto it = g_ws.find(key);
    if (it != g_ws.end()) ws = it->second.lock();
    if (!ws) {
        auto w = std::make_shared<Workspace>();
        w->key = key;
        MI_TRY(fill_workspace(*w));
        g_ws[key] = w;
        ws = w;
    }
    static_cast<WorkspacePtrs &>(*this) = *ws;
    dconv_gram = w_gram; dconv_gram2 = w_gram2; dconv_gram2_bytes = gram2_bytes;
    dconv_tap_dma = true;
    return MI_OK;
}

int Model::fill_workspace(Workspace &w) {
    const size_t B = cfg.max_batch;
    auto A = [&](float **p, size_t per_item) { return w.mem.alloc((void **)p, per_item * B * sizeof(float)); };
    auto dev_alloc = [&](void **p, size_t n) { return w.mem.alloc(p, n); };
    MI_TRY(A(&w.w_xt0, (size_t)2 * SL));
    MI_TRY(A(&w.w_zt, (size_t)4 * 2048 * T));
    MI_TRY(A(&w.w_x0, (size_t)4 * 2048 * T));
    size_t big = 0;
    for (int i = 0; i < 4; ++i) {
        const size_t nf = (size_t)kCh[i] * kFr[i + 1] * T, nt = (size_t)kCh[i] * Lp[i + 1];
        MI_TRY(A(&w.w_skip[i], nf)); MI_TRY(A(&w.w_skip_t[i], nt));
        big = std::max(big, std::max(nf, nt));
    }
    if (cfg.dtype != MI_DTYPE_F32)
        for (int i = 0; i < 3; ++i) {
            const size_t pqf = (size_t)(kFr[i + 1] / 4 + 1) * T, pqt = round_up(ceil_div(Lt[i + 1], 4) + 1, 4);
            float *pf = nullptr, *pt = nullptr;
            MI_TRY(A(&pf, 2 * kCh[i] * pqf)); MI_TRY(A(&pt, 2 * kCh[i] * pqt));
            MI_HIP(hipMemset(pf, 0, 2 * kCh[i] * pqf * B * sizeof(float)));
            MI_HIP(hipMemset(pt, 0, 2 * kCh[i] * pqt * B * sizeof(float)));
            w.w_eimg[0][i] = pf; w.w_eimg[1][i] = pt;
        }
    MI_TRY(A(&w.w_h, big / 2)); MI_TRY(A(&w.w_th, big / 2));
    for (float **p : {&w.w_a, &w.w_b, &w.w_ta, &w.w_tb, &w.w_c, &w.w_tc}) {
        MI_TRY(w.mem.alloc((void **)p, (big * B + 64) * sizeof(float)));
        *p += 32;
    }
    MI_HIP(hipMemset(w.w_h, 0, (big / 2) * B * sizeof(float)));
    MI_HIP(hipMemset(w.w_th, 0, (big / 2) * B * sizeof(float)));
    const size_t Tf = 8 * (size_t)T, Tt = Lt[4];
    for (int br = 0; br < 2; ++br) {
        const size_t P = br ? Tt : Tf;
        MI_TRY(A(&w.w_tr_x[br][0], 512 * P)); MI_TRY(A(&w.w_tr_x[br][1], 512 * P));
        if (cfg.dtype != MI_DTYPE_F32) {
            MI_TRY(A(&w.w_tr_ximg[br][0], 256 * P)); MI_TRY(A(&w.w_tr_ximg[br][1], 256 * P)); MI_TRY(A(&w.w_tr_x1img[br], 256 * P));
        }
        for (int q = 0; q < 2; ++q) MI_TRY(dev_alloc((void **)&w.w_tr_stat[br][q], B * P * sizeof(float2)));
        MI_TRY(dev_alloc((void **)&w.w_tr_stat1[br], B * P * sizeof(float2)));
        MI_TRY(A(&w.w_tr_qkv[br], 1536 * Tf)) ; MI_TRY(A(&w.w_tr_att[br], 512 * P));
        MI_TRY(A(&w.w_tr_x1[br], 512 * P)); MI_TRY(A(&w.w_tr_x2[br], 512 * P)); MI_TRY(A(&w.w_tr_ffh[br], 2048 * P));
    }
    MI_TRY(A(&w.w_yspec, (size_t)4 * S * 2048 * T));
    MI_TRY(A(&w.w_ytime, (size_t)2 * S * SL));
    MI_TRY(A(&w.w_yt, (size_t)4 * S * 2048 * T));
    MI_TRY(A(&w.w_fr, (size_t)S * T * 2 * 4096));
    const size_t max_rows = B * 512;
    w.stats_bytes = max_rows * kStatSlots * 2 * sizeof(double);
    MI_TRY(dev_alloc((void **)&w.w_stats, w.stats_bytes));
    MI_TRY(dev_alloc((void **)&w.w_stats_t, w.stats_bytes));
    w.gram_bytes = B * kStatSlots * 96 * sizeof(double);
    MI_TRY(dev_alloc((void **)&w.w_gram, w.gram_bytes));
    MI_HIP(hipMemset(w.w_gram, 0, w.gram_bytes));
    w.gram2_bytes = B * ((size_t)4 << 20);
    MI_TRY(dev_alloc((void **)&w.w_gram2, w.gram2_bytes));
    MI_HIP(hipMemset(w.w_gram2, 0, w.gram2_bytes));
    w.gram2t_bytes = B * ((size_t)1 << 20);
    MI_TRY(dev_alloc((void **)&w.w_gram2_t, w.gram2t_bytes));
    MI_HIP(hipMemset(w.w_gram2_t, 0, w.gram2t_bytes));
    MI_HIP(hipMemset(w.w_stats, 0, w.stats_bytes));
    MI_HIP(hipMemset(w.w_stats_t, 0, w.stats_bytes));
    MI_TRY(dev_alloc((void **)&w.w_st1, max_rows * sizeof(float2)));
    MI_TRY(dev_alloc((void **)&w.w_st2, max_rows * sizeof(float2)));
    MI_TRY(dev_alloc((void **)&w.w_st1_t, max_rows * sizeof(float2)));
    MI_TRY(dev_alloc((void **)&w.w_st2_t, max_rows * sizeof(float2)));
    MI_TRY(dev_alloc((void **)&w.w_norm_f, B * sizeof(float2))); MI_TRY(dev_alloc((void **)&w.w_denorm_f, B * sizeof(float2)));
    MI_TRY(dev_alloc((void **)&w.w_norm_t, B * sizeof(float2))); MI_TRY(dev_alloc((void **)&w.w_denorm_t, B * sizeof(float2)));
    return MI_OK;
}

#define MI_STAGE(name)                                                                        \
    do {                                                                                      \
        if (switches().debug_sync) {                                                          \
            hipError_t _e = hipStreamSynchronize(st);                                         \
            fprintf(stderr, "[mi] reached %s (%s)\n", name, hipGetErrorString(_e));          \
            fflush(stderr);                                                                   \
            if (_e != hipSuccess) return set_error(MI_EHIP, "stage before %s failed: %s", name, hipGetErrorString(_e)); \
        }                                                                                     \
    } while (0)

int Model::run_tr_layer(int br, int k, int B, const float *x, const float2 *xstat, const float *other, const float2 *ostat,
                        float *out, float2 *outstat, hipStream_t st, const void *ximg, const void *oimg, void *outimg) {
    const TrLayerW &l = tr[br][k];
    const bool cross = k & 1;
    const int Tf = 8 * T, Tt = Lt[4];
    const int Tq = br ? Tt : Tf, Tk = cross ? (br ? Tf : Tt) : Tq;
    const Geo gq{B, 1, Tq, 0}, gk{B, 1, Tk, 0};
    float *qkv = w_tr_qkv[br], *att = w_tr_att[br], *x1 = w_tr_x1[br], *x2 = w_tr_x2[br], *ffh = w_tr_ffh[br];
    double *stats = br ? w_stats_t : w_stats;
    float2 *st1 = br ? w_st1_t : w_st1;
    const bool img = plan.ffn_img, heads = plan.qkv_heads, in_img = plan.in_img, lin2_stats = plan.lin2_stats;
    unsigned short *qh = reinterpret_cast<unsigned short *>(qkv);
    const size_t plane_q = (size_t)B * 512 * Tq, plane_k = (size_t)B * 512 * Tk;
    if (!cross) {
        mi_conv_desc d = base_desc(l.qkv_proj, tr_ktab512[br], x, (int64_t)512 * Tq, gq);
        d.plain = 1; d.epi = MI_EPI_LINEAR; d.flags = MI_FLAG_LN; d.scale = l.qkv_c1; d.pro_stats = (const float *)xstat;
        d.y = qkv; d.y_bstride = (int64_t)1536 * Tq; d.y_cstride = Tq;
        if (heads) { d.flags |= MI_FLAG_HEADS; d.yh = qh; d.yh_n = Tq; }
        if (in_img) { d.xh = ximg; d.xh_n = (int64_t)B * Tq; }
        MI_TRY(conv(d, st));
        if (heads) MI_TRY(attn_heads(qh, qh + plane_q, qh + 2 * plane_q, att, B, Tq, Tq, st));
        else MI_TRY(attn(qkv, qkv + (size_t)512 * Tq, qkv + (size_t)1024 * Tq, att, B, Tq, Tq, (int64_t)1536 * Tq, (int64_t)1536 * Tq,
                         (int64_t)512 * Tq, st, img));
    } else {
        mi_conv_desc d = base_desc(l.q_proj, tr_ktab512[br], x, (int64_t)512 * Tq, gq);
        d.plain = 1; d.epi = MI_EPI_LINEAR; d.flags = MI_FLAG_LN; d.scale = l.q_c1; d.pro_stats = (const float *)xstat;
        d.y = qkv; d.y_bstride = (int64_t)512 * Tq; d.y_cstride = Tq;
        if (heads) { d.flags |= MI_FLAG_HEADS; d.yh = qh; d.yh_n = Tq; }
        if (in_img) { d.xh = ximg; d.xh_n = (int64_t)B * Tq; }
        MI_TRY(conv(d, st));
        float *kv = qkv + (size_t)B * 512 * Tq;
        unsigned short *kvh = qh + plane_q;
        mi_conv_desc e = base_desc(l.kv_proj, tr_ktab512[1 - br], other, (int64_t)512 * Tk, gk);
        e.plain = 1; e.epi = MI_EPI_LINEAR; e.flags = MI_FLAG_LN; e.scale = l.kv_c1; e.pro_stats = (const float *)ostat;
        e.y = kv; e.y_bstride = (int64_t)1024 * Tk; e.y_cstride = Tk;
        if (heads) { e.flags |= MI_FLAG_HEADS; e.yh = kvh; e.yh_n = Tk; }
        if (in_img) { e.xh = oimg; e.xh_n = (int64_t)B * Tk; }
        MI_TRY(conv(e, st));
        if (heads) MI_TRY(attn_heads(qh, kvh, kvh + plane_k, att, B, Tq, Tk, st));
        else MI_TRY(attn(qkv, kv, kv + (size_t)512 * Tk, att, B, Tq, Tk, (int64_t)512 * Tq, (int64_t)1024 * Tk, (int64_t)512 * Tq, st, img));
    }
    {
        mi_conv_desc d = base_desc(l.out_proj, tr_ktab512[br], att, (int64_t)512 * Tq, gq);
        d.plain = 1; d.epi = MI_EPI_LINEAR; d.flags = MI_FLAG_SCALE | MI_FLAG_RES; d.scale = l.gamma1; d.res = x;
        d.y = x1; d.y_bstride = (int64_t)512 * Tq; d.y_cstride = Tq;
        if (img) { d.xh = att; d.xh_n = (int64_t)B * Tq; }
        MI_TRY(conv(d, st));
    }
    MI_TRY(launch_token_stats(x1, B, 512, Tq, w_tr_stat1[br], st, in_img ? w_tr_x1img[br] : nullptr, (int64_t)B * Tq, cfg.dtype));
    {
        mi_conv_desc d = base_desc(l.lin1, tr_ktab512[br], x1, (int64_t)512 * Tq, gq);
        d.plain = 1; d.epi = MI_EPI_LINEAR; d.flags = MI_FLAG_LN | MI_FLAG_GELU; d.scale = l.lin1_c1;
        d.pro_stats = (const float *)w_tr_stat1[br];
        d.y = ffh; d.y_bstride = (int64_t)2048 * Tq; d.y_cstride = Tq;
        if (img) { d.flags |= MI_FLAG_IMG; d.yh = ffh; d.yh_n = (int64_t)B * Tq; }
        if (in_img) { d.xh = w_tr_x1img[br]; d.xh_n = (int64_t)B * Tq; }
        MI_TRY(conv(d, st));
        mi_conv_desc e = base_desc(l.lin2, tr_ktab2048[br], ffh, (int64_t)2048 * Tq, gq);
        if (img) { e.xh = ffh; e.xh_n = (int64_t)B * Tq; }
        e.plain = 1; e.epi = MI_EPI_LINEAR; e.flags = MI_FLAG_SCALE | MI_FLAG_RES; e.scale = l.gamma2; e.res = x1;
        if (lin2_stats) { e.flags |= MI_FLAG_STATS; e.stats = stats; }
        e.y = x2; e.y_bstride = (int64_t)512 * Tq; e.y_cstride = Tq;
        MI_TRY(conv(e, st));
    }
    if (!lin2_stats) MI_TRY(launch_row_stats(x2, B, (int64_t)512 * Tq, (int64_t)512 * Tq, stats, st));
    MI_TRY(launch_finalize_stats(stats, B, (double)512 * Tq, 1e-5f, 0, st1, nullptr, st));
    MI_TRY(launch_gn_apply_tokstats(x2, B, 512, Tq, st1, l.norm_w[3], l.norm_b[3], out, outstat, st, in_img ? outimg : nullptr,
                                    (int64_t)B * Tq, cfg.dtype));
    return MI_OK;
}

int Model::run_core(const float *mix, const float *mag, int B, hipStream_t st) {
    if (ws->dirty) {
        MI_HIP(hipMemsetAsync(w_stats, 0, ws->stats_bytes, st));
        MI_HIP(hipMemsetAsync(w_stats_t, 0, ws->stats_bytes, st));
        MI_HIP(hipMemsetAsync(w_gram, 0, ws->gram_bytes, st));
        MI_HIP(hipMemsetAsync(w_gram2, 0, gram2_bytes, st));
        MI_HIP(hipMemsetAsync(w_gram2_t, 0, gram2t_bytes, st));
        ws->dirty = false;
    }
    const int r = run_core_impl(mix, mag, B, st);
    if (r != MI_OK) {
        ws->dirty = true;
        if (side_st) (void)hipStreamSynchronize(side_st);
    }
    return r;
}

int Model::forward(const float *mix, float *out, int B, hipStream_t st) {
    MI_REQUIRE(mix && out, "forward: null buffer");
    MI_TRY(run_core(mix, nullptr, B, st));
    MI_TRY(launch_istft(w_yspec, B, S, SL, w_denorm_f, w_ytime, w_denorm_t, fft, w_yt, w_fr, out, st));
    MI_STAGE("istft done");
    return MI_OK;
}

int Model::forward_core(const float *mix, const float *mag, float *spec_out, float *time_out, int B, hipStream_t st) {
    MI_REQUIRE(mix && spec_out && time_out, "forward_core: null buffer");
    MI_TRY(run_core(mix, mag, B, st));
    MI_TRY(launch_row_denorm(w_yspec, B, (int64_t)4 * S * 2048 * T, w_denorm_f, spec_out, st));
    MI_TRY(launch_row_denorm(w_ytime, B, (int64_t)2 * S * SL, w_denorm_t, time_out, st));
    return MI_OK;
}

int Model::run_core_impl(const float *mix, const float *mag, int B, hipStream_t st) {
    MI_REQUIRE(B >= 1 && B <= cfg.max_batch, "forward: batch %d outside [1, %d]", B, cfg.max_batch);
    const int Tf = 8 * T, Tt = Lt[4];
    const bool two = !switches().one_stream && g_two_streams && !switches().debug_sync && side_streams() == MI_OK;
    hipStream_t stt = two ? side_st : st;
    auto fork = [&]() -> int {
        if (!two) return MI_OK;
        MI_HIP(hipEventRecord(ev_main, st));
        MI_HIP(hipStreamWaitEvent(side_st, ev_main, 0));
        return MI_OK;
    };
    auto join = [&]() -> int {
        if (!two) return MI_OK;
        MI_HIP(hipEventRecord(ev_side, side_st));
        MI_HIP(hipStreamWaitEvent(st, ev_side, 0));
        return MI_OK;
    };
    MI_TRY(fork());
    MI_TRY(launch_row_stats(mix, B, (int64_t)2 * SL, (int64_t)2 * SL, w_stats_t, stt));
    MI_TRY(launch_finalize_stats(w_stats_t, B, 2.0 * SL, 1e-5f, 1, w_norm_t, w_denorm_t, stt));
    MI_TRY(launch_row_affine(mix, B, (int64_t)2 * SL, w_norm_t, w_xt0, stt));
    MI_STAGE("time normalisation done");
    if (mag) {
        const int64_t cnt = (int64_t)4 * 2048 * T;
        MI_TRY(launch_row_stats(mag, B, cnt, cnt, w_stats, st));
        MI_TRY(launch_finalize_stats(w_stats, B, (double)cnt, 1e-5f, 1, w_norm_f, w_denorm_f, st));
        MI_TRY(launch_row_affine(mag, B, cnt, w_norm_f, w_x0, st));
    } else {
        MI_TRY(launch_stft_frames(mix, B, SL, fft, w_zt, w_stats, st));
        MI_TRY(launch_finalize_stats(w_stats, B, 4.0 * 2048 * T, 1e-5f, 1, w_norm_f, w_denorm_f, st));
        MI_TRY(launch_cac_transpose(w_zt, B, T, w_norm_f, w_x0, st));
    }
    MI_STAGE("stft done");

    const float *xf = w_x0, *xt = w_xt0;
    for (int i = 0; i < 4; ++i) {
        const int Cin = i ? kCh[i - 1] : 4, Cint = i ? kCh[i - 1] : 2, C = kCh[i];
        {
            const Geo gin{B, kFr[i], T, 1}, go{B, kFr[i + 1], T, 1};
            const int64_t Pin = (int64_t)kFr[i] * T, P = (int64_t)kFr[i + 1] * T;
            mi_conv_desc d = base_desc(enc[i].conv, enc[i].ktab_conv, xf, Cin * Pin, gin);
            d.O1 = kFr[i + 1]; d.S1 = 4; d.epi = MI_EPI_LINEAR; d.flags = MI_FLAG_GELU;
            d.y = w_a; d.y_bstride = C * P; d.y_cstride = P;
            d.dma_rows = 1;
            if (plan.enc_img[0][i]) {
                const int Q = kFr[i] / 4 + 1;
                d.xh = w_eimg[0][i - 1]; d.xh_n = (int64_t)cfg.max_batch * Q * T; d.wtap = enc[i].conv.wtap; d.ntaps = 2; d.tap_k2 = 1;
                d.D1 = Q; d.S1 = 1;
            }
            MI_TRY(conv(d, st));
            MI_STAGE("enc conv done");
            MI_TRY(run_dconv(enc[i].dconv, C, go, w_a, w_b, w_h, w_stats, w_st1, w_st2, st));
            MI_STAGE("enc dconv done");
            mi_conv_desc r = base_desc(enc[i].rewrite, enc[i].ktab_rw, w_a, C * P, go);
            r.plain = 1; r.epi = MI_EPI_GLU; r.y = w_skip[i]; r.y_bstride = C * P; r.y_cstride = P;
            if (i == 0) { r.flags = MI_FLAG_EMB; r.emb = freq_emb; }
            if (i < 3 && plan.enc_img[0][i + 1]) {
                const int64_t pq = (int64_t)(kFr[i + 1] / 4 + 1) * T;
                r.flags |= MI_FLAG_IMG4 | MI_FLAG_TR_FREQ; r.yh = w_eimg[0][i]; r.yh_pq = pq; r.yh_n = (int64_t)cfg.max_batch * pq;
            }
            MI_TRY(conv(r, st));
            xf = w_skip[i];
            MI_STAGE("enc rewrite done");
        }
        {
            const Geo gin{B, 1, Lt[i], 0, Lp[i]}, go{B, 1, Lt[i + 1], 0, Lp[i + 1]};
            const int64_t P = Lp[i + 1];
            mi_conv_desc d = base_desc(tenc[i].conv, tenc[i].ktab_conv, xt, (int64_t)Cint * Lp[i], gin);
            d.O2 = Lp[i + 1]; d.o2_valid = Lt[i + 1]; d.S2 = 4; d.epi = MI_EPI_LINEAR; d.flags = MI_FLAG_GELU;
            d.y = w_ta; d.y_bstride = C * P; d.y_cstride = P;
            if (plan.enc_img[1][i]) {
                const int Qp = round_up(ceil_div(Lt[i], 4) + 1, 4);
                d.xh = w_eimg[1][i - 1]; d.xh_n = (int64_t)cfg.max_batch * Qp; d.wtap = tenc[i].conv.wtap; d.ntaps = 2; d.tap_k2 = 2;
                d.D2 = Qp; d.x_ld = Qp; d.S2 = 1;
            }
            MI_TRY(conv(d, stt));
            MI_TRY(run_dconv(tenc[i].dconv, C, go, w_ta, w_tb, w_th, w_stats_t, w_st1_t, w_st2_t, stt, w_gram2_t, gram2t_bytes));
            mi_conv_desc r = base_desc(tenc[i].rewrite, tenc[i].ktab_rw, w_ta, C * P, go);
            r.plain = 1; r.epi = MI_EPI_GLU; r.y = w_skip_t[i]; r.y_bstride = C * P; r.y_cstride = P;
            if (i < 3 && plan.enc_img[1][i + 1]) {
                const int64_t pq = round_up(ceil_div(Lt[i + 1], 4) + 1, 4);
                r.flags |= MI_FLAG_IMG4; r.yh = w_eimg[1][i]; r.yh_pq = pq; r.yh_n = (int64_t)cfg.max_batch * pq;
            }
            MI_TRY(conv(r, stt));
            xt = w_skip_t[i];
            MI_STAGE("tenc layer done");
        }
    }
    int cur[2] = {0, 0};
    const bool in_img = plan.in_img;
    for (int br = 0; br < 2; ++br) {
        const int P = br ? Tt : Tf;
        const Geo g{B, 1, P, 0};
        hipStream_t sb = br ? stt : st;
        mi_conv_desc d = base_desc(chan[br], chan_ktab[br], br ? xt : xf, (int64_t)384 * P, g);
        d.plain = 1; d.epi = MI_EPI_LINEAR; d.y = w_tr_x1[br]; d.y_bstride = (int64_t)512 * P; d.y_cstride = P;
        MI_TRY(conv(d, sb));
        MI_TRY(launch_layernorm_cf(w_tr_x1[br], B, 512, P, norm_in_w[br], norm_in_b[br], pos_emb[br], w_tr_x[br][0],
                                   w_tr_stat[br][0], sb, in_img ? w_tr_ximg[br][0] : nullptr, (int64_t)B * P, cfg.dtype));
    }
    MI_STAGE("upsample + norm_in done");
    for (int k = 0; k < 5; ++k) {
        const float *f_in = w_tr_x[0][cur[0]], *t_in = w_tr_x[1][cur[1]];
        const float2 *f_st = w_tr_stat[0][cur[0]], *t_st = w_tr_stat[1][cur[1]];
        const void *f_img = in_img ? w_tr_ximg[0][cur[0]] : nullptr, *t_img = in_img ? w_tr_ximg[1][cur[1]] : nullptr;
        MI_TRY(join());
        MI_TRY(fork());
        MI_TRY(run_tr_layer(0, k, B, f_in, f_st, t_in, t_st, w_tr_x[0][cur[0] ^ 1], w_tr_stat[0][cur[0] ^ 1], st, f_img, t_img,
                            w_tr_ximg[0][cur[0] ^ 1]));
        MI_TRY(run_tr_layer(1, k, B, t_in, t_st, f_in, f_st, w_tr_x[1][cur[1] ^ 1], w_tr_stat[1][cur[1] ^ 1], stt, t_img, f_img,
                            w_tr_ximg[1][cur[1] ^ 1]));
        cur[0] ^= 1; cur[1] ^= 1;
        MI_STAGE("transformer layer done");
    }
    float *din = w_c, *dtin = w_tc;
    const bool tapimg = plan.tap_img;
    for (int br = 0; br < 2; ++br) {
        const int P = br ? Tt : Tf;
        const Geo g{B, 1, P, 0};
        mi_conv_desc d = base_desc(chan[2 + br], chan_ktab[2 + br], w_tr_x[br][cur[br]], (int64_t)512 * P, g);
        d.plain = 1; d.epi = MI_EPI_LINEAR; d.flags = MI_FLAG_RES; d.res = br ? w_skip_t[3] : w_skip[3];
        d.y = br ? dtin : din; d.y_bstride = (int64_t)384 * P; d.y_cstride = P;
        if (tapimg) { d.flags |= MI_FLAG_IMG; d.yh = br ? dtin : din; d.yh_n = (int64_t)B * P; }
        MI_TRY(conv(d, br ? stt : st));
    }
    for (int j = 0; j < 4; ++j) {
        const int C = kCh[3 - j], Fr = kFr[4 - j];
        const bool last = j == 3;
        {
            const Geo g{B, Fr, T, 1};
            const int64_t P = (int64_t)Fr * T;
            mi_conv_desc r = base_desc(dec[j].rewrite, dec[j].ktab_rw, din, C * P, g);
            r.epi = MI_EPI_GLU; r.y = w_a; r.y_bstride = C * P; r.y_cstride = P;
            r.ntaps = 9; r.tap_k2 = 3; r.tap_pad1 = 1; r.tap_pad2 = 1;
            if (tapimg) { r.xh = din; r.xh_n = (int64_t)B * P; r.wtap = dec[j].rewrite.wtap; }
            MI_TRY(conv(r, st));
            MI_TRY(run_dconv(dec[j].dconv, C, g, w_a, w_b, w_h, w_stats, w_st1, w_st2, st));
            const int Cout = last ? 4 * S : kCh[2 - j];
            mi_conv_desc t = base_desc(dec[j].convtr, dec[j].ktab_tr, w_a, C * P, g);
            t.O1 = Fr + 1; t.epi = MI_EPI_CONVTR; t.flags = MI_FLAG_TR_FREQ; t.out_len = 4 * Fr;
            t.y_cstride = (int64_t)4 * Fr * T; t.y_bstride = Cout * t.y_cstride;
            t.dma_rows = 1;
            if (last) t.y = w_yspec;
            else { t.flags |= MI_FLAG_GELU | MI_FLAG_RES; t.res = w_skip[2 - j]; t.y = din; }
            if (!last && tapimg) { t.flags |= MI_FLAG_IMG; t.yh = din; t.yh_n = (int64_t)B * t.y_cstride; }
            if (tapimg && dec[j].convtr.wtap && !last) {
                MI_TRY(launch_f32_to_image(w_a, B, C, P, cfg.dtype, w_b, st));
                t.xh = w_b; t.xh_n = (int64_t)B * P; t.wtap = dec[j].convtr.wtap; t.ntaps = 2; t.tap_k2 = 1; t.tap_dil1 = -1;
            }
            MI_TRY(conv(t, st));
            MI_STAGE("dec freq layer done");
        }
        {
            const int Lv = Lt[4 - j], L = Lp[4 - j], Lout = Lt[3 - j], Lpo = Lp[3 - j];
            const Geo g{B, 1, Lv, 0, L};
            mi_conv_desc r = base_desc(tdec[j].rewrite, tdec[j].ktab_rw, dtin, (int64_t)C * L, g);
            r.epi = MI_EPI_GLU; r.y = w_ta; r.y_bstride = (int64_t)C * L; r.y_cstride = L;
            r.ntaps = 3; r.tap_k2 = 3; r.tap_pad1 = 0; r.tap_pad2 = 1;
            if (tapimg) { r.xh = dtin; r.xh_n = (int64_t)B * L; r.wtap = tdec[j].rewrite.wtap; }
            MI_TRY(conv(r, stt));
            MI_TRY(run_dconv(tdec[j].dconv, C, g, w_ta, w_tb, w_th, w_stats_t, w_st1_t, w_st2_t, stt, w_gram2_t, gram2t_bytes));
            const int Cout = last ? 2 * S : kCh[2 - j];
            mi_conv_desc t = base_desc(tdec[j].convtr, tdec[j].ktab_tr, w_ta, (int64_t)C * L, g);
            t.O2 = Lv + 1; t.o2_valid = 0; t.epi = MI_EPI_CONVTR; t.out_len = Lout;
            t.y_cstride = Lpo; t.y_bstride = (int64_t)Cout * Lpo;
            if (last) t.y = w_ytime;
            else { t.flags |= MI_FLAG_GELU | MI_FLAG_RES; t.res = w_skip_t[2 - j]; t.y = dtin; }
            if (!last && tapimg) { t.flags |= MI_FLAG_IMG; t.yh = dtin; t.yh_n = (int64_t)B * t.y_cstride; }
            if (tapimg && tdec[j].convtr.wtap && !last) {
                MI_TRY(launch_f32_to_image(w_ta, B, C, L, cfg.dtype, w_tb, stt));
                t.xh = w_tb; t.xh_n = (int64_t)B * L; t.wtap = tdec[j].convtr.wtap; t.ntaps = 2; t.tap_k2 = 2; t.tap_dil2 = -1;
            }
            MI_TRY(conv(t, stt));
        }
    }
    MI_TRY(join());
    MI_STAGE("decoders done");
    return MI_OK;
}

}
```

### include/demucs_amd.h

```cpp
#ifndef DEMUCS_AMD_H
#define DEMUCS_AMD_H

#include <stddef.h>
#include <stdint.h>

#ifdef __cplusplus
extern "C" {
#endif

#define MI_OK 0
#define MI_EINVAL (-1)
#define MI_EHIP (-2)
#define MI_ENOMEM (-3)
#define MI_EWEIGHT (-4)

typedef struct mi_tensor_desc {
    const char *name;
    const float *data;
    int64_t numel;
} mi_tensor_desc;

typedef struct mi_config {
    int32_t n_sources;
    int32_t segment_length;
// ... 183 lines not shown
int64_t mi_sdr_state_bytes(int32_t n_sources);
int64_t mi_sdr_scratch_bytes(int32_t n_sources);
int mi_sdr_update(const void *const *refs, int32_t fmt, int32_t src_ch, int64_t ref_stride, const float *est_dev, int64_t est_stride,
                  int32_t n_sources, int32_t channels, int64_t n, int64_t before, void *state_dev, void *stream);
int mi_sdr_finish(const void *state_dev, int32_t n_sources, void *scratch_dev, double *sums_dev, void *stream);
int mi_sdr(const float *ref_dev, const float *est_dev, int32_t B, int32_t n_sources, int32_t channels, int64_t length, void *state_dev,
           void *scratch_dev, double *sums_dev, void *stream);

#define MI_CLIP_RESCALE 1
#define MI_CLIP_CLAMP 2
#define MI_CLIP_TANH 3
int mi_prevent_clip(const float *x_dev, int64_t numel, int32_t mode, void *peak_dev, float *y_dev, void *stream);
int mi_two_stems(const float *const *stems_dev, int32_t n_stems, int32_t selected, const float *origin_dev, int32_t minus, int64_t numel,
                 float *y_dev, void *stream);

#define MI_DELIVER_SRC 0
#define MI_DELIVER_ORIGIN 1
#define MI_DELIVER_N 2
#define MI_DELIVER_KIND 3
#define MI_DELIVER_SEL 4
#define MI_DELIVER_CLIP 5
#define MI_DELIVER_PEAK 6
#define MI_DELIVER_FMT 7
#define MI_DELIVER_DST_OFF 8
#define MI_DELIVER_COLS 9
#define MI_DELIVER_STEM 0
#define MI_DELIVER_ADD 1
#define MI_DELIVER_MINUS 2
#define MI_DELIVER_I16 0
#define MI_DELIVER_F32 1
int mi_deliver_peaks(const int64_t *table_dev, int32_t n_rows, int64_t max_n, int32_t n_sources, int32_t channels, void *peaks_dev,
                     int32_t n_peaks, int64_t dst_capacity, void *stream);
int mi_deliver_pcm(const int64_t *table_dev, int32_t n_rows, int64_t max_n, int32_t n_sources, int32_t channels, const void *peaks_dev,
                   int32_t n_peaks, void *dst_dev, int64_t dst_capacity, void *stream);

#define MI_RATE_SRC 0
#define MI_RATE_N_IN 1
#define MI_RATE_BEFORE 2
#define MI_RATE_KIND 3
#define MI_RATE_SEL 4
#define MI_RATE_CLIP 5
#define MI_RATE_FMT 6
#define MI_RATE_OLD 7
#define MI_RATE_NEW 8
#define MI_RATE_WIDTH 9
#define MI_RATE_BANK_OFF 10
#define MI_RATE_OUT0 11
#define MI_RATE_N_OUT 12
#define MI_RATE_TOTAL 13
#define MI_RATE_HIST_LEN 14
#define MI_RATE_HIST_RD 15
#define MI_RATE_HIST_WR 16
#define MI_RATE_HIST_START 17
#define MI_RATE_HIST_NEXT 18
#define MI_RATE_DST_OFF 19
#define MI_RATE_COLS 20
#define MI_RATE_LDS_FLOATS 16384
int mi_deliver_resample_pcm(const int64_t *table_dev, int32_t n_rows, int64_t max_groups, int32_t n_sources, int32_t channels,
                            const float *bank_dev, int64_t bank_capacity, float *hist_dev, int64_t hist_capacity, int32_t lds_floats,
                            void *dst_dev, int64_t dst_capacity, void *stream);

int mi_stft_cac(const float *mix_dev, int32_t B, int32_t L, float *cac_dev, void *stream);
int mi_istft_cac(const float *x_dev, int32_t B, int32_t S, int32_t L, float *wav_dev, void *stream);

int mi_stft_norm(const float *mix_dev, int32_t B, int32_t L, float *x_dev, int32_t x_pitch, float *norm_dev, float *denorm_dev, void *stream);
int mi_istft_full(const float *y_dev, int32_t B, int32_t S, int32_t L, int32_t y_pitch, const float *denorm_f_dev, const float *xt_dev,
                  int32_t xt_pitch, const float *denorm_t_dev, float *wav_dev, void *stream);
int mi_item_norm(const float *x_dev, int32_t rows, int64_t count, float *y_dev, float *norm_dev, float *denorm_dev, void *stream);
int mi_item_denorm(const float *x_dev, int32_t rows, int64_t count, const float *denorm_dev, float *y_dev, void *stream);

struct mi_conv_desc;
int mi_conv_forward(const struct mi_conv_desc *desc, void *stream);

int mi_conv_pack_split(const float *wt_dev, int32_t Kpad, int32_t Mpad, int32_t tile_m, void *wx_dev, void *stream);

int mi_conv_pack_tap(const float *wt_dev, int32_t Mpad, int32_t Cin, int32_t ntaps, int32_t dtype, void *wtap_dev, void *stream);
int mi_f32_to_image(const float *x_dev, int32_t B, int32_t C, int64_t P, int32_t dtype, void *img_dev, void *stream);

int mi_conv_pack_half(const float *wt_dev, int32_t Kpad, int32_t Mpad, int32_t dtype, void *wh_dev, void *stream);

int mi_attention(const float *q_dev, const float *k_dev, const float *v_dev, float *o_dev, int32_t B, int32_t heads,
                 int32_t Tq, int32_t Tk, int64_t q_batch_stride, int64_t kv_batch_stride, int64_t o_batch_stride,
                 int32_t dtype, void *stream);

int mi_attention_split(const float *q_dev, const float *k_dev, const float *v_dev, float *o_dev, int32_t B, int32_t heads,
                       int32_t Tq, int32_t Tk, int64_t q_batch_stride, int64_t kv_batch_stride, int64_t o_batch_stride,
                       void *stream);

int mi_attention_heads(const void *q_dev, const void *k_dev, const void *v_dev, float *o_dev, int32_t B, int32_t heads, int32_t Tq, int32_t Tk,
                       int32_t Tq_pitch, int32_t Tk_pitch, int32_t dtype, void *stream);

int mi_attention_heads_image(const void *q_dev, const void *k_dev, const void *v_dev, void *img_dev, int64_t n_img, int32_t B, int32_t heads,
                             int32_t Tq, int32_t Tk, int32_t Tq_pitch, int32_t Tk_pitch, int32_t dtype, void *stream);

int mi_attention_image(const float *q_dev, const float *k_dev, const float *v_dev, void *img_dev, int64_t n_img, int32_t B,
                       int32_t heads, int32_t Tq, int32_t Tk, int64_t q_batch_stride, int64_t kv_batch_stride, int32_t dtype,
                       void *stream);

int mi_gn_gelu(float *x_dev, int32_t B, int32_t C, int32_t C_alloc, int32_t D1, int32_t D2, int32_t row_mode, const float *stats_dev,
               const float *w_dev, const float *b_dev, void *stream);

int32_t mi_gram_order(int32_t h);
int mi_gn_gelu_gram(float *x_dev, int32_t B, int32_t h, int32_t C_alloc, int32_t D1, int32_t D2, int32_t pitch, int32_t row_mode,
                    const float *stats_dev, const float *w_dev, const float *b_dev, double *gram_dev, int32_t slots, void *stream);
int mi_dconv_gn_gelu_gram(float *x_dev, int32_t B, int32_t h, int32_t C_alloc, int32_t D1, int32_t D2, int32_t pitch, int32_t row_mode,
                          const float *stats_dev, const float *w_dev, const float *b_dev, double *gram_dev, int32_t slots, void *stream);
int mi_gram_finalize(double *gram_dev, int32_t rows, int32_t h, int32_t slots, const double *wt_dev, const double *ct_dev, double sum_b,
                     double sum_bsq, double cols, double count, float eps, float *stats_out_dev, void *stream);

int mi_lstm_seq(const float *gx_dev, const float *whh_host, int32_t N, int32_t H, int32_t W, float *out_dev, int32_t mode, void *stream);

int mi_layernorm_cf(const float *x_dev, int32_t B, int32_t C, int32_t T, const float *w_dev, const float *b_dev,
                    const float *add_dev, float *y_dev, void *stream);


int mi_token_norm(int32_t mode, const float *x_dev, int32_t B, int32_t C, int32_t T, const float *w_dev, const float *b_dev,
                  const float *pe_dev, const float *gstat_dev, float *y_dev, float *ostat_dev, void *img_dev, int64_t img_n,
                  int32_t img_dtype, void *stream);

int mi_local_attn(const float *qkc_dev, int32_t B, int32_t C, int32_t T, int32_t ld, float *out_dev, int32_t ld_o, void *stream);

int mi_group_norm_apply(const float *x_dev, int32_t B, int32_t Cin, int32_t G, int32_t in_pitch, int32_t in_len, int32_t off,
                        const float *w_dev, const float *b_dev, int32_t glu, int32_t gelu, const float *scale_dev, const float *res_dev,
                        int32_t res_pitch, float *y_dev, int32_t Cout, int32_t out_len, int32_t out_pitch, int32_t chan_div,
                        double *stats_ws_dev, float *stats_out_dev, void *stream);

int mi_blstm_unfold(const float *x_dev, int32_t B, int32_t C, int32_t T, int32_t F, int32_t W, int32_t S, float *frames_dev, void *stream);
int mi_blstm_restitch(const float *frames_dev, int32_t B, int32_t C, int32_t T, int32_t F, int32_t W, int32_t S, const float *skip_dev,
                      float *y_dev, void *stream);

int mi_row_affine_pitch(const float *x_dev, int32_t B, int32_t C, int32_t L, int32_t out_pitch, const float *norm_dev, float *y_dev,
                        void *stream);


int mi_dconv_row(const float *x_dev, float *y_dev, int32_t B, int32_t C, int32_t Fr, int32_t T, const float *weights_host, int32_t variant,
                 void *stream);

int mi_dconv_time_layer(const float *x_dev, float *y_dev, int32_t B, int32_t C, int32_t Lv, int32_t Lp, int32_t dil,
                        const float *weights_host, float *hbuf_dev, double *stats_dev, double *gram_dev, float *st_dev, void *stream);

void mi_debug_set_post_launch_hook(void (*hook)(void *stream));

enum mi_conv_route {
    MI_ROUTE_TABLE = 0,
    MI_ROUTE_DMA = 1,
    MI_ROUTE_DMATAP = 2,
    MI_ROUTE_DMAROW = 3,
    MI_ROUTE_X6 = 4,
    MI_ROUTE_HALF = 5,
    MI_ROUTE_TAP_HALF = 6,
    MI_ROUTE_TAP_X6 = 7,
    MI_ROUTE_ROWS_X6 = 8,
    MI_ROUTE_HALF_IMG = 9,
    MI_ROUTE_HALF_IMG256 = 10
};

int mi_debug_last_conv_route(void);

int mi_debug_last_conv_tile(void);

int mi_debug_conv_route(const struct mi_conv_desc *desc, int *tile);

int mi_debug_switches(char *buf, int32_t n);

const char *mi_last_error(void);
const char *mi_version(void);

#ifdef __cplusplus
}
#endif
#endif
```

Before: 2406.

## Add time-axis direct-DMA x6 conv route for time encoder and transposed decoder convs

```diff
diff --git a/demucs_amd/_lib.py b/demucs_amd/_lib.py
--- a/demucs_amd/_lib.py
+++ b/demucs_amd/_lib.py
@@ -43,6 +43,7 @@
         ("wtap", C.c_void_p), ("ntaps", C.c_int32), ("tap_k2", C.c_int32), ("tap_pad1", C.c_int32), ("tap_pad2", C.c_int32),
         ("tap_dil1", C.c_int32), ("tap_dil2", C.c_int32), ("yh_pq", C.c_int64),
         ("dma_rows", C.c_int32), ("dma_rows_pad", C.c_int32),
+        ("dma_time", C.c_int32), ("dma_time_pad", C.c_int32),
     ]
 
 
@@ -165,6 +166,7 @@
     "mi_debug_set_post_launch_hook": (None, [C.c_void_p]),
     "mi_debug_last_conv_route": (C.c_int, []),
     "mi_debug_last_conv_tile": (C.c_int, []),
+    "mi_debug_conv_route_launches": (C.c_int64, [C.c_int32, C.c_int32]),
     "mi_debug_conv_route": (C.c_int, [C.POINTER(MiConvDesc), C.POINTER(C.c_int)]),
     "mi_debug_switches": (C.c_int, [C.c_char_p, C.c_int32]),
     "mi_last_error": (C.c_char_p, []),
diff --git a/demucs_amd/csrc/api.hip b/demucs_amd/csrc/api.hip
--- a/demucs_amd/csrc/api.hip
+++ b/demucs_amd/csrc/api.hip
@@ -7,6 +7,7 @@
 
 post_launch_hook_t g_post_launch_hook = nullptr;
 int g_last_conv_route = -1;
+long long g_conv_route_launches[16][8] = {};
 int g_last_conv_tile = -1;
 
 char *last_error_buf() {
@@ -129,6 +130,13 @@
 void mi_debug_set_post_launch_hook(void (*hook)(void *stream)) { g_post_launch_hook = hook; }
 int mi_debug_last_conv_route(void) { return g_last_conv_route; }
 int mi_debug_last_conv_tile(void) { return g_last_conv_tile; }
+int64_t mi_debug_conv_route_launches(int32_t route, int32_t epi) {
+    if (route < 0 || route >= 16 || epi >= 8) return -1;
+    int64_t n = 0;
+    for (int e = 0; e < 8; ++e)
+        if (epi < 0 || e == epi) n += mi::g_conv_route_launches[route][e];
+    return n;
+}
 int mi_debug_conv_route(const struct mi_conv_desc *desc, int *tile) {
     if (!desc) return -1;
     if (conv_check_tile_m(*desc) != MI_OK) return -1;
diff --git a/demucs_amd/csrc/common.h b/demucs_amd/csrc/common.h
--- a/demucs_amd/csrc/common.h
+++ b/demucs_amd/csrc/common.h
@@ -25,6 +25,7 @@
 extern post_launch_hook_t g_post_launch_hook;
 extern int g_last_conv_route;
 extern int g_last_conv_tile;
+extern long long g_conv_route_launches[16][8];
 
 #define MI_CHECK_LAUNCH()                                                   \
     do {                                                                    \
diff --git a/demucs_amd/csrc/conv_route.hip b/demucs_amd/csrc/conv_route.hip
--- a/demucs_amd/csrc/conv_route.hip
+++ b/demucs_amd/csrc/conv_route.hip
@@ -39,6 +39,17 @@
     return !off && !d.half && (split ? has_image : !has_image) && d.ktab && epi_ok && (plain || d.dma_rows) && (tile == 64 || tile == 96 || tile == 128) &&
            d.Mpad % tile == 0 && d.S2 == 1 && d.O2 == ld && ld % 4 == 0 && ((uintptr_t)d.x & 3) == 0 && ((uintptr_t)d.ktab & 63) == 0 &&
            (d.epi == MI_EPI_CONVTR || tile != 64 || d.epi == MI_EPI_LINEAR);
+}
+
+static bool dmatime_eligible(const mi_conv_desc &d, int tile, bool plain, bool has_image) {
+    const int ld = d.x_ld ? d.x_ld : d.D2, o2v = d.o2_valid ? d.o2_valid : d.O2;
+    const int lf = d.flags & (MI_FLAG_GELU | MI_FLAG_SCALE | MI_FLAG_RES | MI_FLAG_LN | MI_FLAG_STATS | MI_FLAG_IMG | MI_FLAG_IMG4 | MI_FLAG_HEADS);
+    const bool tr = d.epi == MI_EPI_CONVTR && !(d.flags & (MI_FLAG_TR_FREQ | MI_FLAG_IMG)) && d.K % 2 == 0 && d.S2 == 1 && d.O2 % 4 == 0 &&
+                    d.o2_valid == d.D2 + 1 && d.o2_valid <= d.O2 && d.x_bstride == (int64_t)(d.K / 2) * ld;
+    const bool enc = d.epi == MI_EPI_LINEAR && lf == MI_FLAG_GELU && d.K % 8 == 0 && d.S2 == 4 && 4 * (int64_t)o2v <= (int64_t)d.D2 + 3 &&
+                     d.x_bstride == (int64_t)(d.K / 8) * ld;
+    return d.dma_time && !d.half && has_image && !plain && (tr || enc) && (tile == 96 || tile == 128) && d.Mpad % tile == 0 && d.D1 == 1 &&
+           d.O1 == 1 && d.S1 == 1 && ld >= d.D2 && ((uintptr_t)d.x & 3) == 0;
 }
 
 int conv_check_tile_m(const mi_conv_desc &d) {
@@ -126,6 +137,8 @@
     };
     if (!plain && !sw.x6_plain_only && dmatap_eligible(d, tile, image, true)) return {MI_ROUTE_TAP_X6, split_tile(d.ntaps), plain};
     if (!sw.x6_plain_only && dmarow_eligible(d, tile, plain, image, true)) return {MI_ROUTE_ROWS_X6, split_tile(kRowTaps), plain};
+    if (!sw.x6_plain_only && dmatime_eligible(d, tile, plain, image))
+        return {MI_ROUTE_TIME_X6, split_tile(d.epi == MI_EPI_CONVTR ? kTimeTr : kTimeEnc), plain};
     const int ktile = small && !plain && d.epi == MI_EPI_GLU && d.Mpad % 96 == 0 ? 96 : tile;
     if (!plain && dmatap_eligible(d, ktile, image)) return {MI_ROUTE_DMATAP, ktile, plain};
     if (dmarow_eligible(d, tile, plain, image)) return {MI_ROUTE_DMAROW, tile, plain};
diff --git a/demucs_amd/csrc/engine_core.h b/demucs_amd/csrc/engine_core.h
--- a/demucs_amd/csrc/engine_core.h
+++ b/demucs_amd/csrc/engine_core.h
@@ -83,6 +83,7 @@
     SPLIT_OPT_IN,
     SPLIT_DEFAULT,
     SPLIT_ROWS,
+    SPLIT_TIME,
 };
 
 struct WeightTable {
diff --git a/demucs_amd/csrc/engine_core.hip b/demucs_amd/csrc/engine_core.hip
--- a/demucs_amd/csrc/engine_core.hip
+++ b/demucs_amd/csrc/engine_core.hip
@@ -89,10 +89,10 @@
     if (!prof.on) return launch_conv(d, st);
     const int route = conv_route(d).route;
     const int tile = d.tile_m && d.tile_m != 192 ? d.tile_m : conv_pick_tile(d.M), ti = tile == 32 ? 0 : tile == 64 ? 1 : tile == 96 ? 2 : 3;
-    const bool tap_x6 = route == MI_ROUTE_TAP_X6, rows_x6 = route == MI_ROUTE_ROWS_X6;
+    const bool tap_x6 = route == MI_ROUTE_TAP_X6, rows_x6 = route == MI_ROUTE_ROWS_X6, time_x6 = route == MI_ROUTE_TIME_X6;
     const int cls = tap_x6    ? 105 + (d.ntaps == 9 ? 2 : 0) + (tile == 128 ? 1 : 0)
                     : rows_x6 ? 109 + (d.epi == MI_EPI_CONVTR ? 4 : d.epi == MI_EPI_GLU ? 2 : 0) + (tile == 128 ? 1 : 0)
-                              : (route >= MI_ROUTE_X6 ? 48 : 0) + d.epi * 8 + ti * 2 + (d.plain ? 1 : 0);
+                              : (route >= MI_ROUTE_X6 && !time_x6 ? 48 : 0) + d.epi * 8 + ti * 2 + (d.plain ? 1 : 0);
     const double N = (double)d.B * d.O1 * d.O2;
     const double in_bytes = 4.0 * (double)d.B * (double)d.x_bstride;
     double out_rows = d.M;
@@ -115,7 +115,7 @@
 
 int EngineCore::pack_split(PackedConv *pc, SplitScope scope) {
     const Switches &sw = switches();
-    const bool in_default = scope == SPLIT_DEFAULT || (scope == SPLIT_ROWS && !sw.no_dma_rows);
+    const bool in_default = scope == SPLIT_DEFAULT || scope == SPLIT_TIME || (scope == SPLIT_ROWS && !sw.no_dma_rows);
     const bool want = sw.x6_scope == 2 || (sw.x6_scope == 1 && in_default && cfg.dtype == MI_DTYPE_F32);
     if (!want || !conv_x6_supported(pc->tile)) return MI_OK;
     const bool t192 = pc->M % 192 == 0 && pc->Mpad == pc->M;
diff --git a/demucs_amd/csrc/gemm_conv.h b/demucs_amd/csrc/gemm_conv.h
--- a/demucs_amd/csrc/gemm_conv.h
+++ b/demucs_amd/csrc/gemm_conv.h
@@ -79,6 +79,8 @@
     int64_t yh_pq;
     int32_t dma_rows;
     int32_t dma_rows_pad;
+    int32_t dma_time;
+    int32_t dma_time_pad;
 } mi_conv_desc;
 
 #ifdef __cplusplus
diff --git a/demucs_amd/csrc/gemm_conv.hip b/demucs_amd/csrc/gemm_conv.hip
--- a/demucs_amd/csrc/gemm_conv.hip
+++ b/demucs_amd/csrc/gemm_conv.hip
@@ -211,6 +211,7 @@
     const int image_tile = d.tile_m == 192 ? 96 : d.tile_m ? d.tile_m : conv_pick_tile(d.M);
     g_last_conv_route = r.route;
     g_last_conv_tile = r.tile;
+    if ((unsigned)r.route < 16u && (unsigned)d.epi < 8u) ++g_conv_route_launches[r.route][d.epi];
     switch (r.route) {
         case MI_ROUTE_TAP_HALF: return launch_conv_tap(d, r.tile, st);
         case MI_ROUTE_HALF:
@@ -218,6 +219,7 @@
         case MI_ROUTE_HALF_IMG256: return launch_conv_half(d, r, st);
         case MI_ROUTE_TAP_X6: return launch_conv_tap_x6(d, r.tile, image_tile, st);
         case MI_ROUTE_ROWS_X6: return launch_conv_rows_x6(d, r.tile, image_tile, st);
+        case MI_ROUTE_TIME_X6: return launch_conv_time_x6(d, r.tile, image_tile, st);
         case MI_ROUTE_X6: return launch_conv_x6(d, r.tile, image_tile, r.plain, st);
         case MI_ROUTE_DMATAP:
             return d.epi == MI_EPI_GLU ? launch_dmatap<MI_EPI_GLU>(d, r.tile, st) : launch_dmatap<MI_EPI_BIAS_STATS>(d, r.tile, st);
diff --git a/demucs_amd/csrc/gemm_loop.h b/demucs_amd/csrc/gemm_loop.h
--- a/demucs_amd/csrc/gemm_loop.h
+++ b/demucs_amd/csrc/gemm_loop.h
@@ -270,8 +270,85 @@
 };
 #undef MI_ROW_LOADS
 
+struct TimeTrTaps {
+    const float *xcol;
+    int64_t chan;
+    int ci0, q0, tap, lofs;
+    bool valid, edge;
+    __device__ __forceinline__ TimeTrTaps(const mi_conv_desc &d, const Wg &w, int N, int64_t) {
+        const ColInfo lc = decompose(w.n0 + w.li * 4, N, w.P, d.O2, w.o2v);
+        valid = lc.valid; q0 = lc.o2; tap = w.lh;
+        chan = d.x_ld ? d.x_ld : d.D2;
+        ci0 = 2 * w.wave; lofs = w.lh * BN + w.li * 4;
+        xcol = d.x + (size_t)lc.b * d.x_bstride + lc.o2 - w.lh;
+        edge = valid && (q0 == 0 || q0 + 4 > d.D2);
+    }
+    __device__ __forceinline__ void prefetch(int) {}
+    __device__ __forceinline__ void issue(const mi_conv_desc &d, int kt, float *brows) const {
+        const float *const zero = d.sink + MI_SINK_FLOATS;
+#pragma unroll
+        for (int j = 0; j < 2; ++j) {
+            const int ci = kt * (BK / 2) + ci0 + j;
+            const bool ok = valid && 2 * ci < d.K;
+            const float *g = xcol + (int64_t)ci * chan;
+            lds_dma16_tracked(ok ? g : zero, brows + 2 * j * BN);
+        }
+    }
+    __device__ __forceinline__ void fix(const mi_conv_desc &d, int, float *brows) const {
+        if (!edge) return;
+        float *sb = brows + lofs;
+#pragma unroll
+        for (int j = 0; j < 2; ++j)
+#pragma unroll
+            for (int e = 0; e < 4; ++e)
+                if ((unsigned)(q0 + e - tap) >= (unsigned)d.D2) sb[2 * j * BN + e] = 0.f;
+    }
+};
+
+struct TimeEncTaps {
+    const float *xcol;
+    int64_t chan;
+    int s0, lofs, wbase;
+    bool valid, edge;
+    __device__ __forceinline__ TimeEncTaps(const mi_conv_desc &d, const Wg &w, int N, int64_t) {
+        const int half = w.wave & 1, chunk = w.wave >> 1, col = 64 * half + w.lane;
+        const ColInfo lc = decompose(w.n0 + col, N, w.P, d.O2, w.o2v);
+        valid = lc.valid;
+        s0 = 4 * lc.o2 - 2 + 4 * chunk;
+        chan = d.x_ld ? d.x_ld : d.D2;
+        xcol = d.x + (size_t)lc.b * d.x_bstride + s0;
+        wbase = (chunk * BN + 64 * half) * 4; lofs = wbase + 4 * w.lane;
+        edge = valid && (s0 < 0 || s0 + 3 >= d.D2);
+    }
+    __device__ __forceinline__ void prefetch(int) {}
+    __device__ __forceinline__ void issue(const mi_conv_desc &d, int kt, float *stage) const {
+        const float *const zero = d.sink + MI_SINK_FLOATS;
+#pragma unroll
+        for (int j = 0; j < 2; ++j) {
+            const int ci = 2 * kt + j;
+            const bool ok = valid && 8 * ci < d.K;
+            const float *g = xcol + (int64_t)ci * chan;
+            lds_dma16_tracked(ok ? g : zero, stage + j * (2 * BN * 4) + wbase);
+        }
+    }
+    __device__ __forceinline__ void fix(const mi_conv_desc &d, int, float *stage) const {
+        if (!edge) return;
+#pragma unroll
+        for (int j = 0; j < 2; ++j)
+#pragma unroll
+            for (int e = 0; e < 4; ++e)
+                if ((unsigned)(s0 + e) >= (unsigned)d.D2) stage[j * (2 * BN * 4) + lofs + e] = 0.f;
+    }
+    static __device__ __forceinline__ void read(const float *stage, int bn, int bh, float (&v)[8]) {
+        const float4 a = *reinterpret_cast<const float4 *>(stage + ((2 * bh) * BN + bn) * 4);
+        const float4 b = *reinterpret_cast<const float4 *>(stage + ((2 * bh + 1) * BN + bn) * 4);
+        v[0] = a.x; v[1] = a.y; v[2] = a.z; v[3] = a.w; v[4] = b.x; v[5] = b.y; v[6] = b.z; v[7] = b.w;
+    }
+};
+
 template <int NT, int DIL = 1>
-using BLoader = std::conditional_t<NT == 0, PlainRows, std::conditional_t<NT == kRowTaps, RowTaps, TapRows<(NT > 0 ? NT : 3), DIL>>>;
+using BLoader = std::conditional_t<NT == 0, PlainRows, std::conditional_t<NT == kRowTaps, RowTaps, std::conditional_t<NT == kTimeTr, TimeTrTaps,
+                                   std::conditional_t<NT == kTimeEnc, TimeEncTaps, TapRows<(NT > 0 ? NT : 3), DIL>>>>>;
 
 struct ConvGeom { int N, MT, NT; };
 static inline int conv_geom(const mi_conv_desc &d, const char *what, int tile, int image_rows, ConvGeom &g, int bn = BN) {
diff --git a/demucs_amd/csrc/gemm_x6.hip b/demucs_amd/csrc/gemm_x6.hip
--- a/demucs_amd/csrc/gemm_x6.hip
+++ b/demucs_amd/csrc/gemm_x6.hip
@@ -35,7 +35,9 @@
     static_assert(NT <= 0 || (!PLAIN && EPI == MI_EPI_GLU), "tap loader: GLU rewrite convs");
     static_assert(!ROWS || (!PLAIN && (EPI == MI_EPI_LINEAR || EPI == MI_EPI_CONVTR || EPI == MI_EPI_GLU)),
                   "row-tap loader: encoder / transposed convs, 1 x 1 + GLU rewrites");
-    static_assert(NT >= kRowTaps, "NT: taps, 0 or kRowTaps");
+    static_assert(NT != kTimeTr || (!PLAIN && EPI == MI_EPI_CONVTR), "time-axis two-tap loader: transposed convs");
+    static_assert(NT != kTimeEnc || (!PLAIN && EPI == MI_EPI_LINEAR && LFLAGS == MI_FLAG_GELU), "time-axis strided loader: encoder convs");
+    static_assert(NT >= kTimeEnc, "NT: taps, 0, kRowTaps, kTimeTr or kTimeEnc");
     static_assert(WN * TN * 32 == BN, "block N tile is 128");
     static_assert(WM * WN == 4, "4 waves");
     constexpr int A_BYTES = BM * 96, B_BYTES = BN * 96, STAGE = A_BYTES + B_BYTES;
@@ -74,11 +76,16 @@
     const size_t b_row = lc.valid ? (size_t)w.P : 0, b_step = lc.valid ? (size_t)BK * w.P : 0;
     float breg[8];
     BLoader<NT> L(d, w, N, w.P);
-#define MI_BRAW_DMA(kt, rs) L.issue(d, (kt), braw + (rs) * (BK * BN) + (4 * w.wave) * BN)
-#define MI_BRAW_FIX(kt, rs) L.fix(d, (kt), braw + (rs) * (BK * BN) + (4 * w.wave) * BN)
+    constexpr bool OWN_STAGE = NT == kTimeEnc;
+#define MI_BRAW_DMA(kt, rs) L.issue(d, (kt), braw + (rs) * (BK * BN) + (OWN_STAGE ? 0 : 4 * w.wave) * BN)
+#define MI_BRAW_FIX(kt, rs) L.fix(d, (kt), braw + (rs) * (BK * BN) + (OWN_STAGE ? 0 : 4 * w.wave) * BN)
 #define MI_BRAW_READ(rs)                                                                                            \
     do {                                                                                                            \
-        _Pragma("unroll") for (int j = 0; j < 8; ++j) breg[j] = braw[(rs) * (BK * BN) + (8 * bh + j) * BN + bn];     \
+        if constexpr (OWN_STAGE) {                                                                                  \
+            L.read(braw + (rs) * (BK * BN), bn, bh, breg);                                                          \
+        } else {                                                                                                    \
+            _Pragma("unroll") for (int j = 0; j < 8; ++j) breg[j] = braw[(rs) * (BK * BN) + (8 * bh + j) * BN + bn]; \
+        }                                                                                                           \
     } while (0)
 
 #define MI_B_LOAD(kt)                                                                                               \
@@ -207,6 +214,16 @@
     conv_x6_body<WM, WN, TM, TN, EPI, LFLAGS, false, HALF_IMG, kRowTaps>(d, N, MT, Gm);
 }
 
+template <int WM, int WN, int TM, int TN, bool HALF_IMG>
+__global__ __launch_bounds__(256, 2) void conv_time_tr_x6_kernel(const mi_conv_desc d, const int N, const int MT, const int Gm) {
+    conv_x6_body<WM, WN, TM, TN, MI_EPI_CONVTR, 0, false, HALF_IMG, kTimeTr>(d, N, MT, Gm);
+}
+
+template <int WM, int WN, int TM, int TN, bool HALF_IMG>
+__global__ __launch_bounds__(256, 2) void conv_time_enc_x6_kernel(const mi_conv_desc d, const int N, const int MT, const int Gm) {
+    conv_x6_body<WM, WN, TM, TN, MI_EPI_LINEAR, MI_FLAG_GELU, false, HALF_IMG, kTimeEnc>(d, N, MT, Gm);
+}
+
 template <int WM, int WN, int TM, int TN, int EPI, int LFLAGS, bool PLAIN, bool HALF_IMG = false, int NTAPS = 0>
 static int launch_cfg_x6(const mi_conv_desc &d, hipStream_t st) {
     constexpr int BM = WM * TM * 32;
@@ -215,6 +232,8 @@
     const int Gm = pick_m_groups(g.MT, (size_t)d.Kpad * d.Mpad * 6);
     if constexpr (NTAPS > 0) MI_LAUNCH_TILES((conv_tap_x6_kernel<WM, WN, TM, TN, HALF_IMG, NTAPS>), d, g, Gm, st);
     else if constexpr (NTAPS == kRowTaps) MI_LAUNCH_TILES((conv_rows_x6_kernel<WM, WN, TM, TN, EPI, LFLAGS, HALF_IMG>), d, g, Gm, st);
+    else if constexpr (NTAPS == kTimeTr) MI_LAUNCH_TILES((conv_time_tr_x6_kernel<WM, WN, TM, TN, HALF_IMG>), d, g, Gm, st);
+    else if constexpr (NTAPS == kTimeEnc) MI_LAUNCH_TILES((conv_time_enc_x6_kernel<WM, WN, TM, TN, HALF_IMG>), d, g, Gm, st);
     else MI_LAUNCH_TILES((conv_gemm_x6_kernel<WM, WN, TM, TN, EPI, LFLAGS, PLAIN, HALF_IMG>), d, g, Gm, st);
     return MI_OK;
 }
@@ -260,6 +279,19 @@
     return launch_tile_x6<MI_EPI_LINEAR, MI_FLAG_GELU, false, kRowTaps>(d, tile, image_tile, st);
 }
 
+int launch_conv_time_x6(const mi_conv_desc &d, int tile, int image_tile, hipStream_t st) {
+    MI_REQUIRE(d.wx && ((uintptr_t)d.wx & 15) == 0, "conv time x6: split weight image missing or misaligned");
+    MI_REQUIRE((image_tile == 96 || image_tile == 128) && d.D1 == 1 && d.O1 == 1, "conv time x6: a 1-D layer on a 96- or 128-row tile (tile %d)", image_tile);
+    if (d.epi == MI_EPI_CONVTR) {
+        MI_REQUIRE(d.O2 % 4 == 0 && d.o2_valid == d.D2 + 1 && d.o2_valid <= d.O2 && d.K % 2 == 0,
+                   "conv time x6: columns 0 .. D2 on a pitch that is a multiple of 4 (D2 %d, O2 %d, o2_valid %d)", d.D2, d.O2, d.o2_valid);
+        return launch_tile_x6<MI_EPI_CONVTR, 0, false, kTimeTr>(d, tile, image_tile, st);
+    }
+    MI_REQUIRE(d.epi == MI_EPI_LINEAR && (d.flags & (MI_FLAG_GELU | MI_FLAG_SCALE | MI_FLAG_RES | MI_FLAG_LN | MI_FLAG_STATS)) == MI_FLAG_GELU &&
+               d.S2 == 4 && d.K % 8 == 0, "conv time x6: CONVTR, or LINEAR + GELU with k = 8, s = 4 (epi %d, flags %d, S2 %d)", d.epi, d.flags, d.S2);
+    return launch_tile_x6<MI_EPI_LINEAR, MI_FLAG_GELU, false, kTimeEnc>(d, tile, image_tile, st);
+}
+
 int launch_conv_x6(const mi_conv_desc &d, int tile, int image_tile, bool plain, hipStream_t st) {
     MI_REQUIRE(d.wx && ((uintptr_t)d.wx & 15) == 0, "conv x6: split weight image missing or misaligned");
     return dispatch_epilogue(d, [&](auto epi, auto lflags) {
diff --git a/demucs_amd/csrc/kernels.h b/demucs_amd/csrc/kernels.h
--- a/demucs_amd/csrc/kernels.h
+++ b/demucs_amd/csrc/kernels.h
@@ -139,14 +139,19 @@
 const Switches &switches();
 constexpr bool conv_x6_supported(int tile) { return tile == 128 || tile == 96 || tile == 64; }
 constexpr int kRowTaps = -1;
+constexpr int kTimeTr = -2;
+constexpr int kTimeEnc = -3;
 constexpr bool conv_x6_tile192(int epi, int lflags, bool plain, int ntaps) {
     if (ntaps > 0) return epi == MI_EPI_GLU;
+    if (ntaps == kTimeTr) return epi == MI_EPI_CONVTR;
+    if (ntaps == kTimeEnc) return epi == MI_EPI_LINEAR && lflags == MI_FLAG_GELU;
     if (ntaps == kRowTaps) return (epi == MI_EPI_LINEAR && lflags == MI_FLAG_GELU) || epi == MI_EPI_CONVTR || epi == MI_EPI_GLU;
     return plain && epi == MI_EPI_LINEAR && lflags == MI_FLAG_LN;
 }
 int launch_conv_x6(const mi_conv_desc &d, int tile, int image_tile, bool plain, hipStream_t st);
 int launch_conv_tap_x6(const mi_conv_desc &d, int tile, int image_tile, hipStream_t st);
 int launch_conv_rows_x6(const mi_conv_desc &d, int tile, int image_tile, hipStream_t st);
+int launch_conv_time_x6(const mi_conv_desc &d, int tile, int image_tile, hipStream_t st);
 int launch_pack_split(const float *wt, int Kpad, int Mpad, int tile_m, void *wx, hipStream_t st);
 
 int launch_conv_half(const mi_conv_desc &d, const ConvRoute &r, hipStream_t st);
diff --git a/demucs_amd/csrc/model.hip b/demucs_amd/csrc/model.hip
--- a/demucs_amd/csrc/model.hip
+++ b/demucs_amd/csrc/model.hip
@@ -75,7 +75,7 @@
         MI_TRY(wt.get(pt + ".rewrite.weight", (int64_t)2 * C * C, &rw));
         MI_TRY(wt.get(pt + ".rewrite.bias", 2 * C, &rb));
         EncW &te = tenc[i];
-        MI_TRY(pack_conv(w, b, C, Cint * 8, false, &te.conv));
+        MI_TRY(pack_conv(w, b, C, Cint * 8, false, &te.conv, 0, i > 0 ? SPLIT_TIME : SPLIT_OPT_IN));
         if (i) MI_TRY(pack_enc_tap(w, Cint, &te.conv));
         MI_TRY(make_ktab(Gather{Cint, 1, 8, 1, 1, 0, 2, (int64_t)Lp[i], Lp[i]}, te.conv.Kpad, &te.ktab_conv));
         MI_TRY(pack_conv(rw, rb, 2 * C, C, true, &te.rewrite, 0, i >= 2 ? SPLIT_ROWS : SPLIT_OPT_IN));
@@ -116,7 +116,7 @@
         MI_TRY(pack_conv(rw, rb, 2 * C, C * 3, true, &td.rewrite, 3, SPLIT_DEFAULT));
         MI_TRY(make_ktab(Gather{C, 1, 3, 1, 1, 0, 1, (int64_t)L, L}, td.rewrite.Kpad, &td.ktab_rw));
         MI_TRY(load_dconv(wt, pt, C, (int64_t)L, L, false, &td.dconv));
-        MI_TRY(pack_convtr(w, b, C, Coutt, &td.convtr));
+        MI_TRY(pack_convtr(w, b, C, Coutt, &td.convtr, 4, j < 3 ? SPLIT_TIME : SPLIT_OPT_IN));
         MI_TRY(make_ktab(Gather{C, 1, 2, 1, -1, 0, 0, (int64_t)L, L}, td.convtr.Kpad, &td.ktab_tr));
     }
     const int Tf = 8 * T, Tt = Lt[4];
@@ -249,7 +249,9 @@
     size_t big = 0;
     for (int i = 0; i < 4; ++i) {
         const size_t nf = (size_t)kCh[i] * kFr[i + 1] * T, nt = (size_t)kCh[i] * Lp[i + 1];
-        MI_TRY(A(&w.w_skip[i], nf)); MI_TRY(A(&w.w_skip_t[i], nt));
+        MI_TRY(A(&w.w_skip[i], nf));
+        MI_TRY(w.mem.alloc((void **)&w.w_skip_t[i], (nt * B + 64) * sizeof(float)));
+        w.w_skip_t[i] += 32;
         big = std::max(big, std::max(nf, nt));
     }
     if (cfg.dtype != MI_DTYPE_F32)
@@ -492,6 +494,7 @@
             mi_conv_desc d = base_desc(tenc[i].conv, tenc[i].ktab_conv, xt, (int64_t)Cint * Lp[i], gin);
             d.O2 = Lp[i + 1]; d.o2_valid = Lt[i + 1]; d.S2 = 4; d.epi = MI_EPI_LINEAR; d.flags = MI_FLAG_GELU;
             d.y = w_ta; d.y_bstride = C * P; d.y_cstride = P;
+            if (d.wx && !d.half) d.dma_time = 1;
             if (plan.enc_img[1][i]) {
                 const int Qp = round_up(ceil_div(Lt[i], 4) + 1, 4);
                 d.xh = w_eimg[1][i - 1]; d.xh_n = (int64_t)cfg.max_batch * Qp; d.wtap = tenc[i].conv.wtap; d.ntaps = 2; d.tap_k2 = 2;
@@ -587,6 +590,9 @@
             mi_conv_desc t = base_desc(tdec[j].convtr, tdec[j].ktab_tr, w_ta, (int64_t)C * L, g);
             t.O2 = Lv + 1; t.o2_valid = 0; t.epi = MI_EPI_CONVTR; t.out_len = Lout;
             t.y_cstride = Lpo; t.y_bstride = (int64_t)Cout * Lpo;
+            if (t.wx && !t.half) {
+                t.O2 = round_up(Lv + 1, 4); t.o2_valid = Lv + 1; t.dma_time = 1;
+            }
             if (last) t.y = w_ytime;
             else { t.flags |= MI_FLAG_GELU | MI_FLAG_RES; t.res = w_skip_t[2 - j]; t.y = dtin; }
             if (!last && tapimg) { t.flags |= MI_FLAG_IMG; t.yh = dtin; t.yh_n = (int64_t)B * t.y_cstride; }
diff --git a/include/demucs_amd.h b/include/demucs_amd.h
--- a/include/demucs_amd.h
+++ b/include/demucs_amd.h
@@ -359,12 +359,15 @@
     MI_ROUTE_TAP_X6 = 7,
     MI_ROUTE_ROWS_X6 = 8,
     MI_ROUTE_HALF_IMG = 9,
-    MI_ROUTE_HALF_IMG256 = 10
+    MI_ROUTE_HALF_IMG256 = 10,
+    MI_ROUTE_TIME_X6 = 11
 };
 
 int mi_debug_last_conv_route(void);
 
 int mi_debug_last_conv_tile(void);
+
+int64_t mi_debug_conv_route_launches(int32_t route, int32_t epi);
 
 int mi_debug_conv_route(const struct mi_conv_desc *desc, int *tile);
 
```

New measurement: 2452, median of 6. 1.9% higher.
